# nianticlabs/panoptic-forecasting

Hardware: AMD Instinct MI355X
Metric: forecast frames/sec @1024x2048, 3-in->dt=3 bg (higher is better)
Workload: dtype f32 as 2 fp16 terms/operand, 3 MFMA products, f32 accumulate (strict f32: fp32_only); 1 GPU; configs[1] bg short-term forecast 3-in dt=3 @1024x2048: 3 warp/splats + HarDNet-70 + upsample/argmax; resident_frames_per_gpu=128, streams=4, sub_batch=32, launch=hipGraph replay, sub-batches staggered, weights=random-init, calibrated (tests/golden/calib_seed1234.json), world=1, device=AMD Radeon Graphics, backend=single process

## Files before the change

### include/pfhip.h

```cpp
#ifndef PFHIP_H
#define PFHIP_H

#include <stddef.h>
#include <stdint.h>

#ifdef __cplusplus
extern "C" {
#endif

#define PF_OK 0
#define PF_EINVAL (-1)
#define PF_EWORKSPACE (-2)
#define PF_EBLOB (-3)
#define PF_EHIP (-4)
#define PF_EUNSUPPORTED (-5)

typedef struct pf_plan pf_plan;

int pf_version(void);
const char *pf_last_error(void);

#define PF_SPLAT_PER_FRAME 1
#define PF_SPLAT_PER_SAMPLE_SENTINEL 2
int pf_warp_splat_workspace(int B, int T, int H, int W, int per_frame, size_t *bytes);
int pf_warp_splat(const float *depth, const uint8_t *depth_mask, const uint8_t *seg, int seg_channels,
                  const float *Kinv, const float *E, const float *T_tgt, const float *Einv,
                  const float *K, int B, int T_total, int t_first, int T, int H, int W, int per_frame,
                  uint8_t *out_seg, float *out_depth, int64_t *out_result2d,
                  void *ws, size_t ws_bytes, void *stream);

int pf_hardnet_plan_create(const void *blob_host, size_t bytes, int in_ch, int n_cls, pf_plan **out);
void pf_hardnet_plan_destroy(pf_plan *plan);
int pf_hardnet_workspace(const pf_plan *plan, int B, int H, int W, size_t *bytes);

#define PF_STATUS_RANGE 1u
#define PF_STATUS_RANGE_LOW 2u
#define PF_WS_STATUS_OFFSET 0
#define PF_WS_STICKY_OFFSET 4
#define PF_WS_STATUS_BYTES 2048
int pf_hardnet_status(const void *ws, unsigned *status, void *stream);
int pf_hardnet_status_sticky(void *ws, unsigned *status, int clear, void *stream);
int pf_hardnet_status_reset(void *ws, void *stream);
int pf_hardnet_range_maxima(const pf_plan *plan, const void *ws, float *maxima, int cap, int *n_ops, void *stream);

#define PF_HOP_NONE 0
#define PF_HOP_TRAINID_LUT 1
#define PF_HOP_DEPTH_U16 2

int pf_bg_forward(const pf_plan *plan, const void *seg, int seg_is_i64, const float *depth,
                  const uint8_t *depth_mask, float depth_mean, float depth_std, int hop_flags,
                  float min_depth, float max_depth, int B, int T, int H, int W, int out_h, int out_w,
                  void *out_seg, int out_seg_is_i64, float *out_logits, float *out_orig_logits,
                  void *ws, size_t ws_bytes, void *stream);

int pf_hardnet_forward_dense(const pf_plan *plan, const float *x, int B, int H, int W, int out_h,
                             int out_w, void *out_seg, int out_seg_is_i64, float *out_logits,
                             float *out_orig_logits, void *ws, size_t ws_bytes, void *stream);

int pf_hop_export(const void *seg, int seg_is_i64, int seg_mode, const float *depth, size_t n, uint8_t *out_seg,
                  uint16_t *out_depth_u16, void *stream);
int pf_hop_load(const uint16_t *depth_u16, size_t n, float min_depth, float max_depth, float *out_depth,
                uint8_t *out_mask, void *stream);

int pf_panoptic_merge_workspace(int n_instances, size_t *bytes);
int pf_panoptic_merge(const void *background, int bg_kind, const float *bg_depth, const uint8_t *bg_depth_mask,
                      const float *masks, int MH, int MW, const float *boxes, int box_is_ulbr,
                      const float *inst_depth, const int64_t *classes, const int32_t *inst_offsets,
                      int n_instances, int B, int H, int W, int use_depth_sorting, int panoptic_ids,
                      int clear_things, void *out, int out_is_i64, void *ws, size_t ws_bytes, void *stream);
int pf_panoptic_encode(const void *seg, int seg_is_i64, int convert_to_ids, int B, int H, int W, uint8_t *out_rgb,
                       int32_t *out_ids, uint8_t *out_present, void *stream);
int pf_panoptic_max_ids(void);

int pf_bg_dense_input(const void *frames, int kind, int channels, const float *depth, const uint8_t *depth_mask, float depth_mean,
                      float depth_std, int B, int T, int H, int W, float *x, void *stream);

int pf_seg_loss_workspace(int B, int out_h, int out_w, size_t *bytes);
int pf_seg_loss(const float *logits, int B, int C, int Hin, int Win, const void *labels, int labels_i64, int out_h,
                int out_w, int ignore_index, double *out3, void *ws, size_t ws_bytes, void *stream);

int pf_fg_weights_size(int flags, size_t *raw_floats, size_t *packed_floats);
int pf_fg_pack(const float *raw, float *packed, int flags, void *stream);
int pf_fg_workspace(int N, int T_in, int T_out, int flags, size_t *bytes);
int pf_fg_forward(const float *packed, int flags, int N, int T_in, int T_out, int odom_T, const float *trajs,
                  const float *traj_mask, const float *vel_mask, const float *feats, const int64_t *output_inds,
                  const float *odom, const float *depths, const float *depth_mask, const int64_t *classes,
                  float *traj_norm, float *traj_unnorm, float *mask_feats, float *output_feats, float *masks,
                  void *ws, size_t ws_bytes, void *stream);

int pf_odom_weights_size(int flags, size_t *raw_floats, size_t *packed_floats);
int pf_odom_pack(const float *raw, float *packed, int flags, void *stream);
int pf_odom_forward(const float *packed, int flags, int B, int T_in, int T_out, const float *inps, float *out,
                    float *out_norm, void *stream);

int pf_set_option(const char *name, int value);
int pf_hardnet_plan_set_option(pf_plan *plan, const char *name, int value);

typedef struct pf_train pf_train;
int pf_train_create(const void *blob, size_t blob_bytes, int in_ch, int n_cls, pf_train **out);
void pf_train_destroy(pf_train *t);
int pf_train_autotune(pf_train *t, int enable);
int pf_train_tuned_shapes(const pf_train *t, int *rows, int cap_rows, int *n_rows);
int pf_train_path_stats(const pf_train *t, int *stats, int cap, int *n);
int pf_train_param_count(const pf_train *t, size_t *n_floats);
int pf_train_param_layout(const pf_train *t, int op_index, size_t *w_off, size_t *aux_off, int *has_bn);
int pf_train_workspace(const pf_train *t, int B, int H, int W, int out_h, int out_w, size_t *bytes);
int pf_train_forward_backward(const pf_train *t, float *theta, float *grad, int accumulate_grads, const void *seg, int seg_is_i64,
                              const float *depth, const uint8_t *depth_mask, float depth_mean, float depth_std, int T,
                              const float *x_dense, int B, int H, int W, const void *labels, int labels_i64, int out_h, int out_w,
                              int ignore_index, float loss_scale, float bn_momentum, float bn_eps, int update_running_stats,
                              double *out3, void *ws, size_t ws_bytes, void *stream);
int pf_train_tensor_view(const pf_train *t, const char *name, int want_grad, int B, int H, int W, int out_h, int out_w,
                         size_t *ws_offset, int *channels, int *h, int *w);
int pf_sgd_workspace(size_t *bytes);
int pf_sgd_step(float *theta, float *grad, float *momentum_buf, const uint8_t *trainable, size_t n, float lr, float momentum,
                float weight_decay, float clip_norm, float clip_value, int first_step, void *ws, size_t ws_bytes, void *stream);

int pf_hardnet_tensor_view(const pf_plan *plan, const char *name, int B, int H, int W,
                           size_t *ws_offset, int *channels, int *h, int *w);
int pf_hardnet_tensor_read(const pf_plan *plan, const char *name, int B, int H, int W, const void *ws, float *dst, void *stream);
int pf_s4_pack(const float *src, void *dst, int B, int C, int H, int W, unsigned *status, void *stream);
int pf_s4_unpack(const void *src, float *dst, int B, int C, int H, int W, void *stream);
int pf_hardnet_flops(const pf_plan *plan, int H, int W, double *flops);

int pf_profile_enable(int on);
int pf_profile_collect(void);
int pf_profile_get(int i, char *label, size_t label_cap, int *launches, double *total_ms, double *flops,
                   double *bytes);

int pf_debug_force_conv(int kind, int p0, int p1, int p2);
int pf_debug_probe_read(long long *host64);

#ifdef __cplusplus
}
#endif
#endif
```

### panoptic-forecasting_amd/bg_model.py

```python
import collections.abc
import ctypes

import torch
import torch.nn.functional as F
from torch import nn

from . import hardnet_arch as arch
from . import lib as _lib
from . import packing
from .model_api import BaseModel
from .pc_transform_model import _as_u8


PLAN_OPTIONS = {'split_f16': 'split_f16', 'split_bf16': 'split_f16', 'fuse_pool': 'fuse_pool', 'fuse_upsample': 'fuse_upsample',
                'use_tuned_table': 'use_tuned_table', 'valu_remainder': 'valu_remainder', 'conv_table_batch': 'table_batch',
                'range_guard': 'range_guard', 'fuse_front': 'fuse_front', 'fuse_pairs': 'fuse_pairs'}
PF_STATUS_RANGE, PF_STATUS_RANGE_LOW = 1, 2
PF_STATUS_ANY = PF_STATUS_RANGE | PF_STATUS_RANGE_LOW
PF_WS_STATUS_BYTES = 2048


class _Pending:
    __slots__ = ('slot', 'event', 'stream', 'args', 'outs', 'done', 'stamps', 'error')


def _stamp(t):
    if not torch.is_tensor(t):
        return None
    return (t.data_ptr(), None if t.is_inference() else t._version)


def _unversioned(stamps):
    return any(s is not None and s[1] is None for s in stamps)


class LazyResult(collections.abc.MutableMapping):

    __slots__ = ('_data', '_model', '_token')

    def __init__(self, data, model, token):
        self._data, self._model, self._token = dict(data), model, token

    def _resolve(self):
        if self._token is not None:
            self._model._resolve(self._token)
            self._token = None

    def __getitem__(self, k):
        self._resolve()
        return self._data[k]

    def __setitem__(self, k, v):
        self._data[k] = v

    def __delitem__(self, k):
        self._resolve()
        del self._data[k]

    def __iter__(self):
        return iter(self._data)

    def __len__(self):
        return len(self._data)

    def __contains__(self, k):
        return k in self._data

    def keys(self):
        return self._data.keys()

    def copy(self):
        self._resolve()
        return dict(self._data)

    def __or__(self, other):
        return {**self.copy(), **other}

    def __ror__(self, other):
        return {**other, **self.copy()}

    def __reduce__(self):
        return (dict, (self.copy(),))

    def __repr__(self):
        return 'LazyResult(%s%s)' % (list(self._data), ', unchecked' if self._token is not None else '')


class _Node(nn.Module):
    """Anonymous container: gives dotted state_dict paths without any behaviour."""


def _get_or_make(root, path):
    node = root
    for part in path:
        if not hasattr(node, part):
            node.add_module(part, _Node())
        node = getattr(node, part)
    return node


class HardNetParams(nn.Module):

    def __init__(self, in_ch, n_cls):
        super().__init__()
        self.spec = arch.Spec(in_ch, n_cls)
        for op in self.spec.conv_ops():
            parts = op.name.split('.')
            if op.bn:
                holder = _get_or_make(self, parts)
                cin = 3 if op.kind == arch.OP_STEM else op.cin
                holder.add_module('conv', nn.Conv2d(cin, op.cout, op.k, op.stride, op.k // 2, bias=False))
                holder.add_module('norm', nn.BatchNorm2d(op.cout))
            else:
                parent = _get_or_make(self, parts[:-1])
                conv = nn.Conv2d(op.cin, op.cout, op.k, op.stride, 0, bias=True)
                nn.init.kaiming_normal_(conv.weight)
                parent.add_module(parts[-1], conv)
        stem = getattr(self.base, '0').conv
        w = stem.weight.data.mean(1, keepdim=True).expand(-1, in_ch, -1, -1).clone()
        stem.weight = nn.Parameter(w)

    def load_pretrained(self, path):
        sd = torch.load(path, map_location='cpu')['model_state']
        sd = {k[len('module.'):]: v for k, v in sd.items()}
        own = self.state_dict()
        for k, v in sd.items():
            if k in own and own[k].shape == v.shape:
                own[k].copy_(v)
            elif k == 'base.0.conv.weight':
                own[k].copy_(v.mean(1, keepdim=True).expand_as(own[k]))


class BGModel(BaseModel):

    def __init__(self, params):
        super().__init__()
        self.num_classes = num_classes = params['data']['num_classes']
        self.use_depth_inps = params['model'].get('use_depth_inps')
        self.num_inputs = params['model'].get('num_inputs', 1)
        self.min_depth = params['data'].get('min_depth')
        self.max_depth = params['data'].get('max_depth')
        self.convert2onehot = params['model'].get('convert2onehot')
        self.return_logits = params['model'].get('return_logits', True)
        final_w = params['model'].get('final_w')
        final_h = params['model'].get('final_h')
        self.final_size = (final_h, final_w) if final_w is not None and final_h is not None else None
        in_ch = num_classes
        if self.use_depth_inps:
            depth_norm_params = params['data'].get('depth_norm_params')
            if depth_norm_params is None:
                mean, std = torch.zeros(1), torch.zeros(1)
            else:
                mean, std = depth_norm_params
            self.depth_mean = nn.Parameter(torch.as_tensor(mean, dtype=torch.float32).reshape(1).clone(),
                                           requires_grad=False)
            self.depth_std = nn.Parameter(torch.as_tensor(std, dtype=torch.float32).reshape(1).clone(),
                                          requires_grad=False)
            in_ch += 1
        in_ch *= self.num_inputs
        self.in_ch = in_ch
        self.model = HardNetParams(in_ch, num_classes)
        pretrain = params['model'].get('hardnet', {}).get('pretrain_path')
        if pretrain is not None:
            self.model.load_pretrained(pretrain)
        self.plan_options = {c_name: int(params['model'][key]) for key, c_name in PLAN_OPTIONS.items()
                             if params['model'].get(key) is not None}
        self.on_range_overflow = params['model'].get('on_range_overflow', 'rerun')
        if self.on_range_overflow not in ('rerun', 'raise', 'ignore'):
            raise ValueError("model.on_range_overflow must be 'rerun', 'raise' or 'ignore'")
        self.range_check = params['model'].get('range_check', 'lazy')
        if self.range_check not in ('lazy', 'sync'):
            raise ValueError("model.range_check must be 'lazy' or 'sync'")
        self.range_reruns = 0
        self._pending = []
        self._pinned = None
        self._ring_next = 0
        self._plan = None
        self._ws = None
        self._norm = None
        self._trainer = None
        self._params_for_trainer = {'data': dict(params['data']), 'model': dict(params['model']),
                                    'training': dict(params.get('training') or {})}

    def load_state_dict(self, state_dict, strict=True):
        res = super().load_state_dict(state_dict, strict)
        self.invalidate()
        return res

    def invalidate(self):
        if self._pending:
            self._drain()
        if self._plan is not None:
            _lib.load().pf_hardnet_plan_destroy(self._plan)
        self._plan = None
        self._norm = None

    def __del__(self):
        try:
            self._pending = []
            self.invalidate()
        except Exception:
            pass

    def _get_plan(self):
        if self._plan is None:
            L = _lib.load()
            blob = packing.pack_blob(self.state_dict(), self.in_ch, self.num_classes)
            buf = ctypes.create_string_buffer(blob, len(blob))
            plan = ctypes.c_void_p()
            _lib.check(L.pf_hardnet_plan_create(buf, len(blob), self.in_ch, self.num_classes, ctypes.byref(plan)),
                       'pf_hardnet_plan_create')
            self._plan = plan
            for name, value in self.plan_options.items():
                _lib.check(L.pf_hardnet_plan_set_option(plan, name.encode(), value), 'pf_hardnet_plan_set_option')
            if self.use_depth_inps:
                self._norm = (float(self.depth_mean.item()), float(self.depth_std.item()))
        return self._plan

    def _workspace(self, b, h, w, device):
        L = _lib.load()
        need = ctypes.c_size_t()
        _lib.check(L.pf_hardnet_workspace(self._get_plan(), b, h, w, ctypes.byref(need)), 'pf_hardnet_workspace')
        if self._ws is None or self._ws.numel() < need.value or self._ws.device != device:
            if torch.cuda.is_current_stream_capturing():
                raise _lib.PfError('bg forward: the workspace must exist before stream capture (run one forward first)')
            self._drain()
            self._ws = torch.empty(need.value, dtype=torch.uint8, device=device)
            self._ws[:PF_WS_STATUS_BYTES].zero_()
        return self._ws

    def _guarded(self):
        return not (self.on_range_overflow == 'ignore' or self.plan_options.get('split_f16', 1) == 0
                    or self.plan_options.get('range_guard', 1) == 0)

    def range_status(self):
        if self._ws is None:
            return 0
        return int(self._ws[:4].view(torch.int32).item())

    def range_status_sticky(self, clear=False):
        if self._ws is None:
            return 0
        w = self._ws[4:8].view(torch.int32)
        v = int(w.item())
        if clear:
            w.zero_()
        return v

    def check_range(self, clear=True):
        self._drain()
        v = self.range_status_sticky(clear)
        if (v & PF_STATUS_ANY) and self._guarded():
            raise _lib.PfError('bg forward: status %d (PF_STATUS_RANGE = 1: |activation| > 65504, PF_STATUS_RANGE_LOW = 2: a tensor of '
                               'tiny values) on the two-term fp16 operand path inside a captured graph: the outputs of the flagged '
                               'replays are not usable; run eagerly (re-run on fp32) or with model.split_f16 = 0' % v)
        return v

    def range_maxima(self):
        L, plan = _lib.load(), self._get_plan()
        names = [op.name for op in self.model.spec.ops]
        buf = (ctypes.c_float * len(names))()
        n = ctypes.c_int()
        _lib.check(L.pf_hardnet_range_maxima(plan, self._ws.data_ptr(), buf, len(names), ctypes.byref(n), _lib.stream_ptr()),
                   'pf_hardnet_range_maxima')
        return {names[i]: float(buf[i]) for i in range(n.value)}

    _RING = 32

    def _resolve(self, token, owner=True):
        if token.done:
            if token.error is not None and owner:
                raise token.error
            return
        if not token.event.query():
            token.event.synchronize()
        token.done = True
        if token in self._pending:
            self._pending.remove(token)
        status = int(self._pinned[token.slot, 0])
        args, outs, stamps = token.args, token.outs, token.stamps
        token.args = token.outs = token.stamps = None
        if not (status & PF_STATUS_ANY):
            return
        if self.on_range_overflow == 'raise':
            token.error = _lib.PfError('bg forward: status %d on the two-term fp16 operand path (PF_STATUS_RANGE = 1: an activation '
                                       'exceeded 65504; PF_STATUS_RANGE_LOW = 2: a tensor of tiny values, max below 2^-6); run with '
                                       "model.split_f16 = 0 or on_range_overflow = 'rerun'" % status)
        elif stamps is not None and stamps != tuple(_stamp(t) for t in args[:3]):
            token.error = _lib.PfError('bg forward: status %d on the two-term fp16 operand path, and the input tensors of that forward were '
                                       'modified in place before its result was first touched - the fp32 re-run cannot see the original '
                                       "frame.  Keep a forward's inputs unchanged until its result has been read (or model.settle()), or "
                                       "build the model with model.range_check = 'sync'" % status)
        if token.error is not None:
            if owner:
                raise token.error
            return
        L, plan = _lib.load(), self._get_plan()
        self.range_reruns += 1
        prior = self.plan_options.get('split_f16', 1)
        _lib.check(L.pf_hardnet_plan_set_option(plan, b'split_f16', 0), 'pf_hardnet_plan_set_option')
        try:
            here = torch.cuda.current_stream()
            with torch.cuda.stream(token.stream):
                self._run_once(*args, outs=outs)
            if here != token.stream:
                here.wait_stream(token.stream)
        finally:
            _lib.check(L.pf_hardnet_plan_set_option(plan, b'split_f16', prior), 'pf_hardnet_plan_set_option')

    def _poll(self):
        while self._pending and self._pending[0].event.query():
            self._resolve(self._pending[0], owner=False)

    def _drain(self):
        while self._pending:
            self._resolve(self._pending[0], owner=False)

    def settle(self):
        self._drain()

    def run_async(self, inps, depths, depth_masks, want_logits=True, want_orig=True, hop_flags=0, seg_dtype=torch.int64,
                  own_inputs=False):
        capturing = torch.cuda.is_current_stream_capturing()
        if not capturing:
            self._poll()
        args = (inps, depths, depth_masks, want_logits, want_orig, hop_flags, seg_dtype)
        outs = self._run_once(*args)
        if not self._guarded() or capturing:
            return outs, None
        if self._pinned is None:
            self._pinned = torch.zeros((self._RING, 2), dtype=torch.int32).pin_memory()
        slot = self._ring_next
        self._ring_next = (slot + 1) % self._RING
        for t in list(self._pending):
            if t.slot == slot:
                self._resolve(t, owner=False)
        self._pinned[slot].copy_(self._ws[:8].view(torch.int32), non_blocking=True)
        token = _Pending()
        token.slot, token.args, token.outs, token.done, token.error = slot, args, outs, False, None
        token.stamps = None if own_inputs else tuple(_stamp(t) for t in args[:3])
        token.stream = torch.cuda.current_stream()
        token.event = torch.cuda.Event()
        token.event.record(token.stream)
        self._pending.append(token)
        if token.stamps is not None and _unversioned(token.stamps):
            self._resolve(token)
            return outs, None
        return outs, token

    def run(self, inps, depths, depth_masks, want_logits=True, want_orig=True, hop_flags=0, seg_dtype=torch.int64):
        outs, token = self.run_async(inps, depths, depth_masks, want_logits, want_orig, hop_flags, seg_dtype)
        if token is not None:
            self._resolve(token)
        return outs

    def _run_once(self, inps, depths, depth_masks, want_logits, want_orig, hop_flags, seg_dtype, outs=None):
        L = _lib.load()
        plan = self._get_plan()
        fused = bool(self.convert2onehot and self.use_depth_inps and inps.dim() == 4)
        if fused:
            b, t, h, w = inps.shape
        else:
            x = self._dense_input(inps, depths, depth_masks)
            b, _, h, w = x.shape
        dev = inps.device
        oh, ow = self.final_size if self.final_size is not None else (h, w)
        ws = self._workspace(b, h, w, dev)
        if outs is not None:
            seg, logits, orig = outs
        else:
            seg = torch.empty((b, oh, ow), dtype=seg_dtype, device=dev)
            logits = torch.empty((b, self.num_classes, oh, ow), dtype=torch.float32, device=dev) if want_logits else None
            orig = None
            if want_orig:
                vo, vc, vh, vw = ctypes.c_size_t(), ctypes.c_int(), ctypes.c_int(), ctypes.c_int()
                _lib.check(L.pf_hardnet_tensor_view(plan, b'finalConv', b, h, w, ctypes.byref(vo), ctypes.byref(vc),
                                                    ctypes.byref(vh), ctypes.byref(vw)), 'pf_hardnet_tensor_view')
                orig = torch.empty((b, vc.value, vh.value, vw.value), dtype=torch.float32, device=dev)
        ptr = lambda t_: t_.data_ptr() if t_ is not None else None
        i64 = int(seg_dtype == torch.int64)
        if fused:
            if inps.dtype not in (torch.uint8, torch.int64):
                inps = inps.long()
            inps = _lib.require_cuda(inps.contiguous(), 'seg')
            depths = _lib.require_cuda(depths.float().contiguous(), 'depth')
            mask = None
            if not (hop_flags & 2):
                mask = _lib.require_cuda(_as_u8(depth_masks), 'depth_mask')
            mean, std = self._norm
            rc = L.pf_bg_forward(plan, inps.data_ptr(), int(inps.dtype == torch.int64), depths.data_ptr(), ptr(mask),
                                 mean, std, hop_flags, float(self.min_depth or 0.0), float(self.max_depth or 0.0),
                                 b, t, h, w, oh, ow, seg.data_ptr(), i64, ptr(logits), ptr(orig),
                                 ws.data_ptr(), ws.numel(), _lib.stream_ptr())
            _lib.check(rc, 'pf_bg_forward')
        else:
            x = _lib.require_cuda(x.contiguous(), 'input')
            rc = L.pf_hardnet_forward_dense(plan, x.data_ptr(), b, h, w, oh, ow, seg.data_ptr(), i64, ptr(logits),
                                            ptr(orig), ws.data_ptr(), ws.numel(), _lib.stream_ptr())
            _lib.check(rc, 'pf_hardnet_forward_dense')
        return seg, logits, orig

    def _dense_input(self, inps, depths, depth_masks):
        L = _lib.load()
        if self.convert2onehot:
            b, t, h, w = inps.shape
            if inps.dtype not in (torch.uint8, torch.int64):
                inps = inps.long()
            frames, kind, c = _lib.require_cuda(inps.contiguous(), 'seg'), int(inps.dtype == torch.int64), self.num_classes
        else:
            b, t, c, h, w = inps.shape
            frames, kind = _lib.require_cuda(inps.float().contiguous(), 'seg'), 2
        dptr = mptr = None
        mean = std = 0.0
        if self.use_depth_inps:
            depths = _lib.require_cuda(depths.float().contiguous(), 'depth')
            mask = _lib.require_cuda(_as_u8(depth_masks), 'depth_mask')
            dptr, mptr = depths.data_ptr(), mask.data_ptr()
            self._get_plan()
            mean, std = self._norm
        x = torch.empty((b, t * c + (t if self.use_depth_inps else 0), h, w), dtype=torch.float32, device=inps.device)
        _lib.check(L.pf_bg_dense_input(frames.data_ptr(), kind, c, dptr, mptr, mean, std, b, t, h, w, x.data_ptr(), _lib.stream_ptr()),
                   'pf_bg_dense_input')
        return x

    def forward(self, inps, depths, depth_masks, return_orig_size=False):
        _, logits, orig = self.run(inps, depths, depth_masks, True, return_orig_size)
        return (logits, orig) if return_orig_size else logits

    def loss(self, inputs, labels):
        if self.training:
            return self._train_loss(inputs, labels)
        with torch.no_grad():
            return self._eval_loss(inputs, labels)

    def _get_trainer(self):
        from . import bg_train
        if self._trainer is None:
            self._trainer = bg_train.BGTrainer(self._params_for_trainer, device='cuda')
        if not self._trainer.is_adopted():
            self._trainer.adopt(self)
        return self._trainer

    def _train_loss(self, inputs, labels):
        from . import bg_train
        tr = self._get_trainer()
        self.invalidate()
        loss, acc = bg_train.TrainStepFunction.apply(tr, inputs, labels, *tr._adopted)
        torch._foreach_add_(self._bn_counters(), 1)
        return {'loss': loss, 'accuracy': acc}

    def _bn_counters(self):
        return [b for k, b in self.named_buffers() if k.endswith('num_batches_tracked')]

    def _eval_loss(self, inputs, labels):
        L = _lib.load()
        seg_labels = labels['seg']
        _, _, orig = self.run(inputs['seg'], inputs.get('depth'), inputs.get('depth_mask'), want_logits=False, want_orig=True)
        if seg_labels.dtype not in (torch.uint8, torch.int64):
            seg_labels = seg_labels.long()
        seg_labels = _lib.require_cuda(seg_labels.contiguous(), 'labels')
        b, c, hin, win = orig.shape
        oh, ow = seg_labels.shape[-2], seg_labels.shape[-1]
        need = ctypes.c_size_t()
        _lib.check(L.pf_seg_loss_workspace(b, oh, ow, ctypes.byref(need)), 'pf_seg_loss_workspace')
        ws = torch.empty(need.value, dtype=torch.uint8, device=orig.device)
        out3 = torch.empty(3, dtype=torch.float64, device=orig.device)
        _lib.check(L.pf_seg_loss(orig.data_ptr(), b, c, hin, win, seg_labels.data_ptr(), int(seg_labels.dtype == torch.int64), oh, ow,
                                 255, out3.data_ptr(), ws.data_ptr(), ws.numel(), _lib.stream_ptr()), 'pf_seg_loss')
        return {'loss': (out3[0] / out3[1]).float(), 'accuracy': (out3[2] / out3[1]).float()}

    @torch.no_grad()
    def predict(self, inputs, labels=None):
        (seg, logits, orig), token = self.run_async(inputs['seg'], inputs.get('depth'), inputs.get('depth_mask'),
                                                    want_logits=self.return_logits, want_orig=True)
        out = {'seg': seg, 'orig_size_logits': orig}
        if logits is not None:
            out['logits'] = logits
        if token is not None and self.range_check == 'sync':
            self._resolve(token)
            token = None
        return LazyResult(out, self, token)
```

### panoptic-forecasting_amd/csrc/conv_mfma.h

```cpp
#pragma once
#include "pf_blob.h"
#include "pf_common.h"

namespace pf {

struct ConvArgs {
    const float *src[kConvMaxSrc];
    int src_ctotal[kConvMaxSrc];
    int src_choff[kConvMaxSrc];
    int src_cstart[kConvMaxSrc + 1];
    int src_chunk0[kConvMaxSrc + 1];
    int n_src;
    const float *wpk;
    const float *bias;
    float *dst;
    int dst_ctotal, dst_choff;
    int Cin, Cout, Hin, Win, Hout, Wout;
    int tilesX, tilesY, nchunks, relu;
    const float *zero_page;
    int ntiles;
    int no_bias;
    int pool;
    const float *res;
    int res_ctotal, res_choff, Hres, Wres;
    float res_sh, res_sw;
    int res_lds_off;
    int res_rows, res_cols;
    unsigned res_magic_cs, res_magic_cols;
    const float *wrem;
    int rem;
    int src_begin, src_end;
    int chunk_begin, chunk_end;
    long long *probe;
    unsigned *status;
    unsigned *range_slot;
    int kacc;
    int accum;
    float acc_scale;
    int dst_fmt;
    int dst_c4;
    int dst_limit;
    int src_fmt;
    int src_c4[kConvMaxSrc];
    int src_g0[kConvMaxSrc];
    int src_gn[kConvMaxSrc];
    int src_ent0[kConvMaxSrc + 1];
};

typedef _Float16 split_t;
typedef split_t split_x2 __attribute__((ext_vector_type(2)));
typedef split_t split_x4 __attribute__((ext_vector_type(4)));
typedef split_t split_x8 __attribute__((ext_vector_type(8)));
constexpr float kSplitMaxAbs = 65504.f;
__device__ __forceinline__ void split_terms2(float x0, float x1, split_x2 &hi, split_x2 &mid) {
#if defined(__HIP_DEVICE_COMPILE__)
    typedef float f32x2 __attribute__((ext_vector_type(2)));
    hi = __builtin_convertvector(f32x2{x0, x1}, split_x2);
    const unsigned hu = __builtin_bit_cast(unsigned, hi);
    unsigned mu;
    asm("v_fma_mixlo_f16 %0, %1, -1.0, %2 op_sel_hi:[1,0,0]" : "=v"(mu) : "v"(hu), "v"(x0));
    asm("v_fma_mixhi_f16 %0, %1, -1.0, %2 op_sel:[1,0,0] op_sel_hi:[1,0,0]" : "+v"(mu) : "v"(hu), "v"(x1));
    mid = __builtin_bit_cast(split_x2, mu);
#endif
}
__device__ __forceinline__ float range_acc(float m, float a, float b, float c, float d) {
#if defined(__HIP_DEVICE_COMPILE__)
    asm("v_max3_f32 %0, %0, |%1|, |%2|" : "+v"(m) : "v"(a), "v"(b));
    asm("v_max3_f32 %0, %0, |%1|, |%2|" : "+v"(m) : "v"(c), "v"(d));
#endif
    return m;
}
constexpr float kRangeTarget = 8.0f;
constexpr float kRangeLowMax = 0.015625f;
__device__ __forceinline__ bool range_sampled() {
#if defined(__HIP_DEVICE_COMPILE__)
    const unsigned total = gridDim.x * gridDim.y * gridDim.z;
    const unsigned id = blockIdx.x + gridDim.x * (blockIdx.y + gridDim.y * blockIdx.z);
    const unsigned mask = total >= 16u ? (1u << (28 - __builtin_clz(total))) - 1u : 0u;
    return (((id * 0x9E3779B1u) >> 9) & mask) == 0u;
#else
    return false;
#endif
}
__device__ __forceinline__ void range_commit(unsigned *status, unsigned *slot, float m) {
#if defined(__HIP_DEVICE_COMPILE__)
    if (status == nullptr) return;
    if (!(m <= kSplitMaxAbs)) atomicOr(status, 1u);
    if (slot == nullptr || !range_sampled()) return;
    const unsigned mb = __builtin_bit_cast(unsigned, m);
    unsigned wm = 0;
    unsigned long long above = __builtin_amdgcn_ballot_w64(mb > wm);
    while (above != 0) {
        wm = (unsigned)__builtin_amdgcn_readlane((int)mb, (int)__builtin_ctzll(above));
        above = __builtin_amdgcn_ballot_w64(mb > wm);
    }
    const unsigned lane_id = __builtin_amdgcn_mbcnt_hi(~0u, __builtin_amdgcn_mbcnt_lo(~0u, 0u));
    if (lane_id == (unsigned)__builtin_ctzll(__builtin_amdgcn_ballot_w64(true))) atomicMax(slot, wm | 1u);
#endif
}
template <typename V4>
__device__ __forceinline__ void split_terms4(const V4 &v, split_x4 &hi, split_x4 &mid) {
    split_x2 h0, m0, h1, m1;
    split_terms2(v[0], v[1], h0, m0);
    split_terms2(v[2], v[3], h1, m1);
    hi = split_x4{h0[0], h0[1], h1[0], h1[1]};
    mid = split_x4{m0[0], m0[1], m1[0], m1[1]};
}
#define PF_MFMA_SPLIT(a, b, c) __builtin_amdgcn_mfma_f32_16x16x32_f16((a), (b), (c), 0, 0, 0)
unsigned short split_host_f16(float x);
float split_host_f32(unsigned short h);
float split_weight_scale(const float *w, size_t n);

__device__ __forceinline__ void xcd_tile_order(int ntiles_xy, int &tile_lin, int &group) {
#if defined(__HIP_DEVICE_COMPILE__)
    if ((ntiles_xy & 7) != 0) {
        tile_lin = (int)blockIdx.x;
        group = (int)blockIdx.y;
        return;
    }
    const int ngroups = (int)gridDim.y;
    const int lin = (int)blockIdx.x + ntiles_xy * (int)blockIdx.y;
    const int xcd = lin & 7, pos = lin >> 3;
    const int t = pos / ngroups;
    group = pos - t * ngroups;
    tile_lin = xcd * (ntiles_xy >> 3) + t;
#endif
}

struct ConvTiling {
    int ks, stride;
    int kc;
    int nt;
    int twt;
    int cout_blocks, nchunks;
    size_t packed_floats() const { return (size_t)cout_blocks * nchunks * (kc / 4) * ks * ks * nt * 64; }
};

ConvTiling choose_tiling(int ks, int stride, int cin, int cout, int wout_hint);
void pack_conv_weights(const float *w_oihw, int cin, int cout, const ConvTiling &t, float *out);
int launch_conv(const ConvArgs &a, const ConvTiling &t, int B, hipStream_t stream);

constexpr int dma_kc_ct(int ks, int stride) { return ks == 1 ? 16 : (stride == 2 ? 4 : 8); }
inline int dma_kc(int ks, int stride) { return dma_kc_ct(ks, stride); }
int dma_chunks(const int *src_ch, int n_src, int ks, int stride);
inline int dma_rem_rv(int rem) { return rem <= 2 ? 2 : (rem + 3) / 4 * 4; }
inline int dma_valu_split(int cout) {
    if (cout < 16) return 0;
    return cout % 16;
}
void pack_conv_weights_rem(const float *w_oihw, int cin, int cout, int rem, int ks, int kc, const int *src_ch, int n_src, float *out);
void pack_conv_weights_tiled(const float *w_oihw, int cin, int cout, int ks, int kc, const int *src_ch, int n_src, float *out);
int launch_conv_dma(const ConvArgs &a, int ks, int stride, int B, hipStream_t stream, int force_wm = 0, int force_nt = 0, int model_B = 0);
bool conv_dma_supported(const ConvArgs &a, int ks, int stride, int B, int force_wm, int force_nt, int model_B, int *wm, int *nt);

constexpr int wave_kc_ct(int ks) { return ks == 1 ? 32 : 8; }
inline int wave_kc(int ks) { return wave_kc_ct(ks); }
int wave_chunks(const int *src_ch, int n_src, int ks);
void pack_conv_weights_wave(const float *w_oihw, int cin, int cout, int ks, const int *src_ch, int n_src, float *out);
size_t wave_packed_floats(const int *src_ch, int n_src, int cout, int ks);
int launch_conv_wave(const ConvArgs &a, int ks, int mh, int nt, int wk, int B, hipStream_t stream);
bool conv_wave_supported(const ConvArgs &a, int ks, int mh, int nt, int wk);
constexpr size_t wave_lds_bytes(int ks, int mh, int nt, int wk) {
    const int kc = wave_kc_ct(ks), ih = mh + ks - 1, iw = 16 + (ks == 3 ? 8 : 0);
    const int raw = ih * iw, plane = (raw + 15) / 32 * 32 + 16, nit = (kc * (plane / 4) + 63) / 64;
    const size_t ring = (size_t)wk * 2 * nit * 256, red = (size_t)wk * mh * nt * 256;
    return 4 * (ring > red ? ring : red);
}

int split_chunks(const int *src_ch, int n_src);
size_t split_packed_floats(const int *src_ch, int n_src, int cout);
void pack_conv_weights_split(const float *w_oihw, int cin, int cout, const int *src_ch, int n_src, float *out);
int launch_conv_split(const ConvArgs &a, int nt, int wide, int B, hipStream_t stream);
bool conv_split_supported(const ConvArgs &a);
int split1_chunks(const int *src_ch, int n_src);
size_t split1_packed_floats(const int *src_ch, int n_src, int cout);
void pack_conv_weights_split1(const float *w_oihw, int cin, int cout, const int *src_ch, int n_src, float *out);
int launch_conv_split1(const ConvArgs &a, int nt, int B, hipStream_t stream);
bool conv_split1_supported(const ConvArgs &a, int nt);

struct S4Range { int choff, ch; };
int s4_entries(const S4Range *r, int n_src, int ks, int pad_sources);
int s4_rounds(const S4Range *r, int n_src, int ks, int pad_sources);
size_t s4_packed_floats(const S4Range *r, int n_src, int cout, int ks, int pad_sources);
void pack_conv_weights_s4(const float *w_oihw, int cin, int cout, int ks, const S4Range *r, int n_src, int pad_sources, float *out);
int launch_conv_s4(const ConvArgs &a, int ks, int nt, int wide, int B, hipStream_t stream);
void pack_conv_weights_s4_ex(const float *w_oihw, int cin, int cout, int ks, const S4Range *r, const int *cstart, int n_src, int pad_sources, float *out);

struct PairArgs {
    ConvArgs c;
    const float *p_wpk;
    const float *p_w9;
    const float *p_bias;
    float p_acc_scale;
    float *p_dst;
    int p_dst_c4, p_dst_choff, p_dst_limit, p_cout, p_cin, p_ntiles, p_relu;
    unsigned *p_range_slot;
    int rounds_s;
    int round_d;
    int merged;
};
bool conv_pair_supports(int c_cout, int p_cout);
bool conv_pair_merged_supports(int c_cout, int p_cout);
bool pair_wanted(int p_cin, int p_cout, int c_cin, int c_cout, int h, int w, int B, int mode);
size_t pair_p_two_floats(const S4Range &r, int cout);
size_t pair_p_nine_floats(const S4Range &r, int cout);
void pack_conv_weights_pair_p(const float *w_oihw, int cin, int cout, const S4Range &r, float *two, float *nine);
int launch_conv_pair(const PairArgs &pa, int B, hipStream_t stream);
int launch_s4_pack(const float *src, void *dst, int B, int C, int H, int W, unsigned *status, hipStream_t stream);
int launch_range_check(const float *x, size_t n, unsigned *status, unsigned *slot, hipStream_t stream);
int launch_range_finalize(unsigned *st, int live_word, int first_slot, int n_slots, int sticky_word, hipStream_t stream);
int launch_s4_unpack(const void *src, float *dst, int B, int C, int H, int W, hipStream_t stream);

struct FrontArgs {
    const void *x;
    const void *w1, *w2;
    const float *bias1, *bias2;
    float scale1, scale2;
    float *dst;
    int dst_fmt, dst_c4, dst_ctotal, dst_choff, dst_limit;
    int H1, W1, H2, W2, C1, C2, relu1, relu2;
    int tilesX, tilesY;
    int seg_steps;
    unsigned *status;
    unsigned *range_slot_mid, *range_slot;
    long long *probe;
};

bool conv_front_supports(int c0, int c1, int c2, int h1, int w1, int dst_ctotal);
int launch_conv_front(const FrontArgs &a, int B, hipStream_t s);

struct ConvChoice {
    int kind, p0, p1, p2;
};
ConvChoice choose_conv(int ks, int stride, int cin, int cout, int hout, int wout, int B, int need = 0, int use_tuned = 1);
bool choose_s4(int ks, int cin, int cout, int hout, int wout, int B, ConvChoice *out);
long long *probe_buffer();
extern ConvChoice g_conv_force;

}
```

### panoptic-forecasting_amd/csrc/conv_s4.hip

```cpp
#include <cstring>
#include <vector>

#include "conv_s4.h"
#include "pf_prof.h"

#ifndef PF_PROBE
#define PF_PROBE 0
#endif
#if PF_PROBE
#define S4_PROBE(i) do { if (threadIdx.x == 0 && blockIdx.x == gridDim.x / 2 && blockIdx.y == 0 && blockIdx.z == gridDim.z / 2 && a.probe && (i) < 60) a.probe[i] = clock64(); } while (0)
#else
#define S4_PROBE(i) do { } while (0)
#endif

[[maybe_unused]] constexpr int kS4IssueFirst = 1, kS4IssueStep = 2;

namespace pf {

template <int NT, int TW_, int TH_ = 8, int KS_ = 1>
struct S4Cfg {
    static constexpr int TW = TW_, TH = TH_, MTR = TW / 16, MP = 2 * MTR;
    static constexpr int KS = KS_;
    static constexpr int NW = TH / 2, NTHR = 64 * NW;
    static constexpr int IW = TW + 4, IH = TH + 2;
    static constexpr int ROWP = IW / 2, PIECES = IH * ROWP;
    static constexpr int NDMA_ALL = (PIECES + 63) / 64;
    static constexpr int NDMA = (NDMA_ALL + NW / 4 - 1) / (NW / 4);
    static constexpr bool COLREG = (NT == 2 || NT == 3) && TW_ == 32;
    static constexpr int PLANE = COLREG ? PIECES * 16 : NDMA_ALL * 64 * 16;
    static constexpr int ABUF = 4 * PLANE;
    static constexpr int WBLK = 2 * 64 * 16;
    static constexpr int BPT = COLREG ? 2 : 3;
    static constexpr int WBUF = NT * BPT * WBLK;
    static constexpr int WPIECES = WBUF / 16, NITW = (WPIECES + NTHR - 1) / NTHR;
    static constexpr size_t STAGES_BYTES = 2 * (size_t)ABUF + 2 * (size_t)WBUF;
    static constexpr size_t LDS_BYTES = KS * STAGES_BYTES + NT * 16 * sizeof(float);
    static_assert(KS == 1 || (size_t)MP * NT * NW * 64 * 16 <= STAGES_BYTES, "the K-split hand-over uses group 1's stage ring");
};

#define S4_KERNEL_NAME conv_s4_kernel
#define S4_KERNEL_KACC 0
#define S4_KERNEL_WAVES (KS_ == 4 ? 1 : (TH_ == 16 || KS_ == 2) ? 2 : (TW_ == 32 && NT <= 2) ? 4 : (TW_ == 32 && NT == 3) ? 3 : 2)
#include "conv_s4_kernel.inc"
#undef S4_KERNEL_NAME
#undef S4_KERNEL_KACC
#undef S4_KERNEL_WAVES
#define S4_KERNEL_NAME conv_s4_blocked_kernel
#define S4_KERNEL_KACC 1
#define S4_KERNEL_WAVES (NT == 1 ? 4 : (NT == 2 ? 3 : 2))
#include "conv_s4_kernel.inc"
#undef S4_KERNEL_NAME
#undef S4_KERNEL_KACC
#undef S4_KERNEL_WAVES

template <int NT, int TW_, int TH_ = 8, int KS_ = 1>
static int launch_s4_cfg(const ConvArgs &a0, int B, hipStream_t s) {
    using C = S4Cfg<NT, TW_, TH_, KS_>;
    ConvArgs a = a0;
    a.tilesX = (a.Wout + C::TW - 1) / C::TW;
    a.tilesY = (a.Hout + C::TH - 1) / C::TH;
    static bool attr_set = false;
    if (!attr_set) {
        PF_HIP_CHECK(hipFuncSetAttribute(reinterpret_cast<const void *>(&conv_s4_kernel<NT, TW_, TH_, KS_>),
                                         hipFuncAttributeMaxDynamicSharedMemorySize, (int)C::LDS_BYTES));
        attr_set = true;
    }
    char label[96];
    snprintf(label, sizeof(label), "void pf::conv_s4_kernel<%d, %d, %d, %d>(pf::ConvArgs)", NT, TW_, TH_, KS_);
    const double px = (double)B * a.Hout * a.Wout;
    ProfScope ps(s, label, 2.0 * px * a.Cout * a.Cin * 9,
                 4.0 * ((double)B * a.Cin * a.Hin * a.Win + px * a.Cout + (double)a.Cout * a.Cin * 9));
    hipLaunchKernelGGL((conv_s4_kernel<NT, TW_, TH_, KS_>), dim3(a.tilesX * a.tilesY, (a.ntiles + NT - 1) / NT, B), dim3(C::NTHR * C::KS), C::LDS_BYTES, s, a);
    PF_LAUNCH_CHECK("conv_s4_kernel");
    return PF_OK;
}

template <int NT>
static int launch_s4_blocked_cfg(const ConvArgs &a0, int B, hipStream_t s) {
    using C = S4Cfg<NT, 32, 8, 1>;
    ConvArgs a = a0;
    a.tilesX = (a.Wout + C::TW - 1) / C::TW;
    a.tilesY = (a.Hout + C::TH - 1) / C::TH;
    static bool attr_set = false;
    if (!attr_set) {
        PF_HIP_CHECK(hipFuncSetAttribute(reinterpret_cast<const void *>(&conv_s4_blocked_kernel<NT, 32, 8, 1>), hipFuncAttributeMaxDynamicSharedMemorySize, (int)C::LDS_BYTES));
        attr_set = true;
    }
    char label[96];
    snprintf(label, sizeof(label), "void pf::conv_s4_blocked_kernel<%d, 32, 8, 1>(pf::ConvArgs)", NT);
    const double px = (double)B * a.Hout * a.Wout;
    ProfScope ps(s, label, 2.0 * px * a.Cout * a.Cin * 9, 4.0 * ((double)B * a.Cin * a.Hin * a.Win + px * a.Cout + (double)a.Cout * a.Cin * 9));
    hipLaunchKernelGGL((conv_s4_blocked_kernel<NT, 32, 8, 1>), dim3(a.tilesX * a.tilesY, (a.ntiles + NT - 1) / NT, B), dim3(C::NTHR), C::LDS_BYTES, s, a);
    PF_LAUNCH_CHECK("conv_s4_blocked_kernel");
    return PF_OK;
}

template <int NT>
struct S41Cfg {
    static constexpr int TW = 32, TH = 8, MP = 4;
    static constexpr int WBUF = NT * 2 * 64 * 16;
    static constexpr int BIAS_OFF = 2 * WBUF;
    static constexpr int MAIN = 2 * WBUF + 256;
    static constexpr int WPIECES = WBUF / 16, NITW = (WPIECES + 255) / 256;
};

typedef unsigned s4_u32x4 __attribute__((ext_vector_type(4)));
typedef unsigned s4_u32x2 __attribute__((ext_vector_type(2)));

template <int NT, int EPI>
__global__ __launch_bounds__(256, NT <= 2 ? 4 : (NT == 3 ? 3 : 2)) void conv_s4_1x1_kernel(ConvArgs a) {
#if defined(__HIP_DEVICE_COMPILE__)
    using C = S41Cfg<NT>;
    extern __shared__ __attribute__((aligned(16))) unsigned char smem_raw[];
    const int tid = threadIdx.x, lane = tid & 63;
    const int wave = __builtin_amdgcn_readfirstlane(tid >> 6);
    int tid_lin, cgroup;
    xcd_tile_order(a.tilesX * a.tilesY, tid_lin, cgroup);
    const int tileY = tid_lin / a.tilesX, tileX = tid_lin - tileY * a.tilesX;
    const int tile0 = cgroup * NT, b = blockIdx.z;
    const size_t plane_bytes = (size_t)a.Hin * a.Win * 8;
    auto wbuf = [&](int i) { return smem_raw + i * C::WBUF; };
    const int g = lane >> 4;

    s4_f32x4 acc[C::MP][NT];
#pragma unroll
    for (int m = 0; m < C::MP; ++m)
#pragma unroll
        for (int n = 0; n < NT; ++n) acc[m][n] = s4_f32x4{0.f, 0.f, 0.f, 0.f};
    const bool has_res = EPI == 1 && a.res && a.res_lds_off >= 0;
    ResWin rw = ResWin();

    int poff[2];
#pragma unroll
    for (int rr = 0; rr < 2; ++rr) {
        const int gy = tileY * C::TH + 2 * wave + rr, gx = tileX * C::TW + 2 * (lane & 15);
        poff[rr] = (gy < a.Hin && gx < a.Win) ? (gy * a.Win + gx) * 8 : -1;
    }
    unsigned woff[C::NITW];
#pragma unroll
    for (int it = 0; it < C::NITW; ++it) {
        const int p = it * 256 + tid, n = p / (2 * 64);
        woff[it] = (p < C::WPIECES && tile0 + n < a.ntiles) ? (unsigned)((tile0 + n) * a.nchunks * (2 * 64) + (p - n * (2 * 64))) * 16u : kS4Oob;
    }
    const __amdgpu_buffer_rsrc_t wrsrc = __builtin_amdgcn_make_buffer_rsrc((void *)a.wpk, 0, 0x7FFFFFFF, 0x00020000);

    float *bias_lds = reinterpret_cast<float *>(smem_raw + C::BIAS_OFF);
    if (wave == 0 && lane < NT * 16) {
        const __amdgpu_buffer_rsrc_t brs = __builtin_amdgcn_make_buffer_rsrc((void *)a.bias, 0, 0x7FFFFFFF, 0x00020000);
        const int co = tile0 * 16 + lane;
        __builtin_amdgcn_raw_ptr_buffer_load_lds(brs, (s4_lds_ptr_t)bias_lds, 4, (!a.no_bias && co < a.ntiles * 16) ? (unsigned)co * 4u : kS4Oob, 0,
                                                 0, 0);
    }

    const int cb = a.chunk_begin, nrounds = a.chunk_end - cb;
    auto load_round = [&](int r, s4_u32x4 (&x)[2][2][2]) {
#pragma unroll
        for (int h = 0; h < 2; ++h) {
            const int e = 8 * (cb + r) + 2 * g + h;
            const float *sp = a.src[0];
            int c4 = a.src_c4[0], g0 = a.src_g0[0], gn = a.src_gn[0], e0 = 0;
#pragma unroll
            for (int k = 1; k < kConvMaxSrc; ++k) {
                const bool take = k < a.n_src && e >= a.src_ent0[k];
                sp = take ? a.src[k] : sp;
                c4 = take ? a.src_c4[k] : c4;
                g0 = take ? a.src_g0[k] : g0;
                gn = take ? a.src_gn[k] : gn;
                e0 = take ? a.src_ent0[k] : e0;
            }
            const bool real = e - e0 < gn;
            const char *hi = reinterpret_cast<const char *>(sp) + ((size_t)b * 2 * c4 + (g0 + min(e - e0, gn - 1))) * plane_bytes;
            const size_t tstride = (size_t)c4 * plane_bytes;
#pragma unroll
            for (int rr = 0; rr < 2; ++rr) {
                const bool ok = real && poff[rr] >= 0;
                const char *p = ok ? hi + poff[rr] : reinterpret_cast<const char *>(a.zero_page);
                x[rr][h][0] = *reinterpret_cast<const s4_u32x4 *>(p);
                x[rr][h][1] = *reinterpret_cast<const s4_u32x4 *>(ok ? p + tstride : p);
            }
        }
    };
    auto load_weights = [&](int r, unsigned char *wdst) {
#pragma unroll
        for (int it = 0; it < C::NITW; ++it)
            if (it * 256 + tid < C::WPIECES)
                __builtin_amdgcn_raw_ptr_buffer_load_lds(wrsrc, (s4_lds_ptr_t)(wdst + (it * 256 + wave * 64) * 16), 16, woff[it],
                                                         (unsigned)(cb + r) * (2 * 64 * 16), 0, 0);
    };

    s4_u32x4 cur[2][2][2], nxt[2][2][2];
    if (nrounds > 0) {
        load_weights(0, wbuf(0));
        load_round(0, cur);
    }
    if (has_res) {
        rw = res_window(a, tileY * C::TH, C::TH, tileX * C::TW, C::TW);
        rw.rows = a.res_rows;
        rw.cols = a.res_cols;
        rw.cs = res_chan_stride(a.res_rows, a.res_cols);
        const unsigned per = (unsigned)(rw.rows * rw.cols), total = (unsigned)(NT * 16 * rw.cs);
        const size_t rplane = (size_t)a.Hres * a.Wres;
        const __amdgpu_buffer_rsrc_t rrs = __builtin_amdgcn_make_buffer_rsrc(
            (void *)(a.res + ((size_t)b * a.res_ctotal + a.res_choff + tile0 * 16) * rplane), 0, 0x7FFFFFFF, 0x00020000);
        unsigned char *rdst = smem_raw + a.res_lds_off * 4;
        for (unsigned e0 = (unsigned)wave * 64; e0 < total; e0 += 256) {
            const unsigned e = e0 + lane;
            const unsigned c = __umulhi(e, a.res_magic_cs), rem = e - c * (unsigned)rw.cs;
            const unsigned r = __umulhi(rem, a.res_magic_cols), x = rem - r * (unsigned)rw.cols;
            const int row = min(rw.sy0 + (int)r, a.Hres - 1), col = min(rw.sx0 + (int)x, a.Wres - 1);
            const bool ok = e < total && rem < per && tile0 * 16 + (int)c < a.Cout;
            const unsigned off = ok ? (unsigned)((c * rplane + (size_t)row * a.Wres + col) * 4) : kS4Oob;
            __builtin_amdgcn_raw_ptr_buffer_load_lds(rrs, (s4_lds_ptr_t)(rdst + e0 * 4), 4, off, 0, 0, 0);
        }
    }

    for (int round = 0; round < nrounds; ++round) {
        asm volatile("s_waitcnt vmcnt(0)" ::: "memory");
        __syncthreads();
        const bool more = round + 1 < nrounds;
        if (more) {
            load_weights(round + 1, wbuf((round + 1) & 1));
            load_round(round + 1, nxt);
        }
        const unsigned char *wb = wbuf(round & 1);
        s4_h8 bh[NT], bm[NT];
#pragma unroll
        for (int n = 0; n < NT; ++n) {
            bh[n] = *reinterpret_cast<const s4_h8 *>(wb + ((n * 2 + 0) * 64 + lane) * 16);
            bm[n] = *reinterpret_cast<const s4_h8 *>(wb + ((n * 2 + 1) * 64 + lane) * 16);
        }
#pragma unroll
        for (int rr = 0; rr < 2; ++rr)
#pragma unroll
            for (int q = 0; q < 2; ++q) {
                const s4_u32x4 h0 = cur[rr][0][0], h1 = cur[rr][1][0], m0 = cur[rr][0][1], m1 = cur[rr][1][1];
                const s4_u32x4 fh = q ? s4_u32x4{h0[2], h0[3], h1[2], h1[3]} : s4_u32x4{h0[0], h0[1], h1[0], h1[1]};
                const s4_u32x4 fm = q ? s4_u32x4{m0[2], m0[3], m1[2], m1[3]} : s4_u32x4{m0[0], m0[1], m1[0], m1[1]};
                const s4_h8 ah = __builtin_bit_cast(s4_h8, fh), am = __builtin_bit_cast(s4_h8, fm);
                const int m = rr * 2 + q;
#pragma unroll
                for (int n = 0; n < NT; ++n) acc[m][n] = PF_MFMA_SPLIT(bh[n], am, acc[m][n]);
#pragma unroll
                for (int n = 0; n < NT; ++n) acc[m][n] = PF_MFMA_SPLIT(bm[n], ah, acc[m][n]);
#pragma unroll
                for (int n = 0; n < NT; ++n) acc[m][n] = PF_MFMA_SPLIT(bh[n], ah, acc[m][n]);
            }
        if (more) {
#pragma unroll
            for (int rr = 0; rr < 2; ++rr)
#pragma unroll
                for (int h = 0; h < 2; ++h)
#pragma unroll
                    for (int t = 0; t < 2; ++t) cur[rr][h][t] = nxt[rr][h][t];
        }
    }

    if (has_res) {
        asm volatile("s_waitcnt vmcnt(0)" ::: "memory");
        __syncthreads();
    }
    {
        __builtin_amdgcn_s_waitcnt(0x0F70);
        const lds_float *res_lds = (const lds_float *)(reinterpret_cast<float *>(smem_raw) + (has_res ? a.res_lds_off : 0));
        const int i2 = 2 * (lane & 15);
        const int ox = tileX * C::TW + i2;
        const bool pooled = EPI == 1 && a.pool;
        const int Ho = pooled ? a.Hout >> 1 : a.Hout, Wo = pooled ? a.Wout >> 1 : a.Wout;
        const size_t hw = (size_t)Ho * Wo, term = (size_t)a.dst_c4 * hw * 8;
        const bool mis = (a.dst_choff & 2) != 0;
        typedef split_x2 h2;
        float vmax = 0.f;
        const float relu_lo1 = a.relu ? 0.f : -__builtin_inff();
        auto finish = [&](int rr, int q, int n, const int (&o0)[2], const int (&o1)[2], const float (&lx1)[2], float hy1) {
            s4_f32x4 v = acc[rr * 2 + q][n];
            const s4_f32x4 b4 = *reinterpret_cast<const s4_f32x4 *>(bias_lds + n * 16 + 4 * g);
#pragma unroll
            for (int r = 0; r < 4; ++r) {
                v[r] = v[r] * a.acc_scale + b4[r];
                if (has_res) {
                    const lds_float *chan = res_lds + (n * 16 + 4 * g + r) * rw.cs;
                    const float lx0 = 1.f - lx1[q], hy0 = 1.f - hy1;
                    const float t0 = lx0 * chan[o0[q]] + lx1[q] * chan[o0[q] + 1];
                    const float t1 = lx0 * chan[o1[q]] + lx1[q] * chan[o1[q] + 1];
                    v[r] += hy0 * t0 + hy1 * t1;
                }
                v[r] = fmaxf(v[r], relu_lo1);
            }
            vmax = range_acc(vmax, v[0], v[1], v[2], v[3]);
            return v;
        };
        auto store_px = [&](int co, size_t pix, s4_f32x4 v) {
            if (a.dst_fmt) {
                s4_h4 hi, mid;
                split_terms4(v, hi, mid);
                const int chb = a.dst_choff + co;
                const bool ok0 = chb < a.dst_limit, ok1 = chb + 2 < a.dst_limit;
                char *p = reinterpret_cast<char *>(a.dst) + (size_t)b * 2 * term + pix * 8 + (size_t)(chb >> 2) * hw * 8;
                if (!mis) {
                    if (ok1) {
                        *reinterpret_cast<s4_h4 *>(p) = hi;
                        *reinterpret_cast<s4_h4 *>(p + term) = mid;
                    } else if (ok0) {
                        *reinterpret_cast<h2 *>(p) = h2{hi[0], hi[1]};
                        *reinterpret_cast<h2 *>(p + term) = h2{mid[0], mid[1]};
                    }
                } else {
                    if (ok0) {
                        *reinterpret_cast<h2 *>(p + 4) = h2{hi[0], hi[1]};
                        *reinterpret_cast<h2 *>(p + 4 + term) = h2{mid[0], mid[1]};
                    }
                    if (ok1) {
                        *reinterpret_cast<h2 *>(p + hw * 8) = h2{hi[2], hi[3]};
                        *reinterpret_cast<h2 *>(p + hw * 8 + term) = h2{mid[2], mid[3]};
                    }
                }
            } else {
#pragma unroll
                for (int r = 0; r < 4; ++r)
                    if (co + r < a.Cout) a.dst[((size_t)b * a.dst_ctotal + a.dst_choff + co + r) * hw + pix] = v[r];
            }
        };
        auto store_pair = [&](int co, size_t pix, s4_f32x4 v0, s4_f32x4 v1) {
            const int chb = a.dst_choff + co;
            if (a.dst_fmt && !mis && chb + 2 < a.dst_limit) {
                s4_h4 h0, m0, h1, m1;
                split_terms4(v0, h0, m0);
                split_terms4(v1, h1, m1);
                const s4_h8 hi = s4_join(h0, h1), mid = s4_join(m0, m1);
                char *p = reinterpret_cast<char *>(a.dst) + (size_t)b * 2 * term + pix * 8 + (size_t)(chb >> 2) * hw * 8;
                *reinterpret_cast<s4_h8 *>(p) = hi;
                *reinterpret_cast<s4_h8 *>(p + term) = mid;
            } else if (!a.dst_fmt) {
                typedef float f2 __attribute__((ext_vector_type(2)));
#pragma unroll
                for (int r = 0; r < 4; ++r)
                    if (co + r < a.Cout)
                        *reinterpret_cast<f2 *>(a.dst + ((size_t)b * a.dst_ctotal + a.dst_choff + co + r) * hw + pix) = f2{v0[r], v1[r]};
            } else {
                store_px(co, pix, v0);
                store_px(co, pix + 1, v1);
            }
        };
#pragma unroll
        for (int rr = 0; rr < 2; ++rr) {
            if (pooled && rr == 1) continue;
            const int oy = tileY * C::TH + 2 * wave + rr;
            if (oy >= a.Hout || ox >= a.Wout) continue;
            if (pooled && oy + 1 >= a.Hout) continue;
            int o0[2] = {0, 0}, o1[2] = {0, 0}, p0[2] = {0, 0}, p1[2] = {0, 0};
            float lx1[2] = {0.f, 0.f}, hy1 = 0.f, hy1b = 0.f;
            if (has_res) {
                int y0, y1;
                float hy0;
                lin_coord(oy, a.res_sh, a.Hres, y0, y1, hy0, hy1);
                int z0 = 0, z1 = 0;
                if (pooled) lin_coord(oy + 1, a.res_sh, a.Hres, z0, z1, hy0, hy1b);
#pragma unroll
                for (int q = 0; q < 2; ++q) {
                    int x0, x1;
                    float lx0;
                    lin_coord(min(ox + q, a.Wout - 1), a.res_sw, a.Wres, x0, x1, lx0, lx1[q]);
                    o0[q] = (y0 - rw.sy0) * rw.cols + (x0 - rw.sx0);
                    o1[q] = (y1 - rw.sy0) * rw.cols + (x0 - rw.sx0);
                    p0[q] = (z0 - rw.sy0) * rw.cols + (x0 - rw.sx0);
                    p1[q] = (z1 - rw.sy0) * rw.cols + (x0 - rw.sx0);
                }
            }
#pragma unroll
            for (int n = 0; n < NT; ++n) {
                const int co = (tile0 + n) * 16 + 4 * g;
                if (co >= a.Cout + 2) continue;
                const s4_f32x4 va = finish(rr, 0, n, o0, o1, lx1, hy1), vb = finish(rr, 1, n, o0, o1, lx1, hy1);
                if (!pooled) {
                    store_pair(co, (size_t)oy * a.Wout + ox, va, vb);
                } else {
                    const s4_f32x4 vc = finish(1, 0, n, p0, p1, lx1, hy1b), vd = finish(1, 1, n, p0, p1, lx1, hy1b);
                    s4_f32x4 pv;
#pragma unroll
                    for (int r = 0; r < 4; ++r) pv[r] = (((va[r] + vb[r]) + vc[r]) + vd[r]) * 0.25f;
                    if ((oy >> 1) < Ho && (ox >> 1) < Wo) store_px(co, (size_t)(oy >> 1) * Wo + (ox >> 1), pv);
                }
                __builtin_amdgcn_sched_barrier(0);
            }
        }
        range_commit(a.status, a.range_slot, vmax);
    }
#endif
}

template <int NT, int EPI>
static int launch_s41_cfg(const ConvArgs &a0, int B, hipStream_t s) {
    using C = S41Cfg<NT>;
    ConvArgs a = a0;
    a.tilesX = (a.Wout + C::TW - 1) / C::TW;
    a.tilesY = (a.Hout + C::TH - 1) / C::TH;
    size_t lds = C::MAIN;
    a.res_lds_off = -1;
    if (a.res) {
        a.res_rows = res_extent(C::TH, a.res_sh);
        a.res_cols = res_extent(C::TW, a.res_sw);
        const int cs = res_chan_stride(a.res_rows, a.res_cols);
        const size_t need = (size_t)NT * 16 * cs * sizeof(float);
        if (need > 64 * 1024 || (size_t)NT * 16 * cs >= 65536) return fail(PF_EUNSUPPORTED, "conv_s4 1x1: residual window of %zu B does not fit LDS", need);
        a.res_magic_cs = (unsigned)(0x100000000ull / (unsigned)cs) + 1u;
        a.res_magic_cols = (unsigned)(0x100000000ull / (unsigned)a.res_cols) + 1u;
        a.res_lds_off = C::MAIN / 4;
        lds = C::MAIN + align_up(need, 256);
    }
    static size_t attr_lds = 0;
    if (lds > attr_lds) {
        PF_HIP_CHECK(hipFuncSetAttribute(reinterpret_cast<const void *>(&conv_s4_1x1_kernel<NT, EPI>),
                                         hipFuncAttributeMaxDynamicSharedMemorySize, (int)lds));
        attr_lds = lds;
    }
    char label[112];
    snprintf(label, sizeof(label), "void pf::conv_s4_1x1_kernel<%d, %d>(pf::ConvArgs)", NT, EPI);
    if (a.res) strncat(label, " +res", sizeof(label) - strlen(label) - 1);
    if (a.pool) strncat(label, " +pool", sizeof(label) - strlen(label) - 1);
    if (a.no_bias) strncat(label, " lowres-half", sizeof(label) - strlen(label) - 1);
    const double px = (double)B * a.Hout * a.Wout;
    ProfScope ps(s, label, 2.0 * px * a.Cout * a.Cin, 4.0 * ((double)B * a.Cin * a.Hin * a.Win + px * a.Cout + (double)a.Cout * a.Cin));
    hipLaunchKernelGGL((conv_s4_1x1_kernel<NT, EPI>), dim3(a.tilesX * a.tilesY, (a.ntiles + NT - 1) / NT, B), dim3(256), lds, s, a);
    PF_LAUNCH_CHECK("conv_s4_1x1_kernel");
    return PF_OK;
}

int launch_conv_s4(const ConvArgs &a, int ks, int nt, int wide, int B, hipStream_t s) {
    if (!a.src_fmt) return fail(PF_EINVAL, "conv_s4: sources are not in the S4 layout");
    if ((a.Wout & 3) != 0 || a.Hin != a.Hout || a.Win != a.Wout) return fail(PF_EUNSUPPORTED, "conv_s4: stride 1, width % 4 == 0 only");
    nt = nt < 1 ? 1 : (nt > a.ntiles ? a.ntiles : nt);
    if (ks == 3) {
        if (a.pool || a.res || a.no_bias) return fail(PF_EUNSUPPORTED, "conv_s4 3x3: no fused epilogue stages");
        if (a.chunk_begin != 0 || a.chunk_end != a.nchunks) return fail(PF_EUNSUPPORTED, "conv_s4 3x3: whole K range only");
        if (a.kacc) {
            if (nt == 1) return launch_s4_blocked_cfg<1>(a, B, s);
            if (nt == 2) return launch_s4_blocked_cfg<2>(a, B, s);
            return launch_s4_blocked_cfg<3>(a, B, s);
        }
        if (wide == 2) {
            if (nt == 1) return launch_s4_cfg<1, 32, 16>(a, B, s);
            return launch_s4_cfg<2, 32, 16>(a, B, s);
        }
        if (wide == 4 && a.nchunks >= 16) {
            if (nt == 1) return launch_s4_cfg<1, 32, 8, 4>(a, B, s);
            return launch_s4_cfg<2, 32, 8, 4>(a, B, s);
        }
        if (wide >= 3 && a.nchunks >= 8) {
            if (nt == 1) return launch_s4_cfg<1, 32, 8, 2>(a, B, s);
            return launch_s4_cfg<2, 32, 8, 2>(a, B, s);
        }
        if (wide >= 3) wide = 0;
        if (wide) {
            if (nt == 1) return launch_s4_cfg<1, 64>(a, B, s);
            if (nt == 2) return launch_s4_cfg<2, 64>(a, B, s);
            return launch_s4_cfg<3, 32>(a, B, s);
        }
        if (nt == 1) return launch_s4_cfg<1, 32>(a, B, s);
        if (nt == 2) return launch_s4_cfg<2, 32>(a, B, s);
        if (nt == 3) return launch_s4_cfg<3, 32>(a, B, s);
        return launch_s4_cfg<4, 32>(a, B, s);
    }
    nt = nt > 4 ? 4 : nt;
    const bool fused = a.pool || a.res || a.no_bias;
#define PF_S41(NT_) \
    if (nt == NT_) return fused ? launch_s41_cfg<NT_, 1>(a, B, s) : launch_s41_cfg<NT_, 0>(a, B, s);
    PF_S41(1) PF_S41(2) PF_S41(3) PF_S41(4)
#undef PF_S41
    return PF_EUNSUPPORTED;
}

static int s4_range_groups(const S4Range &r) { return (r.choff + r.ch + 3) / 4 - r.choff / 4; }
int s4_entries(const S4Range *r, int n_src, int ks, int pad_sources) {
    const int per = ks == 3 ? 2 : 8;
    int n = 0;
    for (int j = 0; j < n_src; ++j) n += pad_sources ? (s4_range_groups(r[j]) + per - 1) / per * per : s4_range_groups(r[j]);
    return n;
}
int s4_rounds(const S4Range *r, int n_src, int ks, int pad_sources) {
    const int per = ks == 3 ? 2 : 8;
    return (s4_entries(r, n_src, ks, pad_sources) + per - 1) / per;
}
size_t s4_packed_floats(const S4Range *r, int n_src, int cout, int ks, int pad_sources) {
    const int rounds = s4_rounds(r, n_src, ks, pad_sources);
    return (size_t)((cout + 15) / 16) * (ks == 3 ? s4_blocks_total(rounds) : rounds) * 2 * 64 * 4;
}

void pack_conv_weights_s4(const float *w, int cin, int cout, int ks, const S4Range *r, int n_src, int pad_sources, float *out_f) {
    pack_conv_weights_s4_ex(w, cin, cout, ks, r, nullptr, n_src, pad_sources, out_f);
}
void pack_conv_weights_s4_ex(const float *w, int cin, int cout, int ks, const S4Range *r, const int *cstart, int n_src, int pad_sources, float *out_f) {
    unsigned short *out = reinterpret_cast<unsigned short *>(out_f);
    std::vector<int> ent_c0, ent_lo, ent_hi;
    const int per = ks == 3 ? 2 : 8;
    int c0 = 0;
    for (int j = 0; j < n_src; ++j) {
        if (cstart) c0 = cstart[j];
        const int g0 = r[j].choff / 4, g1 = (r[j].choff + r[j].ch + 3) / 4;
        for (int g = g0; g < g1; ++g) {
            ent_c0.push_back(c0 + 4 * g - r[j].choff);
            ent_lo.push_back(c0);
            ent_hi.push_back(c0 + r[j].ch);
        }
        while (pad_sources && ent_c0.size() % per != 0) {
            ent_c0.push_back(0);
            ent_lo.push_back(0);
            ent_hi.push_back(0);
        }
        c0 += r[j].ch;
    }
    const int n_ent = (int)ent_c0.size(), rounds = (n_ent + per - 1) / per, ntiles = (cout + 15) / 16;
    size_t o = 0;
    auto block = [&](int t, auto ent_of, auto tap_of) {
        for (int term = 0; term < 2; ++term)
            for (int lane = 0; lane < 64; ++lane)
                for (int e = 0; e < 8; ++e) {
                    const int co = t * 16 + (lane & 15), g = lane >> 4;
                    const int ent = ent_of(g, e / 4), tap = tap_of(g);
                    float v = 0.f;
                    if (co < cout && tap >= 0 && ent >= 0 && ent < n_ent) {
                        const int ci = ent_c0[ent] + (e & 3);
                        if (ci >= ent_lo[ent] && ci < ent_hi[ent]) v = w[((size_t)co * cin + ci) * ks * ks + tap];
                    }
                    const unsigned short hi = split_host_f16(v);
                    out[o++] = term == 0 ? hi : split_host_f16(v - split_host_f32(hi));
                }
    };
    static const int tap3[2][4] = {{0, 1, 3, 4}, {6, 7, 2, 5}};
    for (int t = 0; t < ntiles; ++t)
        for (int rd = 0; rd < rounds; ++rd) {
            if (ks == 1) {
                block(t, [&](int g, int h) { return rd * 8 + g * 2 + h; }, [](int) { return 0; });
                continue;
            }
            for (int s = 0; s < 2; ++s) block(t, [&](int, int h) { return rd * 2 + h; }, [&](int g) { return tap3[s][g]; });
            if ((rd & 3) == 3 || rd == rounds - 1) {
                const int q = rd / 4;
                block(t, [&](int g, int h) { return 4 * q + g < rounds ? (4 * q + g) * 2 + h : -1; }, [](int) { return 8; });
            }
        }
}

__global__ void s4_pack_kernel(const float *src, unsigned short *dst, int B, int C, int H, int W, unsigned *status) {
    const size_t hw = (size_t)H * W, c4 = (C + 3) / 4, n = (size_t)B * c4 * hw;
    bool bad = false;
    for (size_t i = (size_t)blockIdx.x * blockDim.x + threadIdx.x; i < n; i += (size_t)gridDim.x * blockDim.x) {
        const size_t px = i % hw, g = (i / hw) % c4, b = i / (hw * c4);
        for (int r = 0; r < 4; ++r) {
            const int c = (int)g * 4 + r;
            const float x = c < C ? src[((size_t)b * C + c) * hw + px] : 0.f;
            bad = bad || !(fabsf(x) <= kSplitMaxAbs);
            split_x2 h, m;
            split_terms2(x, 0.f, h, m);
            dst[(((b * 2 + 0) * c4 + g) * hw + px) * 4 + r] = __builtin_bit_cast(unsigned short, h[0]);
            dst[(((b * 2 + 1) * c4 + g) * hw + px) * 4 + r] = __builtin_bit_cast(unsigned short, m[0]);
        }
    }
    if (bad && status) atomicOr(status, 1u);
}
__global__ void range_check_kernel(const float *x, size_t n, unsigned *status, unsigned *slot) {
    bool bad = false;
    float m = 0.f;
    const size_t n4 = n / 4;
    for (size_t i = (size_t)blockIdx.x * blockDim.x + threadIdx.x; i < n4; i += (size_t)gridDim.x * blockDim.x) {
        const s4_f32x4 v = reinterpret_cast<const s4_f32x4 *>(x)[i];
        bad = bad || !(fabsf(v[0]) <= kSplitMaxAbs) || !(fabsf(v[1]) <= kSplitMaxAbs) || !(fabsf(v[2]) <= kSplitMaxAbs) ||
              !(fabsf(v[3]) <= kSplitMaxAbs);
        m = range_acc(m, v[0], v[1], v[2], v[3]);
    }
    if (blockIdx.x == 0 && threadIdx.x < n - n4 * 4) {
        const float t = x[n4 * 4 + threadIdx.x];
        bad = bad || !(fabsf(t) <= kSplitMaxAbs);
        m = range_acc(m, t, 0.f, 0.f, 0.f);
    }
    if (bad) atomicOr(status, 1u);
    range_commit(status, slot, m);
}
int launch_range_check(const float *x, size_t n, unsigned *status, unsigned *slot, hipStream_t s) {
    if (!status || n == 0) return PF_OK;
    if ((reinterpret_cast<uintptr_t>(x) & 15) != 0) return fail(PF_EINVAL, "range check: input is not 16-B aligned");
    const size_t blocks = (n / 4 + 255) / 256;
    hipLaunchKernelGGL(range_check_kernel, dim3((unsigned)(blocks < 2048 ? (blocks ? blocks : 1) : 2048)), dim3(256), 0, s, x, n, status, slot);
    PF_LAUNCH_CHECK("range_check_kernel");
    return PF_OK;
}
__global__ void range_finalize_kernel(unsigned *st, int live_word, int first_slot, int n_slots, unsigned low_bits, int sticky_word) {
    __shared__ unsigned low;
    if (threadIdx.x == 0) low = 0;
    __syncthreads();
    for (int i = threadIdx.x; i < n_slots; i += blockDim.x) {
        const unsigned v = st[first_slot + i];
        if ((v & ~1u) != 0 && v < low_bits) low = 1;
        st[first_slot + n_slots + i] = v;
        st[first_slot + i] = 0;
    }
    __syncthreads();
    if (threadIdx.x == 0) {
        const unsigned w = st[live_word] | (low ? 2u : 0u);
        st[0] = w;
        st[sticky_word] |= w;
        st[live_word] = 0;
    }
}
int launch_range_finalize(unsigned *st, int live_word, int first_slot, int n_slots, int sticky_word, hipStream_t s) {
    hipLaunchKernelGGL(range_finalize_kernel, dim3(1), dim3(256), 0, s, st, live_word, first_slot, n_slots,
                       __builtin_bit_cast(unsigned, kRangeLowMax), sticky_word);
    PF_LAUNCH_CHECK("range_finalize_kernel");
    return PF_OK;
}
__global__ void s4_unpack_kernel(const unsigned short *src, float *dst, int B, int C, int H, int W) {
    const size_t hw = (size_t)H * W, c4 = (C + 3) / 4, n = (size_t)B * C * hw;
    for (size_t i = (size_t)blockIdx.x * blockDim.x + threadIdx.x; i < n; i += (size_t)gridDim.x * blockDim.x) {
        const size_t px = i % hw, c = (i / hw) % C, b = i / (hw * C);
        const size_t at = ((c / 4) * hw + px) * 4 + (c & 3);
        const unsigned short h = src[(b * 2 + 0) * c4 * hw * 4 + at], m = src[(b * 2 + 1) * c4 * hw * 4 + at];
        dst[i] = (float)__builtin_bit_cast(split_t, h) + (float)__builtin_bit_cast(split_t, m);
    }
}
int launch_s4_pack(const float *src, void *dst, int B, int C, int H, int W, unsigned *status, hipStream_t s) {
    hipLaunchKernelGGL(s4_pack_kernel, dim3(1024), dim3(256), 0, s, src, (unsigned short *)dst, B, C, H, W, status);
    PF_LAUNCH_CHECK("s4_pack_kernel");
    return PF_OK;
}
int launch_s4_unpack(const void *src, float *dst, int B, int C, int H, int W, hipStream_t s) {
    hipLaunchKernelGGL(s4_unpack_kernel, dim3(1024), dim3(256), 0, s, (const unsigned short *)src, dst, B, C, H, W);
    PF_LAUNCH_CHECK("s4_unpack_kernel");
    return PF_OK;
}

}
```

### panoptic-forecasting_amd/csrc/conv_s4_kernel.inc

```
template <int NT, int TW_, int TH_, int KS_>
__global__ __launch_bounds__(32 * TH_ * KS_, S4_KERNEL_WAVES) void S4_KERNEL_NAME(ConvArgs a) {
    [[maybe_unused]] constexpr int KACC = S4_KERNEL_KACC;
#if defined(__HIP_DEVICE_COMPILE__)
    using C = S4Cfg<NT, TW_, TH_, KS_>;
    extern __shared__ __attribute__((aligned(16))) unsigned char smem_all[];
    const int lane = threadIdx.x & 63;
    const int wave_all = __builtin_amdgcn_readfirstlane((int)threadIdx.x >> 6);
    const int kgrp = C::KS > 1 ? wave_all / C::NW : 0;
    const int wave = C::KS > 1 ? wave_all % C::NW : wave_all;
    const int tid = C::KS > 1 ? (int)threadIdx.x & (C::NTHR - 1) : (int)threadIdx.x;
    unsigned char *const smem_raw = smem_all + kgrp * C::STAGES_BYTES;
    int tid_lin, cgroup;
    xcd_tile_order(a.tilesX * a.tilesY, tid_lin, cgroup);
    const int tileY = tid_lin / a.tilesX, tileX = tid_lin - tileY * a.tilesX;
    const int tile0 = cgroup * NT, b = blockIdx.z;
    const int iy0 = tileY * C::TH - 1, ix0 = tileX * C::TW - 2;
    const size_t plane_bytes = (size_t)a.Hin * a.Win * 8;
    auto abuf = [&](int i) { return smem_raw + i * C::ABUF; };
    auto wbuf = [&](int i) { return smem_raw + 2 * C::ABUF + i * C::WBUF; };

    s4_f32x4 acc[C::MP][NT];
    [[maybe_unused]] s4_f32x4 tot[KACC ? C::MP : 1][KACC ? NT : 1];
#pragma unroll
    for (int m = 0; m < C::MP; ++m)
#pragma unroll
        for (int n = 0; n < NT; ++n) {
            acc[m][n] = s4_f32x4{0.f, 0.f, 0.f, 0.f};
            if constexpr (KACC) tot[m][n] = s4_f32x4{0.f, 0.f, 0.f, 0.f};
        }

    const int w4 = C::NW == 4 ? wave : (wave & 3), jb = C::NW == 4 ? 0 : (wave >> 2) * C::NDMA;
    unsigned poff[C::NDMA];
#pragma unroll
    for (int j = 0; j < C::NDMA; ++j) {
        const int p = (jb + j) * 64 + lane, row = p / C::ROWP, cp = p - row * C::ROWP;
        const int gy = iy0 + row, gx = ix0 + 2 * cp;
        poff[j] = (p < C::PIECES && gy >= 0 && gy < a.Hin && gx >= 0 && gx < a.Win) ? (unsigned)(gy * a.Win + gx) * 8u : kS4Oob;
    }
    const int nblocks = s4_blocks_total(a.nchunks);
    unsigned woff[C::NITW];
    bool wcol[C::NITW];
#pragma unroll
    for (int it = 0; it < C::NITW; ++it) {
        const int p = it * C::NTHR + tid, n = p / (C::BPT * 2 * 64), rem = p - n * (C::BPT * 2 * 64);
        woff[it] = (p < C::WPIECES && tile0 + n < a.ntiles) ? ((unsigned)(tile0 + n) * (unsigned)nblocks * (2 * 64) + (unsigned)rem) * 16u : kS4Oob;
        wcol[it] = rem >= 2 * 2 * 64;
    }
    const __amdgpu_buffer_rsrc_t wrsrc = __builtin_amdgcn_make_buffer_rsrc((void *)a.wpk, 0, 0x7FFFFFFF, 0x00020000);

    const int g = lane >> 4;
    int aoff[2], aoff_col;
    {
        const int ky[2] = {g >> 1, g < 2 ? 2 : g - 2};
        const int kx[2] = {g & 1, g < 2 ? g : 2};
#pragma unroll
        for (int s = 0; s < 2; ++s) aoff[s] = ((wave * 2 + ky[s]) * C::IW + (lane & 15) + kx[s] + 1) * 8;
        aoff_col = ((wave * 2 + 2) * C::IW + (lane & 15) + 2 + 1) * 8;
    }

    float *bias_lds = reinterpret_cast<float *>(smem_all + C::KS * C::STAGES_BYTES);
    if (wave_all == 0 && lane < NT * 16) {
        const __amdgpu_buffer_rsrc_t brs = __builtin_amdgcn_make_buffer_rsrc((void *)a.bias, 0, 0x7FFFFFFF, 0x00020000);
        const int co = tile0 * 16 + lane;
        __builtin_amdgcn_raw_ptr_buffer_load_lds(brs, (s4_lds_ptr_t)bias_lds, 4, co < a.ntiles * 16 ? (unsigned)co * 4u : kS4Oob, 0, 0, 0);
    }

    const int nrounds = a.nchunks;
    const int chunk = C::KS > 1 ? (((nrounds + C::KS - 1) / C::KS + 3) / 4) * 4 : nrounds;
    const int r_begin = min(nrounds, kgrp * chunk), r_end = min(nrounds, r_begin + chunk);
    const int n_iter = chunk;
    constexpr int HALVES = C::MP / 4;
    __amdgpu_buffer_rsrc_t ars;
    unsigned asoff = 0;
    bool areal = true;
    auto prepare_round = [&](int r) {
        const char *base;
        unsigned goff, tstride;
        areal = s4_entry(a, 2 * r + (w4 & 1), b, plane_bytes, base, goff, tstride);
        ars = __builtin_amdgcn_make_buffer_rsrc((void *)base, 0, 0x7FFFFFFF, 0x00020000);
        asoff = goff + (unsigned)(w4 >> 1) * tstride;
    };
    auto is_flush = [&](int r) { return (r & 3) == 3 || r == nrounds - 1; };
    auto issue_part = [&](int r, int stage, int j) {
        if ((jb + j) * 64 + lane < C::PIECES)
            __builtin_amdgcn_raw_ptr_buffer_load_lds(ars, (s4_lds_ptr_t)(abuf(stage) + w4 * C::PLANE + (jb + j) * 1024), 16,
                                                     areal ? poff[j] : kS4Oob, asoff, 0, 0);
        unsigned char *wdst = wbuf(stage);
        const bool flush = is_flush(r);
#pragma unroll
        for (int it = j; it < C::NITW; it += C::NDMA)
            if (it * C::NTHR + tid < C::WPIECES && (flush || !wcol[it]))
                __builtin_amdgcn_raw_ptr_buffer_load_lds(wrsrc, (s4_lds_ptr_t)(wdst + (it * C::NTHR + wave * 64) * 16), 16, woff[it],
                                                         (unsigned)s4_blocks_before(r) * C::WBLK, 0, 0);
    };
    auto issue_slot = [&](int round, bool more, int slot) {
        if (!more) return;
#pragma unroll
        for (int j = 0; j < C::NDMA; ++j)
            if (slot == kS4IssueFirst + j * kS4IssueStep) issue_part(round + 1, (round + 1) & 1, j);
    };
    static_assert(kS4IssueFirst + (C::NDMA - 1) * kS4IssueStep < 6 * HALVES, "every DMA part needs a slot inside the two full instructions");

    s4_h8 col_h[C::MP], col_m[C::MP];
    const s4_h8 zero8 = {0, 0, 0, 0, 0, 0, 0, 0};
#pragma unroll
    for (int m = 0; m < C::MP; ++m) col_h[m] = col_m[m] = zero8;

    if (r_begin < r_end) {
        prepare_round(r_begin);
#pragma unroll
        for (int j = 0; j < C::NDMA; ++j) issue_part(r_begin, r_begin & 1, j);
    }
    for (int it_ = 0; it_ < n_iter; ++it_) {
        const int round = r_begin + it_;
        asm volatile("s_waitcnt vmcnt(0)" ::: "memory");
        S4_PROBE(round * 4 + 0);
        __syncthreads();
        S4_PROBE(round * 4 + 1);
        if (C::KS > 1 && round >= r_end) continue;
        const bool more = round + 1 < r_end;
        if (more) prepare_round(round + 1);
        S4_PROBE(round * 4 + 2);
        const unsigned char *ab = abuf(round & 1), *wb = wbuf(round & 1);
        auto frag = [&](const unsigned char *p, s4_h8 &h, s4_h8 &md) {
            typedef const volatile __attribute__((address_space(3))) s4_h4 *lds_h4;
            const lds_h4 q = (lds_h4)(const __attribute__((address_space(3))) unsigned char *)p;
            constexpr int PL = C::PLANE / 8;
            h = s4_join(q[0], q[PL]);
            md = s4_join(q[2 * PL], q[3 * PL]);
        };
        auto mtile_off = [&](int mm) {
            return ((mm / C::MTR) * C::IW + (mm % C::MTR) * 16) * 8;
        };
        constexpr int FT = (NT == 2 && C::MP == 4) ? 2 : 4;
        auto mfmas = [&](const s4_h8 (&wh)[NT], const s4_h8 (&wm)[NT], int m0, const auto &fh, const auto &fm, int slot0, bool dma) {
            constexpr int FTn = (int)(sizeof(fh) / sizeof(fh[0]));
#pragma unroll
            for (int m = 0; m < FTn; ++m)
#pragma unroll
                for (int n = 0; n < NT; ++n)
                    acc[m0 + m][n] = PF_MFMA_SPLIT(wh[n], fm[m], acc[m0 + m][n]);
            if (dma) issue_slot(round, more, slot0 + 0);
#pragma unroll
            for (int m = 0; m < FTn; ++m)
#pragma unroll
                for (int n = 0; n < NT; ++n)
                    acc[m0 + m][n] = PF_MFMA_SPLIT(wm[n], fh[m], acc[m0 + m][n]);
            if (dma) issue_slot(round, more, slot0 + 1);
#pragma unroll
            for (int m = 0; m < FTn; ++m)
#pragma unroll
                for (int n = 0; n < NT; ++n)
                    acc[m0 + m][n] = PF_MFMA_SPLIT(wh[n], fh[m], acc[m0 + m][n]);
            if (dma) issue_slot(round, more, slot0 + 2);
        };
        constexpr int NB = C::MP / FT;
#pragma unroll
        for (int s = 0; s < 2; ++s) {
            s4_h8 wh[NT], wm[NT];
#pragma unroll
            for (int n = 0; n < NT; ++n) {
                wh[n] = *reinterpret_cast<const s4_h8 *>(wb + (((n * C::BPT + s) * 2 + 0) * 64 + lane) * 16);
                wm[n] = *reinterpret_cast<const s4_h8 *>(wb + (((n * C::BPT + s) * 2 + 1) * 64 + lane) * 16);
            }
#pragma unroll
            for (int bt = 0; bt < NB; ++bt) {
                s4_h8 fh[FT], fm[FT];
#pragma unroll
                for (int m = 0; m < FT; ++m) frag(ab + aoff[s] + mtile_off(bt * FT + m), fh[m], fm[m]);
                mfmas(wh, wm, bt * FT, fh, fm, 3 * (s * NB + bt), true);
                __builtin_amdgcn_sched_barrier(0);
            }
        }
        if (g == (round & 3)) {
#pragma unroll
            for (int m = 0; m < C::MP; ++m) frag(ab + aoff_col + mtile_off(m), col_h[m], col_m[m]);
        }
        if (is_flush(round)) {
            s4_h8 cwh[NT], cwm[NT];
#pragma unroll
            for (int n = 0; n < NT; ++n) {
                if (C::COLREG) {
                    const bool real = tile0 + n < a.ntiles;
                    const char *wp = reinterpret_cast<const char *>(a.wpk) +
                                     ((size_t)(real ? tile0 + n : 0) * nblocks + s4_blocks_before(round) + 2) * C::WBLK + lane * 16;
                    cwh[n] = real ? *reinterpret_cast<const s4_h8 *>(wp) : zero8;
                    cwm[n] = real ? *reinterpret_cast<const s4_h8 *>(wp + 64 * 16) : zero8;
                } else {
                    cwh[n] = *reinterpret_cast<const s4_h8 *>(wb + (((n * 3 + 2) * 2 + 0) * 64 + lane) * 16);
                    cwm[n] = *reinterpret_cast<const s4_h8 *>(wb + (((n * 3 + 2) * 2 + 1) * 64 + lane) * 16);
                }
            }
#pragma unroll
            for (int hf = 0; hf < HALVES; ++hf) {
                s4_h8 fh[4], fm[4];
#pragma unroll
                for (int m = 0; m < 4; ++m) {
                    fh[m] = col_h[hf * 4 + m];
                    fm[m] = col_m[hf * 4 + m];
                }
                mfmas(cwh, cwm, hf * 4, fh, fm, 0, false);
                __builtin_amdgcn_sched_barrier(0);
            }
#pragma unroll
            for (int m = 0; m < C::MP; ++m) col_h[m] = col_m[m] = zero8;
        }
        if constexpr (KACC) {
#pragma unroll
            for (int m = 0; m < C::MP; ++m)
#pragma unroll
                for (int n = 0; n < NT; ++n) {
                    tot[m][n] += acc[m][n];
                    acc[m][n] = s4_f32x4{0.f, 0.f, 0.f, 0.f};
                }
        }
        S4_PROBE(round * 4 + 3);
    }
    if constexpr (KACC) {
#pragma unroll
        for (int m = 0; m < C::MP; ++m)
#pragma unroll
            for (int n = 0; n < NT; ++n) acc[m][n] = tot[m][n];
    }
    S4_PROBE(58);
    if (C::KS > 1) {
        __syncthreads();
        if (kgrp > 0) {
            s4_f32x4 *red = reinterpret_cast<s4_f32x4 *>(smem_raw);
#pragma unroll
            for (int m = 0; m < C::MP; ++m)
#pragma unroll
                for (int n = 0; n < NT; ++n) red[((m * NT + n) * C::NW + wave) * 64 + lane] = acc[m][n];
        }
        __syncthreads();
        if (kgrp > 0) return;
#pragma unroll
        for (int k = 1; k < C::KS; ++k) {
            const s4_f32x4 *red = reinterpret_cast<const s4_f32x4 *>(smem_all + k * C::STAGES_BYTES);
#pragma unroll
            for (int m = 0; m < C::MP; ++m)
#pragma unroll
                for (int n = 0; n < NT; ++n) acc[m][n] += red[((m * NT + n) * C::NW + wave) * 64 + lane];
        }
    }

    {
        __builtin_amdgcn_s_waitcnt(0x0F70);
        const int g = lane >> 4, px = lane & 15;
        const size_t hw = (size_t)a.Hout * a.Wout;
        const size_t term = (size_t)a.dst_c4 * hw * 8;
        const bool mis = (a.dst_choff & 2) != 0;
        const float relu_lo = a.relu ? 0.f : -__builtin_inff();
        float vmax = 0.f;
        typedef split_x2 h2;
        auto store_px = [&](int co, size_t pix, s4_f32x4 v) {
            s4_h4 hi, mid;
            split_terms4(v, hi, mid);
            const int chb = a.dst_choff + co;
            const bool ok0 = chb < a.dst_limit, ok1 = chb + 2 < a.dst_limit;
            char *p = reinterpret_cast<char *>(a.dst) + (size_t)b * 2 * term + pix * 8 + (size_t)(chb >> 2) * hw * 8;
            if (!mis) {
                if (ok1) {
                    *reinterpret_cast<s4_h4 *>(p) = hi;
                    *reinterpret_cast<s4_h4 *>(p + term) = mid;
                } else if (ok0) {
                    *reinterpret_cast<h2 *>(p) = h2{hi[0], hi[1]};
                    *reinterpret_cast<h2 *>(p + term) = h2{mid[0], mid[1]};
                }
            } else {
                if (ok0) {
                    *reinterpret_cast<h2 *>(p + 4) = h2{hi[0], hi[1]};
                    *reinterpret_cast<h2 *>(p + 4 + term) = h2{mid[0], mid[1]};
                }
                if (ok1) {
                    *reinterpret_cast<h2 *>(p + hw * 8) = h2{hi[2], hi[3]};
                    *reinterpret_cast<h2 *>(p + hw * 8 + term) = h2{mid[2], mid[3]};
                }
            }
        };
#pragma unroll
        for (int m = 0; m < C::MP; ++m) {
            const int mt = wave * C::MP + m;
            const int oy = tileY * C::TH + mt / C::MTR;
            const int ox = tileX * C::TW + (mt % C::MTR) * 16 + px;
            if (oy >= a.Hout || ox >= a.Wout) continue;
            const size_t pix = (size_t)oy * a.Wout + ox;
#pragma unroll
            for (int n = 0; n < NT; ++n) {
                const int co = (tile0 + n) * 16 + 4 * g;
                if (co >= a.Cout + 2) continue;
                s4_f32x4 v = acc[m][n];
                const s4_f32x4 b4 = *reinterpret_cast<const s4_f32x4 *>(bias_lds + n * 16 + 4 * g);
#pragma unroll
                for (int r = 0; r < 4; ++r) v[r] = fmaxf(v[r] * a.acc_scale + b4[r], relu_lo);
                vmax = range_acc(vmax, v[0], v[1], v[2], v[3]);
                if (a.dst_fmt) {
                    store_px(co, pix, v);
                } else {
#pragma unroll
                    for (int r = 0; r < 4; ++r)
                        if (co + r < a.Cout) a.dst[((size_t)b * a.dst_ctotal + a.dst_choff + co + r) * hw + pix] = v[r];
                }
            }
        }
        range_commit(a.status, a.range_slot, vmax);
    }
    S4_PROBE(59);
#endif
}
```

### panoptic-forecasting_amd/csrc/conv_select.cpp

```cpp
#include "conv_mfma.h"

namespace pf {

ConvChoice g_conv_force = {0, 0, 0, 0};

namespace {
struct Tuned {
    int ks, cin, cout, hout, wout, B;
    ConvChoice c;
};
const Tuned kTuned[] = {
#include "conv_tuned.inc"
};

const Tuned kTunedS4[] = {
    {0, 0, 0, 0, 0, 0, {0, 0, 0, 0}},
#include "conv_s4_tuned.inc"
};

}

namespace {
bool measured_geometry(int ks, int cin, int cout, int hout, int wout, int B, int *ht, int *wt, double *b_eq, bool *exact) {
    const Tuned *first = nullptr;
    for (const Tuned &t : kTunedS4) {
        if (t.B <= 0 || t.ks != ks || t.cin != cin || t.cout != cout) continue;
        if (t.hout == hout && t.wout == wout) {
            *ht = hout;
            *wt = wout;
            *exact = true;
            *b_eq = (double)B;
            return true;
        }
        if (!first) first = &t;
    }
    if (!first) return false;
    *ht = first->hout;
    *wt = first->wout;
    *exact = false;
    *b_eq = (double)B * hout * wout / ((double)first->hout * first->wout);
    return *b_eq >= 0.5;
}
}

bool choose_s4(int ks, int cin, int cout, int hout, int wout, int B, ConvChoice *out) {
    int ht, wt;
    double b_eq;
    bool exact;
    if (!measured_geometry(ks, cin, cout, hout, wout, B, &ht, &wt, &b_eq, &exact)) return false;
    const Tuned *best = nullptr;
    double best_d = 0.0;
    for (const Tuned &t : kTunedS4) {
        if (t.ks != ks || t.cin != cin || t.cout != cout || t.hout != ht || t.wout != wt || t.B <= 0) continue;
        const double d = t.B > b_eq ? (double)t.B / b_eq : b_eq / (double)t.B;
        if (!best || d < best_d || (d == best_d && t.B > best->B)) { best = &t; best_d = d; }
    }
    if (!best) return false;
    *out = best->c;
    return true;
}

bool pair_wanted(int p_cin, int p_cout, int c_cin, int c_cout, int h, int w, int B, int mode) {
    if (mode == 4) return conv_pair_merged_supports(c_cout, p_cout);
    if (mode >= 2) return true;
    if (mode <= 0) return false;
    const long px = (long)B * h * w;
    return c_cout <= 32 && p_cout <= 16 && px >= 65536 && px <= 196608;
}

ConvChoice choose_conv(int ks, int stride, int cin, int cout, int hout, int wout, int B, int need, int use_tuned) {
    if (stride != 1) return ConvChoice{1, 0, 0, 0};
    int Bt = B, ht = hout, wt = wout;
    if (use_tuned) {
        double b_eq = (double)B;
        bool exact = true;
        if (!measured_geometry(ks, cin, cout, hout, wout, B, &ht, &wt, &b_eq, &exact)) { ht = hout; wt = wout; b_eq = (double)B; }
        const int measured[6] = {1, 2, 4, 8, 16, 32};
        Bt = measured[5];
        for (int m : measured)
            if ((double)m >= b_eq) { Bt = (m > 1 && (double)m != b_eq && b_eq * b_eq < (double)m * (m / 2)) ? m / 2 : m; break; }
    }
    for (const Tuned &t : kTuned)
        if (use_tuned && t.ks == ks && t.cin == cin && t.cout == cout && t.hout == ht && t.wout == wt && t.B == Bt &&
            (!(need & 2) || t.c.kind != 2 || t.c.p0 != 1))
            return t.c;
    if (ks == 3 && (need == 0) && (wout & 3) == 0 && (long)B * hout * wout >= 32768) {
        const int nt = cout <= 16 ? 1 : (cout <= 32 ? 2 : 3);
        const long tiles_wide = (long)B * ((hout + 7) / 8) * ((wout + 63) / 64) * (((cout + 15) / 16 + nt - 1) / nt);
        return ConvChoice{4, nt, (nt <= 2 && tiles_wide >= 512) ? 1 : 0, 0};
    }
    const long px = (long)B * hout * wout;
    if (px >= 131072 || (ks == 1 && px >= 32768)) return ConvChoice{1, 0, 0, 0};
    const int ntiles = (cout + 15) / 16;
    ConvChoice best{2, (need & 2) ? 2 : 1, 1, 8};
    long best_reuse = -1, best_waves = -1;
    const int mhs[3] = {4, 2, 1}, wks[3] = {2, 4, 8};
    for (int mh : mhs)
        for (int nt = 2; nt >= 1; --nt) {
            if ((need & 2) && mh == 1) continue;
            if (nt > ntiles) continue;
            for (int wk : wks) {
                if (wave_lds_bytes(ks, mh, nt, wk) > 64 * 1024) continue;
                const long waves = (long)B * ((hout + mh - 1) / mh) * ((wout + 15) / 16) * ((ntiles + nt - 1) / nt) * wk;
                const long reuse = waves >= 2048 ? mh * nt : 0;
                if (reuse > best_reuse || (reuse == best_reuse && reuse == 0 && waves > best_waves)) {
                    best = ConvChoice{2, mh, nt, wk};
                    best_reuse = reuse;
                    best_waves = waves;
                }
            }
        }
    return best;
}

}

static long long *g_probe_dev = nullptr;
namespace pf {
long long *probe_buffer() {
    if (!g_probe_dev) {
        if (hipMalloc((void **)&g_probe_dev, 64 * sizeof(long long)) != hipSuccess) return nullptr;
        (void)hipMemset(g_probe_dev, 0, 64 * sizeof(long long));
        (void)hipMemset(g_probe_dev + 60, 0xFF, sizeof(long long));
    }
    return g_probe_dev;
}
}

extern "C" int pf_debug_probe_read(long long *host64) {
    if (!g_probe_dev) return PF_EINVAL;
    if (hipMemcpy(host64, g_probe_dev, 64 * sizeof(long long), hipMemcpyDeviceToHost) != hipSuccess) return PF_EHIP;
    (void)hipMemset(g_probe_dev, 0, 64 * sizeof(long long));
    (void)hipMemset(g_probe_dev + 60, 0xFF, sizeof(long long));
    return PF_OK;
}

extern "C" int pf_debug_force_conv(int kind, int p0, int p1, int p2) {
    pf::g_conv_force = pf::ConvChoice{kind, p0, p1, p2};
    return PF_OK;
}
```

### panoptic-forecasting_amd/csrc/hardnet_plan.h

```cpp
#pragma once
#include <vector>

#include "conv_epilogue.h"
#include "net_kernels.h"
#include "pf_net.h"

struct ConvPlan {
    pf::ConvTiling tiling;
    size_t wpk_off = 0;
    size_t bias_off = 0;
    size_t raw_off = 0;
    size_t dep_off = 0;
    size_t oh_off = 0;
    size_t tiled_off = 0;
    int tiled_chunks = 0;
    size_t rem_off = 0;
    int rem_count = 0;
    size_t wave_off = 0;
    int wave_chunks = 0;
    size_t split_off = 0;
    int split_chunks = 0;
    size_t s4_off = 0;
    int s4_rounds = 0;
    bool s4_pad = false;
    size_t front_off = 0;
    float split_acc_scale = 1.0f;
    size_t pair_c_off = 0, pair_two_off = 0, pair_nine_off = 0;
    int pair_rounds = 0;
    bool pair_merged = false;
};

struct PlanOptions {
    int fuse_pool = 1, fuse_upsample = 1, valu_remainder = 1, split_f16 = 1, use_tuned_table = 1;
    int table_batch = 0;
    int fuse_front = 1;
    int range_guard = 1;
    int packed_acts = 1;
    int normalize_ranges = 1;
    int profile_tag_ops = 0;
    int fuse_pairs = 1;
};

struct pf_plan {
    pf::NetTable net;
    std::vector<ConvPlan> conv;
    std::vector<int> readers;
    float *dev_weights = nullptr;
    uint8_t *dev_lut = nullptr;
    size_t dev_floats = 0;
    PlanOptions opt;
    mutable std::vector<uint8_t> last_fmt;
    std::vector<std::vector<float>> chan_scale;
    std::vector<size_t> inv_scale_off;
    std::vector<uint8_t> feeds_conv;
};

namespace pf {

extern PlanOptions g_plan_opt;

constexpr size_t kStatusBytes = PF_WS_STATUS_BYTES;
constexpr int kStickyWord = PF_WS_STICKY_OFFSET / 4, kLiveWord = 2, kSlot0 = 16, kMaxSlots = ((int)(kStatusBytes / 4) - kSlot0) / 2;

int layout(const pf_plan *p, int B, int H, int W, std::vector<Dims> &d, std::vector<size_t> &off, size_t &total);

bool is_conv_pair(const NetTable &t, size_t i);

}
```

### panoptic-forecasting_amd/csrc/hardnet_plan.hip

```cpp
#include <cstdlib>
#include <cstring>

#include "hardnet_plan.h"
#include "pf_prof.h"

using namespace pf;

namespace {

enum StepKind : uint8_t {
    S_RANGE_CHECK, S_STEM, S_STEM_FRONT, S_PAIR, S_CONV, S_CONV_S4, S_CONV_GENERIC, S_CONV_SPLIT, S_CONV_SPLIT1, S_CONV_WAVE, S_CONV_DMA,
    S_POOL, S_UPSAMPLE, S_HEAD };
struct PlainArgs { const float *src; float *dst; int planes, hin, win, hout, wout; size_t n; unsigned *status, *slot; };
struct Step {
    StepKind kind;
    int op;
    char tag[96];
    int ci, need, sb, se;
    uint32_t src_t[kConvMaxSrc], dst_t;
    bool can_read, can_write, can_write_s4;
    ConvChoice ch;
    int nt, wide;
    union {
        ConvArgs c; PairArgs pair; PlainArgs x;
        struct { StemArgs stem; FrontArgs front; char front_tag[96]; } sf;
        struct { HeadArgs h; float *orig; size_t orig_bytes; } head;
    } u;
};
inline bool is_conv_step(StepKind k) { return k >= S_CONV_S4 && k <= S_CONV_DMA; }

int build_schedule(const pf_plan *p, const StemArgs *stem, const float *dense_x, int B, int H, int W, int out_h, int out_w,
                   void *out_seg, int out_seg_is_i64, float *out_logits, float *out_orig, void *ws, size_t ws_bytes,
                   std::vector<Step> &steps, std::vector<uint8_t> &fmt) {
    std::vector<Dims> d;
    std::vector<size_t> off;
    size_t ws_need = 0;
    int rc = layout(p, B, H, W, d, off, ws_need);
    if (rc) return rc;
    if (ws_bytes < ws_need) return fail(PF_EWORKSPACE, "workspace %zu B < required %zu B", ws_bytes, ws_need);
    const uint32_t input = p->net.ops[0].src[0].tensor;
    auto tptr = [&](uint32_t t) -> float * {
        return t == input ? const_cast<float *>(dense_x) : reinterpret_cast<float *>((char *)ws + off[t]);
    };

    const bool tags = (p->opt.profile_tag_ops != 0 || g_plan_opt.profile_tag_ops != 0) && prof_enabled();
    const bool fuse = p->opt.fuse_pool != 0;
    const int Bt = p->opt.table_batch > 0 ? p->opt.table_batch : B;
    unsigned *const st_words = reinterpret_cast<unsigned *>(ws);
    unsigned *const status_all = (p->opt.split_f16 && p->opt.range_guard) ? st_words + kLiveWord : nullptr;
    auto status_of = [&](uint32_t dst_t) -> unsigned * { return p->feeds_conv[dst_t] ? status_all : nullptr; };
    auto slot_of = [&](size_t op_i, uint32_t dst_t) -> unsigned * {
        return (status_all && p->feeds_conv[dst_t]) ? st_words + kSlot0 + op_i : nullptr;
    };

    const size_t nT = p->net.tensors.size();
    fmt.assign(nT, 0);
    std::vector<uint8_t> cand(nT, 1);
    std::vector<std::vector<uint8_t>> written(nT);
    for (size_t t = 0; t < nT; ++t) written[t].assign(p->net.tensors[t].channels + 8, 0);
    const bool s4_allowed = p->opt.packed_acts && p->opt.split_f16 && (g_conv_force.kind == 0 || g_conv_force.kind == 5);
    auto claim = [&](uint32_t t, int lo, int hi) -> int {
        std::vector<uint8_t> &wr = written[t];
        if ((lo & 3) == 2 && !wr[lo - 2]) cand[t] = 0;
        const int limit = ((hi & 3) != 0 && !wr[hi]) ? (hi + 3) / 4 * 4 : hi;
        for (int c = lo; c < hi; ++c) wr[c] = 1;
        return limit;
    };
    auto pin_fp32 = [&](const BlobOp &op) {
        for (uint32_t j = 0; j < op.n_src; ++j) cand[op.src[j].tensor] = 0;
        cand[op.dst] = 0;
    };

    steps.clear();
    steps.reserve(2 * p->net.ops.size());
    auto push = [&](StepKind kind, size_t i) -> Step & {
        Step &st = steps.emplace_back();
        memset(&st, 0, sizeof(st));
        st.kind = kind; st.op = (int)i;
        const BlobOp &o = p->net.ops[i];
        const Dims out = o.kind == OP_HEAD ? d[o.src[0].tensor] : d[o.dst];
        if (tags) snprintf(st.tag, sizeof(st.tag), "%02zu %s %u->%u %dx%d", i, p->net.tensors[o.dst].name, o.cin, o.cout, out.h, out.w);
        return st;
    };
    auto conv_step = [&](size_t i, size_t ci, const Dims &in, const Dims &out) -> Step & {
        Step &st = push(S_CONV, i);
        const BlobOp &o = p->net.ops[ci];
        ConvArgs &a = st.u.c;
        st.ci = (int)ci; st.dst_t = o.dst;
        a.n_src = (int)o.n_src;
        int c0 = 0;
        for (int j = 0; j < a.n_src; ++j) {
            a.src[j] = tptr((st.src_t[j] = o.src[j].tensor));
            a.src_ctotal[j] = (int)p->net.tensors[o.src[j].tensor].channels;
            a.src_choff[j] = (int)o.src[j].choff;
            a.src_cstart[j] = c0;
            c0 += (int)o.src[j].ch;
        }
        for (int j = a.n_src; j <= kConvMaxSrc; ++j) a.src_cstart[j] = c0;
        a.bias = p->dev_weights + p->conv[ci].bias_off;
        a.dst = tptr(o.dst);
        a.dst_ctotal = (int)p->net.tensors[o.dst].channels; a.dst_choff = (int)o.dst_choff;
        a.Cin = (int)o.cin; a.Cout = (int)o.cout;
        a.Hin = in.h; a.Win = in.w; a.Hout = out.h; a.Wout = out.w;
        a.relu = (int)o.relu;
        a.zero_page = p->dev_weights;
        a.ntiles = ((int)o.cout + 15) / 16;
        a.src_end = a.n_src;
        a.acc_scale = 1.0f;
        a.status = status_of(o.dst); a.range_slot = slot_of(ci, o.dst);
        return st;
    };
    auto choose = [&](Step &st, int need) {
        const BlobOp &o = p->net.ops[st.ci];
        const ConvPlan &cp = p->conv[st.ci];
        const ConvArgs &a = st.u.c;
        const bool generic = (a.Win & 3) != 0;
        ConvChoice ch{0, 0, 0, 0};
        if (!generic) {
            ch = choose_conv((int)o.k, (int)o.stride, a.Cin, a.Cout, a.Hout, a.Wout, Bt, need, p->opt.use_tuned_table);
            if (g_conv_force.kind == 2 && o.stride == 1) {
                ch = g_conv_force;
                if ((need & 2) && ch.p0 == 1) ch.p0 = 2;
            }
            if (g_conv_force.kind == 1) ch = g_conv_force;
            if (g_conv_force.kind == 4 && cp.split_off && (!need || o.k == 1)) ch = g_conv_force;
            if (ch.kind == 4 && (!cp.split_off || (need && o.k != 1) || !p->opt.split_f16)) ch = ConvChoice{1, 0, 0, 0};
            if (g_conv_force.kind == 5) ch = ConvChoice{1, 0, 0, 0};
        }
        st.ch = ch; st.need = need; st.sb = a.src_begin; st.se = a.src_end;
        const bool forced = g_conv_force.kind == 5;
        const long px = (long)Bt * a.Hout * a.Wout;
        bool want = ch.kind == 4 || (o.k == 1 && px >= 32768 && ch.kind == 1) || forced;
        st.nt = forced ? g_conv_force.p0 : (o.k == 1 ? 4 : (ch.kind == 4 ? ch.p0 : 2));
        st.wide = forced ? g_conv_force.p1 : (ch.kind == 4 ? ch.p1 : 0);
        ConvChoice s4c;
        if (!forced && !generic && p->opt.use_tuned_table && choose_s4((int)o.k, a.Cin, a.Cout, a.Hout, a.Wout, Bt, &s4c)) {
            want = s4c.kind == 5;
            if (want) { st.nt = s4c.p0; st.wide = s4c.p1; }
        }
        const int nt1 = st.nt < 1 ? 1 : (st.nt > a.ntiles ? a.ntiles : st.nt);
        const bool res_fits = !a.res || (size_t)nt1 * 16 * res_chan_stride(res_extent(8, a.res_sh), res_extent(32, a.res_sw)) * sizeof(float) <= 60 * 1024;
        st.can_read = s4_allowed && !generic && o.stride == 1 && o.kind == OP_CONV && cp.s4_off && (need == 0 || o.k == 1) && want &&
                      res_fits && ((a.src_begin == 0 && a.src_end == a.n_src) || cp.s4_pad);
        st.can_write_s4 = s4_allowed && !generic && (a.dst_choff & 1) == 0;
        st.can_write = st.can_write_s4 && (ch.kind == 1 || ch.kind == 4);
        st.u.c.dst_limit = claim(st.dst_t, a.dst_choff, a.dst_choff + a.Cout);
    };
    const bool fuse_up = p->opt.fuse_upsample != 0;
    auto can_commute_upsample = [&](size_t i, const Dims &in, const Dims &out) -> bool {
        if (!fuse || !fuse_up || i + 1 >= p->net.ops.size()) return false;
        const BlobOp &o = p->net.ops[i], &n = p->net.ops[i + 1];
        return n.kind == OP_CONV && n.k == 1 && n.stride == 1 && n.n_src == 2 && n.src[0].tensor == o.dst &&
               n.src[0].choff == 0 && n.src[0].ch == p->net.tensors[o.dst].channels && p->readers[o.dst] == 1 &&
               (in.w & 3) == 0 && (out.w & 3) == 0 && n.cout <= p->net.tensors[o.dst].channels &&
               2 * in.h <= out.h + 1 && 2 * in.w <= out.w + 1;
    };

    cand[input] = 0;
    for (size_t i = 0; i < p->net.ops.size(); ++i) {
        const BlobOp &o = p->net.ops[i];
        const Dims in = d[o.src[0].tensor];
        const Dims out = o.kind == OP_HEAD ? in : d[o.dst];
        if (o.kind == OP_STEM && stem) {
            StemArgs a = *stem;
            a.w = p->dev_weights + p->conv[i].raw_off; a.wdep = p->dev_weights + p->conv[i].dep_off;
            a.woh = p->conv[i].oh_off ? p->dev_weights + p->conv[i].oh_off : nullptr; a.bias = p->dev_weights + p->conv[i].bias_off;
            a.status = status_of(o.dst); a.range_slot = slot_of(i, o.dst);
            a.lut = p->dev_lut; a.dst = tptr(o.dst); a.Hout = out.h; a.Wout = out.w;
            bool front = false;
            if (s4_allowed && p->opt.fuse_front && i + 2 < p->net.ops.size()) {
                const BlobOp &n1 = p->net.ops[i + 1], &n2 = p->net.ops[i + 2];
                front = n1.kind == OP_CONV && n1.k == 3 && n1.stride == 1 && n1.n_src == 1 && n1.src[0].tensor == o.dst && n1.src[0].choff == 0 &&
                        n1.src[0].ch == p->net.tensors[o.dst].channels && n1.dst_choff == 0 && n1.cout == p->net.tensors[n1.dst].channels &&
                        p->readers[o.dst] == 1 && p->readers[n1.dst] == 1 && n1.relu && p->conv[i + 1].s4_off && p->conv[i + 1].s4_rounds == 2 &&
                        n2.kind == OP_CONV && n2.k == 3 && n2.stride == 2 && n2.n_src == 1 && n2.src[0].tensor == n1.dst && n2.src[0].choff == 0 &&
                        n2.src[0].ch == n1.cout && p->conv[i + 2].front_off && (n2.dst_choff & 3) == 0 &&
                        conv_front_supports((int)o.cout, (int)n1.cout, (int)n2.cout, out.h, out.w, (int)p->net.tensors[n2.dst].channels) && stem_writes_s4(a) && g_conv_force.kind == 0;
            }
            if (!front) {
                if (o.cout != 16 || o.k != 3 || o.stride != 2 || o.dst_choff != 0 ||
                    p->net.tensors[o.dst].channels != 16 || (uint32_t)(a.T * (a.n_cls + 1)) != o.cin)
                    return fail(PF_EUNSUPPORTED, "fused stem expects a 3x3/s2 conv %d->16, got %u->%u k%u s%u",
                                a.T * (a.n_cls + 1), o.cin, o.cout, o.k, o.stride);
                push(S_STEM, i).u.sf.stem = a;
                pin_fp32(o);
                continue;
            }
            const BlobOp &n1 = p->net.ops[i + 1], &n2 = p->net.ops[i + 2];
            const Dims o2 = d[n2.dst];
            cand[o.dst] = 0; cand[n1.dst] = 0;
            Step &st = push(S_STEM_FRONT, i);
            st.u.sf.stem = a; st.u.sf.stem.dst_fmt = 1;
            FrontArgs &f = st.u.sf.front;
            f.x = tptr(o.dst);
            f.w1 = p->dev_weights + p->conv[i + 1].s4_off; f.w2 = p->dev_weights + p->conv[i + 2].front_off;
            f.bias1 = p->dev_weights + p->conv[i + 1].bias_off; f.bias2 = p->dev_weights + p->conv[i + 2].bias_off;
            f.scale1 = p->conv[i + 1].split_acc_scale; f.scale2 = p->conv[i + 2].split_acc_scale;
            f.dst = tptr(n2.dst);
            f.dst_ctotal = (int)p->net.tensors[n2.dst].channels; f.dst_c4 = (f.dst_ctotal + 3) / 4; f.dst_choff = (int)n2.dst_choff;
            f.dst_limit = claim(n2.dst, f.dst_choff, f.dst_choff + (int)n2.cout);
            f.H1 = out.h; f.W1 = out.w; f.H2 = o2.h; f.W2 = o2.w;
            f.C1 = (int)n1.cout; f.C2 = (int)n2.cout; f.relu1 = (int)n1.relu; f.relu2 = (int)n2.relu;
            f.status = status_all;
            f.range_slot_mid = slot_of(i + 1, n1.dst); f.range_slot = slot_of(i + 2, n2.dst);
            st.dst_t = n2.dst; st.can_write = st.can_write_s4 = true;
            if (tags)
                snprintf(st.u.sf.front_tag, sizeof(st.u.sf.front_tag), "%02zu+%02zu %s+%s %u->%u->%u %dx%d", i + 1, i + 2, p->net.tensors[n1.dst].name,
                         p->net.tensors[n2.dst].name, o.cout, n1.cout, n2.cout, o2.h, o2.w);
            i += 2;
        } else if (o.kind == OP_STEM || o.kind == OP_CONV) {
            if (o.src[0].tensor == input && !dense_x)
                return fail(PF_EINVAL, "network input is consumed by a generic conv: use pf_hardnet_forward_dense");
            if (o.src[0].tensor == input && status_all) {
                PlainArgs &x = push(S_RANGE_CHECK, i).u.x;
                x.src = dense_x; x.n = (size_t)B * p->net.tensors[input].channels * in.h * in.w;
                x.status = status_all; x.slot = st_words + kSlot0 + kMaxSlots - 1;
            }
            const BlobOp *pool = nullptr;
            if (fuse && i + 1 < p->net.ops.size() && p->net.ops[i + 1].kind == OP_POOL && o.stride == 1 && o.k == 1 && (in.w & 3) == 0 &&
                p->net.ops[i + 1].src[0].tensor == o.dst && o.dst_choff == 0 && o.cout == p->net.tensors[o.dst].channels &&
                p->readers[o.dst] == 1 && out.h >= 2 && out.w >= 2)
                pool = &p->net.ops[i + 1];
            Step &st = conv_step(i, i, in, out);
            if (pool) {
                ConvArgs &a = st.u.c;
                a.pool = 1; a.dst = tptr(pool->dst); a.dst_ctotal = (int)p->net.tensors[pool->dst].channels;
                st.dst_t = pool->dst;
                a.status = status_of(pool->dst); a.range_slot = slot_of(i, pool->dst);
                ++i;
            }
            choose(st, pool ? 2 : 0);
        } else if (o.kind == OP_UPSAMPLE && can_commute_upsample(i, in, out)) {
            const BlobOp &n = p->net.ops[i + 1];
            const Dims hi = out;
            cand[o.dst] = 0;
            auto tag_half = [&](Step &st, const char *half, int cin, const Dims &dd) {
                if (tags)
                    snprintf(st.tag, sizeof(st.tag), "%02zu%c %s.%s %d->%u %dx%d", i + 1, half[0] == 'l' ? 'a' : 'b', p->net.tensors[n.dst].name,
                             half, cin, n.cout, dd.h, dd.w);
            };
            Step &ls = conv_step(i, i + 1, in, in);
            ConvArgs &lo = ls.u.c;
            lo.src[0] = tptr(o.src[0].tensor);
            ls.src_t[0] = o.src[0].tensor;
            lo.src_ctotal[0] = (int)p->net.tensors[o.src[0].tensor].channels; lo.src_choff[0] = (int)o.src[0].choff;
            lo.dst = tptr(o.dst);
            ls.dst_t = o.dst;
            lo.dst_ctotal = (int)n.cout; lo.dst_choff = 0;
            lo.relu = 0; lo.no_bias = 1;
            lo.status = nullptr; lo.range_slot = nullptr;
            lo.Cin = (int)n.src[0].ch;
            lo.src_end = 1;
            tag_half(ls, "lo", lo.Cin, in);
            choose(ls, 4);
            Step &hs = conv_step(i, i + 1, hi, hi);
            ConvArgs &ha = hs.u.c;
            ha.Cin = (int)n.src[1].ch;
            ha.src_begin = 1; ha.src_end = 2;
            tag_half(hs, "hi", ha.Cin, hi);
            ha.res = tptr(o.dst); ha.res_ctotal = (int)n.cout;
            ha.Hres = in.h; ha.Wres = in.w;
            ha.res_sh = hi.h > 1 ? (float)(in.h - 1) / (float)(hi.h - 1) : 0.f;
            ha.res_sw = hi.w > 1 ? (float)(in.w - 1) / (float)(hi.w - 1) : 0.f;
            choose(hs, 4);
            ++i;
        } else if (o.kind == OP_HEAD) {
            pin_fp32(o);
            Step &st = push(S_HEAD, i);
            HeadArgs &a = st.u.head.h;
            a.logits = tptr(o.src[0].tensor);
            a.out_seg = out_seg; a.out_logits = out_logits; a.out_is_i64 = out_seg_is_i64;
            a.B = B; a.C = (int)o.cin; a.Hin = in.h; a.Win = in.w; a.Hout = out_h; a.Wout = out_w;
            st.u.head.orig = out_orig; st.u.head.orig_bytes = (size_t)B * a.C * in.h * in.w * sizeof(float);
        } else {
            pin_fp32(o);
            PlainArgs &x = push(o.kind == OP_POOL ? S_POOL : S_UPSAMPLE, i).u.x;
            x.src = tptr(o.src[0].tensor); x.dst = tptr(o.dst); x.planes = B * (int)o.cin;
            x.hin = in.h; x.win = in.w; x.hout = out.h; x.wout = out.w;
            x.status = status_of(o.dst); x.slot = slot_of(i, o.dst);
        }
    }

    if (!s4_allowed) std::fill(cand.begin(), cand.end(), 0);
    for (bool changed = true; changed;) {
        changed = false;
        for (const Step &r : steps) {
            if (r.kind != S_CONV && r.kind != S_STEM_FRONT) continue;
            bool all = r.can_read;
            for (int j = r.sb; j < r.se; ++j) all = all && cand[r.src_t[j]];
            if (!all)
                for (int j = r.sb; j < r.se; ++j)
                    if (cand[r.src_t[j]]) { cand[r.src_t[j]] = 0; changed = true; }
            if (!(r.can_write || (all && r.can_write_s4)) && cand[r.dst_t]) { cand[r.dst_t] = 0; changed = true; }
        }
    }
    std::vector<uint8_t> read_s4(nT, 0);
    for (const Step &r : steps)
        if (r.kind == S_CONV)
            for (int j = r.sb; j < r.se; ++j) read_s4[r.src_t[j]] = 1;
    for (size_t t = 0; t < nT; ++t) fmt[t] = cand[t] && read_s4[t];

    for (Step &st : steps) {
        if (st.kind == S_STEM_FRONT) {
            st.u.sf.front.dst_fmt = fmt[st.dst_t];
            fmt[p->net.ops[st.op].dst] = 1;
            fmt[p->net.ops[st.op + 1].dst] = 0xFF;
        }
        if (st.kind != S_CONV) continue;
        const BlobOp &o = p->net.ops[st.ci];
        const ConvPlan &cp = p->conv[st.ci];
        ConvArgs &a = st.u.c;
        a.dst_fmt = fmt[st.dst_t]; a.dst_c4 = (a.dst_ctotal + 3) / 4;
        bool s4 = st.can_read;
        for (int j = st.sb; j < st.se; ++j) s4 = s4 && fmt[st.src_t[j]];
        if (s4) {
            const int per = o.k == 3 ? 2 : 8;
            int e = 0;
            for (int j = 0; j < a.n_src; ++j) {
                const int ch0 = a.src_choff[j], chn = a.src_cstart[j + 1] - a.src_cstart[j];
                a.src_c4[j] = (a.src_ctotal[j] + 3) / 4;
                a.src_g0[j] = ch0 / 4;
                a.src_gn[j] = (ch0 + chn + 3) / 4 - ch0 / 4;
                a.src_ent0[j] = e;
                e += cp.s4_pad ? (a.src_gn[j] + per - 1) / per * per : a.src_gn[j];
            }
            for (int j = a.n_src; j <= kConvMaxSrc; ++j) a.src_ent0[j] = e;
            a.src_fmt = 1; a.acc_scale = cp.split_acc_scale;
            a.wpk = p->dev_weights + cp.s4_off; a.nchunks = cp.s4_rounds;
            a.chunk_begin = a.src_ent0[a.src_begin] / per;
            a.chunk_end = (a.src_ent0[a.src_end] + per - 1) / per;
            st.kind = S_CONV_S4; continue;
        }
        if ((a.Win & 3) != 0) {
            if (st.need) return fail(PF_EUNSUPPORTED, "fused conv on a width that is not a multiple of 4");
            a.wpk = p->dev_weights + cp.wpk_off; a.nchunks = cp.tiling.nchunks;
            st.kind = S_CONV_GENERIC; continue;
        }
        auto use = [&](size_t wpk_off, int nchunks, int kc) {
            a.wpk = p->dev_weights + wpk_off;
            a.nchunks = nchunks;
            a.src_chunk0[0] = 0;
            for (int j = 0; j < kConvMaxSrc; ++j)
                a.src_chunk0[j + 1] = a.src_chunk0[j] + (j < a.n_src ? ((int)o.src[j].ch + kc - 1) / kc : 0);
            a.chunk_begin = a.src_chunk0[a.src_begin];
            a.chunk_end = a.src_chunk0[a.src_end];
        };
        ConvChoice &ch = st.ch;
        if (ch.kind == 4) {
            use(cp.split_off, cp.split_chunks, o.k == 1 ? 32 : 8);
            a.acc_scale = cp.split_acc_scale;
            st.kind = o.k == 1 ? S_CONV_SPLIT1 : S_CONV_SPLIT;
            if (o.k == 1 ? conv_split1_supported(a, ch.p0) : conv_split_supported(a)) continue;
            ch = ConvChoice{1, 0, 0, 0};
        }
        if (ch.kind == 2) {
            use(cp.wave_off, cp.wave_chunks, wave_kc((int)o.k));
            ch.p1 = ch.p1 < a.ntiles ? ch.p1 : a.ntiles;
            st.kind = S_CONV_WAVE;
            if (conv_wave_supported(a, (int)o.k, ch.p0, ch.p1, ch.p2)) continue;
            ch = ConvChoice{1, 0, 0, 0};
        }
        use(cp.tiled_off, cp.tiled_chunks, dma_kc((int)o.k, (int)o.stride));
        st.kind = S_CONV_DMA;
        int wm, nt;
        if (p->opt.valu_remainder && cp.rem_off && !st.need && !a.dst_fmt && a.src_begin == 0 && a.src_end == a.n_src && (ch.p0 == 0 || ch.p0 == 4)) {
            ConvArgs r = a;
            r.rem = cp.rem_count;
            r.wrem = p->dev_weights + cp.rem_off;
            r.ntiles = ((int)o.cout - r.rem) / 16;
            if (conv_dma_supported(r, (int)o.k, (int)o.stride, B, 4, ch.p0 == 4 && ch.p1 > 0 ? ch.p1 : 0, p->opt.table_batch, &wm, &nt)) {
                a = r;
                ch = ConvChoice{1, wm, nt, 0};
                continue;
            }
        }
        conv_dma_supported(a, (int)o.k, (int)o.stride, B, ch.p0, ch.p1, p->opt.table_batch, &wm, &nt);
        ch = ConvChoice{1, wm, nt, 0};
    }

    size_t w = 0;
    for (size_t k = 0; k < steps.size(); ++k, ++w) {
        const size_t i = (size_t)steps[k].op;
        const bool pair = p->opt.fuse_pairs && k + 1 < steps.size() && steps[k].kind == S_CONV_S4 && steps[k + 1].kind == S_CONV_S4 &&
                          steps[k + 1].op == (int)i + 1 && is_conv_pair(p->net, i) && p->conv[i + 1].pair_c_off && steps[k].u.c.dst_fmt && steps[k + 1].u.c.dst_fmt;
        const BlobOp &o = p->net.ops[i];
        if (!pair || !pair_wanted((int)o.cin, (int)o.cout, (int)p->net.ops[i + 1].cin, (int)p->net.ops[i + 1].cout, d[o.dst].h, d[o.dst].w, Bt,
                                  p->opt.fuse_pairs)) {
            if (w != k) steps[w] = steps[k];
            continue;
        }
        const BlobOp &C = p->net.ops[i + 1];
        Step st = steps[k + 1];
        st.kind = S_PAIR; st.op = (int)i;
        if (tags)
            snprintf(st.tag, sizeof(st.tag), "%02zu+%02zu %s+%s %u->%u->%u %dx%d", i, i + 1, p->net.tensors[o.dst].name, p->net.tensors[C.dst].name, o.cin,
                     o.cout, C.cout, d[o.dst].h, d[o.dst].w);
        PairArgs &pa = st.u.pair;
        ConvArgs &a = pa.c;
        const int n = (int)C.n_src;
        int e = 0;
        for (int j = 0; j < n; ++j) {
            const BlobSrc &sj = C.src[(j + 1) % n];
            const bool isP = j == n - 1;
            a.src[j] = tptr(sj.tensor);
            a.src_ctotal[j] = (int)p->net.tensors[sj.tensor].channels;
            a.src_choff[j] = (int)sj.choff;
            a.src_c4[j] = (a.src_ctotal[j] + 3) / 4;
            a.src_g0[j] = isP ? 0 : (int)sj.choff / 4;
            a.src_gn[j] = isP ? ((int)sj.ch + 3) / 4 : ((int)sj.choff + (int)sj.ch + 3) / 4 - (int)sj.choff / 4;
            a.src_ent0[j] = e;
            e += (a.src_gn[j] + 1) / 2 * 2;
        }
        for (int j = n; j <= kConvMaxSrc; ++j) a.src_ent0[j] = e;
        a.chunk_begin = a.chunk_end = 0;
        a.wpk = p->dev_weights + p->conv[i + 1].pair_c_off; a.nchunks = p->conv[i + 1].pair_rounds;
        pa.p_wpk = p->dev_weights + p->conv[i + 1].pair_two_off; pa.p_w9 = p->dev_weights + p->conv[i + 1].pair_nine_off;
        pa.p_bias = p->dev_weights + p->conv[i].bias_off; pa.p_acc_scale = p->conv[i].split_acc_scale;
        pa.p_dst = tptr(o.dst); pa.p_dst_c4 = ((int)p->net.tensors[o.dst].channels + 3) / 4;
        pa.p_dst_choff = (int)o.dst_choff; pa.p_dst_limit = steps[k].u.c.dst_limit;
        pa.p_cout = (int)o.cout; pa.p_cin = (int)o.cin; pa.p_ntiles = ((int)o.cout + 15) / 16; pa.p_relu = (int)o.relu;
        pa.p_range_slot = slot_of(i, o.dst);
        pa.rounds_s = a.src_ent0[1] / 2; pa.round_d = a.src_ent0[n - 1] / 2;
        pa.merged = p->conv[i + 1].pair_merged && p->opt.fuse_pairs != 3;
        steps[w] = st;
        ++k;
    }
    steps.resize(w);
    return PF_OK;
}

int run_net(const pf_plan *p, const StemArgs *stem, const float *dense_x, int B, int H, int W, int out_h, int out_w,
            void *out_seg, int out_seg_is_i64, float *out_logits, float *out_orig, void *ws, size_t ws_bytes,
            hipStream_t s) {
    std::vector<Step> steps;
    std::vector<uint8_t> fmt;
    int rc = build_schedule(p, stem, dense_x, B, H, W, out_h, out_w, out_seg, out_seg_is_i64, out_logits, out_orig, ws, ws_bytes, steps, fmt);
    if (rc) return rc;
    p->last_fmt = fmt;
    static const bool sync_ops = ab_env("PF_SYNC_OPS") != nullptr;
    static const bool probe_on = ab_env("PF_PROBE") != nullptr;
    long long *const probe = probe_on ? probe_buffer() : nullptr;
    for (size_t k = 0; k < steps.size(); ++k) {
        Step &st = steps[k];
        if (sync_ops && (k == 0 || steps[k - 1].op != st.op))
            fprintf(stderr, "[pf] before op %d (%s): %s\n", st.op, p->net.tensors[p->net.ops[st.op].dst].name, hipGetErrorString(hipStreamSynchronize(s)));
        else if (sync_ops && is_conv_step(steps[k - 1].kind) && steps[k - 1].u.c.no_bias)
            fprintf(stderr, "[pf]   low-resolution half: %s\n", hipGetErrorString(hipStreamSynchronize(s)));
        if (st.tag[0]) prof_set_tag(st.tag);
        const BlobOp &o = p->net.ops[st.ci];
        ConvArgs &a = st.u.c;
        const PlainArgs &x = st.u.x;
        if (is_conv_step(st.kind)) a.probe = probe;
        switch (st.kind) {
            case S_RANGE_CHECK: rc = launch_range_check(x.src, x.n, x.status, x.slot, s); break;
            case S_STEM: st.u.sf.stem.probe = probe; rc = launch_stem(st.u.sf.stem, s); break;
            case S_STEM_FRONT:
                if ((rc = launch_stem(st.u.sf.stem, s))) break;
                if (st.u.sf.front_tag[0]) prof_set_tag(st.u.sf.front_tag);
                st.u.sf.front.probe = probe; rc = launch_conv_front(st.u.sf.front, B, s); break;
            case S_PAIR: st.u.pair.c.probe = probe; rc = launch_conv_pair(st.u.pair, B, s); break;
            case S_CONV_S4: rc = launch_conv_s4(a, (int)o.k, st.nt, st.wide, B, s); break;
            case S_CONV_GENERIC: rc = launch_conv(a, p->conv[st.ci].tiling, B, s); break;
            case S_CONV_SPLIT: rc = launch_conv_split(a, st.ch.p0, st.ch.p1, B, s); break;
            case S_CONV_SPLIT1: rc = launch_conv_split1(a, st.ch.p0, B, s); break;
            case S_CONV_WAVE: rc = launch_conv_wave(a, (int)o.k, st.ch.p0, st.ch.p1, st.ch.p2, B, s); break;
            case S_CONV_DMA: rc = launch_conv_dma(a, (int)o.k, (int)o.stride, B, s, st.ch.p0, st.ch.p1, p->opt.table_batch); break;
            case S_POOL: rc = launch_avgpool2(x.src, x.dst, x.planes, x.hin, x.win, x.status, x.slot, s); break;
            case S_UPSAMPLE: rc = launch_upsample(x.src, x.dst, x.planes, x.hin, x.win, x.hout, x.wout, x.status, x.slot, s); break;
            case S_HEAD:
                if (st.u.head.orig && (rc = launch_copy(st.u.head.orig, st.u.head.h.logits, st.u.head.orig_bytes, s))) break;
                rc = launch_head(st.u.head.h, s); break;
            case S_CONV: break;
        }
        if (rc) return rc;
    }
    if (p->opt.profile_tag_ops != 0 || g_plan_opt.profile_tag_ops != 0) prof_set_tag(nullptr);
    return launch_range_finalize(reinterpret_cast<unsigned *>(ws), kLiveWord, kSlot0, kMaxSlots, kStickyWord, s);
}

}

extern "C" int pf_bg_forward(const pf_plan *p, const void *seg, int seg_is_i64, const float *depth,
                             const uint8_t *depth_mask, float depth_mean, float depth_std, int hop_flags,
                             float min_depth, float max_depth, int B, int T, int H, int W, int out_h, int out_w,
                             void *out_seg, int out_seg_is_i64, float *out_logits, float *out_orig_logits, void *ws,
                             size_t ws_bytes, void *stream) {
    if (!p || !seg || !depth || !out_seg || !ws) return fail(PF_EINVAL, "pf_bg_forward: null pointer argument");
    if (!depth_mask && !(hop_flags & PF_HOP_DEPTH_U16))
        return fail(PF_EINVAL, "pf_bg_forward: depth_mask is required unless PF_HOP_DEPTH_U16 is set");
    if (B <= 0 || T <= 0 || H <= 0 || W <= 0 || out_h <= 0 || out_w <= 0)
        return fail(PF_EINVAL, "pf_bg_forward: bad dims");
    if (p->net.ops.empty() || p->net.ops[0].kind != OP_STEM)
        return fail(PF_EUNSUPPORTED, "pf_bg_forward: plan does not start with a fused stem");
    StemArgs st;
    memset(&st, 0, sizeof(st));
    st.seg = seg; st.depth = depth; st.mask = depth_mask;
    st.depth_mean = depth_mean; st.depth_std = depth_std; st.min_depth = min_depth; st.max_depth = max_depth;
    st.seg_is_i64 = seg_is_i64; st.hop = hop_flags; st.B = B; st.T = T; st.n_cls = (int)p->net.hdr.n_cls;
    st.H = H; st.W = W;
    return run_net(p, &st, nullptr, B, H, W, out_h, out_w, out_seg, out_seg_is_i64, out_logits, out_orig_logits, ws,
                   ws_bytes, (hipStream_t)stream);
}

extern "C" int pf_hardnet_forward_dense(const pf_plan *p, const float *x, int B, int H, int W, int out_h, int out_w,
                                        void *out_seg, int out_seg_is_i64, float *out_logits, float *out_orig_logits,
                                        void *ws, size_t ws_bytes, void *stream) {
    if (!p || !x || !ws) return fail(PF_EINVAL, "pf_hardnet_forward_dense: null pointer argument");
    if (B <= 0 || H <= 0 || W <= 0) return fail(PF_EINVAL, "pf_hardnet_forward_dense: bad dims");
    const bool has_head = !p->net.ops.empty() && p->net.ops.back().kind == OP_HEAD;
    if (has_head && (!out_seg || out_h <= 0 || out_w <= 0))
        return fail(PF_EINVAL, "pf_hardnet_forward_dense: out_seg/out size required");
    return run_net(p, nullptr, x, B, H, W, out_h, out_w, out_seg, out_seg_is_i64, out_logits, out_orig_logits, ws,
                   ws_bytes, (hipStream_t)stream);
}
```

### panoptic-forecasting_amd/csrc/plan_access.hip

```cpp
#include <cstring>

#include "hardnet_plan.h"

using namespace pf;

int pf::layout(const pf_plan *p, int B, int H, int W, std::vector<Dims> &d, std::vector<size_t> &off, size_t &total) {
    int rc = propagate_dims(p->net, H, W, d);
    if (rc) return rc;
    off.assign(p->net.tensors.size(), (size_t)-1);
    size_t cur = kStatusBytes;
    const uint32_t input = p->net.ops[0].src[0].tensor;
    for (size_t t = 0; t < p->net.tensors.size(); ++t) {
        if (t == input || d[t].h == 0) continue;
        off[t] = cur;
        cur += align_up((size_t)B * ((p->net.tensors[t].channels + 3) / 4 * 4) * d[t].h * d[t].w * sizeof(float), 256);
    }
    total = cur;
    return PF_OK;
}

extern "C" int pf_hardnet_workspace(const pf_plan *p, int B, int H, int W, size_t *bytes) {
    if (!p || !bytes || B <= 0 || H <= 0 || W <= 0) return fail(PF_EINVAL, "pf_hardnet_workspace: bad argument");
    std::vector<Dims> d;
    std::vector<size_t> off;
    return layout(p, B, H, W, d, off, *bytes);
}

extern "C" int pf_hardnet_status(const void *ws, unsigned *status, void *stream) {
    if (!ws || !status) return fail(PF_EINVAL, "pf_hardnet_status: null argument");
    PF_HIP_CHECK(hipMemcpyAsync(status, ws, sizeof(unsigned), hipMemcpyDeviceToHost, (hipStream_t)stream));
    PF_HIP_CHECK(hipStreamSynchronize((hipStream_t)stream));
    return PF_OK;
}

extern "C" int pf_hardnet_status_sticky(void *ws, unsigned *status, int clear, void *stream) {
    if (!ws || !status) return fail(PF_EINVAL, "pf_hardnet_status_sticky: null argument");
    char *w = (char *)ws + PF_WS_STICKY_OFFSET;
    PF_HIP_CHECK(hipMemcpyAsync(status, w, sizeof(unsigned), hipMemcpyDeviceToHost, (hipStream_t)stream));
    if (clear) {
        int rc = launch_zero_fill(w, sizeof(unsigned), (hipStream_t)stream);
        if (rc) return rc;
    }
    PF_HIP_CHECK(hipStreamSynchronize((hipStream_t)stream));
    return PF_OK;
}

extern "C" int pf_hardnet_status_reset(void *ws, void *stream) {
    if (!ws) return fail(PF_EINVAL, "pf_hardnet_status_reset: null argument");
    return launch_zero_fill(ws, PF_WS_STATUS_BYTES, (hipStream_t)stream);
}

extern "C" int pf_hardnet_range_maxima(const pf_plan *p, const void *ws, float *maxima, int cap, int *n_ops, void *stream) {
    if (!p || !ws || !maxima || !n_ops) return fail(PF_EINVAL, "pf_hardnet_range_maxima: null argument");
    *n_ops = (int)p->net.ops.size();
    if (cap < *n_ops) return fail(PF_EINVAL, "pf_hardnet_range_maxima: room for %d values, the plan has %d ops", cap, *n_ops);
    PF_HIP_CHECK(hipMemcpyAsync(maxima, (const char *)ws + (kSlot0 + kMaxSlots) * 4, p->net.ops.size() * sizeof(float), hipMemcpyDeviceToHost, (hipStream_t)stream));
    PF_HIP_CHECK(hipStreamSynchronize((hipStream_t)stream));
    return PF_OK;
}

extern "C" int pf_hardnet_tensor_view(const pf_plan *p, const char *name, int B, int H, int W, size_t *ws_offset,
                                      int *channels, int *h, int *w) {
    if (!p || !name || !ws_offset || !channels || !h || !w) return fail(PF_EINVAL, "pf_hardnet_tensor_view: null");
    std::vector<Dims> d;
    std::vector<size_t> off;
    size_t total;
    int rc = layout(p, B, H, W, d, off, total);
    if (rc) return rc;
    for (size_t t = 0; t < p->net.tensors.size(); ++t) {
        if (strncmp(p->net.tensors[t].name, name, sizeof(p->net.tensors[t].name)) == 0) {
            if (off[t] == (size_t)-1) return fail(PF_EINVAL, "tensor '%s' is not materialised", name);
            *ws_offset = off[t];
            *channels = (int)p->net.tensors[t].channels;
            *h = d[t].h;
            *w = d[t].w;
            return PF_OK;
        }
    }
    return fail(PF_EINVAL, "no tensor named '%s'", name);
}

__global__ void unscale_channels_kernel(float *x, const float *inv_scale, int C, size_t hw, size_t n) {
    for (size_t i = (size_t)blockIdx.x * blockDim.x + threadIdx.x; i < n; i += (size_t)gridDim.x * blockDim.x)
        x[i] *= inv_scale[(i / hw) % C];
}

extern "C" int pf_hardnet_tensor_read(const pf_plan *p, const char *name, int B, int H, int W, const void *ws, float *dst,
                                      void *stream) {
    if (!p || !name || !ws || !dst) return fail(PF_EINVAL, "pf_hardnet_tensor_read: null");
    size_t off;
    int c, h, w;
    int rc = pf_hardnet_tensor_view(p, name, B, H, W, &off, &c, &h, &w);
    if (rc) return rc;
    size_t t = 0;
    while (strncmp(p->net.tensors[t].name, name, sizeof(p->net.tensors[t].name)) != 0) ++t;
    const char *src = (const char *)ws + off;
    if (t < p->last_fmt.size() && p->last_fmt[t] == 0xFF)
        return fail(PF_EUNSUPPORTED, "tensor '%s' was elided by the fused front end (never stored); set plan option fuse_front = 0 to tap it", name);
    if (t < p->last_fmt.size() && p->last_fmt[t]) {
        if ((rc = launch_s4_unpack(src, dst, B, c, h, w, (hipStream_t)stream))) return rc;
    } else {
        int rc = launch_copy(dst, src, (size_t)B * c * h * w * sizeof(float), (hipStream_t)stream);
        if (rc) return rc;
    }
    if (p->inv_scale_off[t]) {
        const size_t n = (size_t)B * c * h * w;
        hipLaunchKernelGGL(unscale_channels_kernel, dim3((unsigned)((n + 255) / 256 < 4096 ? (n + 255) / 256 : 4096)), dim3(256), 0, (hipStream_t)stream,
                           dst, p->dev_weights + p->inv_scale_off[t], c, (size_t)h * w, n);
        PF_LAUNCH_CHECK("unscale_channels_kernel");
    }
    return PF_OK;
}

extern "C" int pf_s4_pack(const float *src, void *dst, int B, int C, int H, int W, unsigned *status, void *stream) {
    if (!src || !dst || B <= 0 || C <= 0 || H <= 0 || W <= 0) return fail(PF_EINVAL, "pf_s4_pack: bad argument");
    return launch_s4_pack(src, dst, B, C, H, W, status, (hipStream_t)stream);
}
extern "C" int pf_s4_unpack(const void *src, float *dst, int B, int C, int H, int W, void *stream) {
    if (!src || !dst || B <= 0 || C <= 0 || H <= 0 || W <= 0) return fail(PF_EINVAL, "pf_s4_unpack: bad argument");
    return launch_s4_unpack(src, dst, B, C, H, W, (hipStream_t)stream);
}

extern "C" int pf_hardnet_flops(const pf_plan *p, int H, int W, double *flops) {
    if (!p || !flops) return fail(PF_EINVAL, "pf_hardnet_flops: null");
    std::vector<Dims> d;
    int rc = propagate_dims(p->net, H, W, d);
    if (rc) return rc;
    double f = 0;
    for (const BlobOp &o : p->net.ops)
        if (o.kind == OP_STEM || o.kind == OP_CONV)
            f += 2.0 * o.cout * d[o.dst].h * d[o.dst].w * o.cin * o.k * o.k;
    *flops = f;
    return PF_OK;
}
```

### panoptic-forecasting_amd/csrc/plan_create.hip

```cpp
#include <algorithm>
#include <cmath>
#include <cstring>

#include "hardnet_plan.h"

using namespace pf;

namespace pf {
PlanOptions g_plan_opt;
extern int g_opt_train_side, g_opt_wgrad_taps, g_opt_train_s4, g_opt_train_kacc, g_opt_train_table_batch, g_opt_up_two_pass;
}

namespace {

struct Option {
    const char *name, *alias;
    int PlanOptions::*member;
    int *global;
    bool process, per_plan, clamp0;
};
const Option kOptions[] = {
    {"fuse_pool", nullptr, &PlanOptions::fuse_pool, nullptr, true, true, false},
    {"fuse_upsample", nullptr, &PlanOptions::fuse_upsample, nullptr, true, true, false},
    {"use_tuned_table", nullptr, &PlanOptions::use_tuned_table, nullptr, true, true, false},
    {"valu_remainder", nullptr, &PlanOptions::valu_remainder, nullptr, true, true, false},
    {"split_f16", "split_bf16", &PlanOptions::split_f16, nullptr, true, true, false},
    {"packed_acts", nullptr, &PlanOptions::packed_acts, nullptr, true, true, false},
    {"range_guard", nullptr, &PlanOptions::range_guard, nullptr, true, true, false},
    {"fuse_front", nullptr, &PlanOptions::fuse_front, nullptr, true, true, false},
    {"fuse_pairs", nullptr, &PlanOptions::fuse_pairs, nullptr, true, true, false},
    {"profile_tag_ops", nullptr, &PlanOptions::profile_tag_ops, nullptr, true, true, false},
    {"table_batch", nullptr, &PlanOptions::table_batch, nullptr, false, true, true},
    {"normalize_ranges", nullptr, &PlanOptions::normalize_ranges, nullptr, true, false, false},
    {"train_side_stream", nullptr, nullptr, &g_opt_train_side, true, false, false},
    {"wgrad_taps", nullptr, nullptr, &g_opt_wgrad_taps, true, false, false},
    {"train_forward_s4", nullptr, nullptr, &g_opt_train_s4, true, false, false},
    {"train_blocked_sum", nullptr, nullptr, &g_opt_train_kacc, true, false, false},
    {"train_table_batch", nullptr, nullptr, &g_opt_train_table_batch, true, false, true},
    {"upsample_bwd_two_pass", nullptr, nullptr, &g_opt_up_two_pass, true, false, false},
};

int set_option(const char *who, PlanOptions *plan, const char *name, int value) {
    for (const Option &o : kOptions) {
        if (strcmp(name, o.name) != 0 && !(o.alias && !strcmp(name, o.alias))) continue;
        if (!(plan ? o.per_plan : o.process)) break;
        if (o.clamp0 && value < 0) value = 0;
        *(o.member ? &((plan ? *plan : g_plan_opt).*o.member) : o.global) = value;
        return PF_OK;
    }
    return fail(PF_EINVAL, "%s: unknown option '%s'", who, name);
}

}

extern "C" int pf_set_option(const char *name, int value) {
    if (!name) return fail(PF_EINVAL, "pf_set_option: null name");
    return set_option("pf_set_option", nullptr, name, value);
}

extern "C" int pf_hardnet_plan_set_option(pf_plan *p, const char *name, int value) {
    if (!p || !name) return fail(PF_EINVAL, "pf_hardnet_plan_set_option: null argument");
    return set_option("pf_hardnet_plan_set_option", &p->opt, name, value);
}

bool pf::is_conv_pair(const NetTable &t, size_t i) {
    if (i + 1 >= t.ops.size()) return false;
    const BlobOp &P = t.ops[i], &C = t.ops[i + 1];
    if (P.kind != OP_CONV || C.kind != OP_CONV || P.k != 3 || C.k != 3 || P.stride != 1 || C.stride != 1) return false;
    if (P.n_src != 1 || C.n_src < 2 || (P.dst_choff & 1) || (C.dst_choff & 1)) return false;
    if (C.src[0].tensor != P.dst || C.src[0].choff != P.dst_choff || C.src[0].ch != P.cout) return false;
    if (C.src[1].tensor != P.src[0].tensor || C.src[1].choff != P.src[0].choff || C.src[1].ch != P.src[0].ch) return false;
    for (uint32_t j = 0; j < C.n_src; ++j)
        if (C.src[j].choff & 1) return false;
    return conv_pair_supports((int)C.cout, (int)P.cout);
}

static void fill_lut(uint8_t *lut) {
    memset(lut, 0, 256);
    for (int i = 0; i < 34; ++i) lut[i] = 255;
    const int ids[19] = {7, 8, 11, 12, 13, 17, 19, 20, 21, 22, 23, 24, 25, 26, 27, 28, 31, 32, 33};
    for (int t = 0; t < 19; ++t) lut[ids[t]] = (uint8_t)t;
}

static void normalize_ranges(pf_plan *p, std::vector<float> &w) {
    const size_t nT = p->net.tensors.size();
    p->chan_scale.assign(nT, std::vector<float>());
    std::vector<std::vector<double>> est(nT);
    for (size_t t = 0; t < nT; ++t) {
        p->chan_scale[t].assign(p->net.tensors[t].channels, 1.0f);
        est[t].assign(p->net.tensors[t].channels, 1.0);
    }
    p->feeds_conv.assign(nT, 0);
    for (size_t i = p->net.ops.size(); i-- > 0;) {
        const BlobOp &o = p->net.ops[i];
        if (o.kind == OP_STEM || o.kind == OP_CONV)
            for (uint32_t j = 0; j < o.n_src; ++j) p->feeds_conv[o.src[j].tensor] = 1;
        else if ((o.kind == OP_POOL || o.kind == OP_UPSAMPLE) && p->feeds_conv[o.dst])
            p->feeds_conv[o.src[0].tensor] = 1;
    }
    std::vector<uint8_t> pinned(nT, 0), read(nT, 0);
    for (const BlobOp &o : p->net.ops) {
        for (uint32_t j = 0; j < (o.kind == OP_UPSAMPLE ? 1u : o.n_src); ++j) read[o.src[j].tensor] = 1;
        if (o.kind == OP_HEAD) pinned[o.src[0].tensor] = 1;
    }
    for (size_t t = 0; t < nT; ++t) pinned[t] = pinned[t] || !read[t] || !p->feeds_conv[t];
    if (p->net.ops.empty()) return;
    const uint32_t input = p->net.ops[0].src[0].tensor;
    pinned[input] = 1;
    if (p->net.ops[0].kind == OP_STEM && p->net.hdr.n_cls > 0) {
        const uint32_t C = p->net.tensors[input].channels, T = C / (p->net.hdr.n_cls + 1);
        if (T * (p->net.hdr.n_cls + 1) == C)
            for (uint32_t c = 0; c < T * p->net.hdr.n_cls; ++c) est[input][c] = std::sqrt(1.0 / p->net.hdr.n_cls);
    }
    for (size_t i = p->net.ops.size(); i-- > 0;) {
        const BlobOp &o = p->net.ops[i];
        if ((o.kind == OP_POOL || o.kind == OP_UPSAMPLE) && pinned[o.dst]) pinned[o.src[0].tensor] = 1;
    }
    for (const BlobOp &o : p->net.ops) {
        if (o.kind == OP_POOL || o.kind == OP_UPSAMPLE) {
            for (uint32_t c = 0; c < o.src[0].ch; ++c) {
                p->chan_scale[o.dst][o.dst_choff + c] = p->chan_scale[o.src[0].tensor][o.src[0].choff + c];
                est[o.dst][o.dst_choff + c] = est[o.src[0].tensor][o.src[0].choff + c];
            }
            continue;
        }
        if (o.kind != OP_STEM && o.kind != OP_CONV) continue;
        const size_t kk = (size_t)o.k * o.k;
        std::vector<double> e_in(o.cin);
        std::vector<float> s_in(o.cin);
        uint32_t k0 = 0;
        for (uint32_t j = 0; j < o.n_src; ++j)
            for (uint32_t c = 0; c < o.src[j].ch; ++c, ++k0) {
                e_in[k0] = est[o.src[j].tensor][o.src[j].choff + c];
                s_in[k0] = p->chan_scale[o.src[j].tensor][o.src[j].choff + c];
            }
        for (uint32_t co = 0; co < o.cout; ++co) {
            float *wr = w.data() + o.w_off + (size_t)co * o.cin * kk;
            float &b = w[o.b_off + co];
            double var = (double)b * b;
            for (uint32_t k = 0; k < o.cin; ++k) {
                double ss = 0;
                for (size_t q = 0; q < kk; ++q) ss += (double)wr[k * kk + q] * wr[k * kk + q];
                var += ss * e_in[k] * e_in[k];
            }
            double e = std::sqrt(var);
            if (o.relu) e *= 0.70710678118654752;
            float s_out = 1.0f;
            if (p->opt.normalize_ranges && !pinned[o.dst] && e > 0 && std::isfinite(e)) {
                int ex = (int)std::lround(std::log2((double)kRangeTarget / e));
                ex = ex < -60 ? -60 : (ex > 60 ? 60 : ex);
                s_out = std::ldexp(1.0f, ex);
            }
            for (uint32_t k = 0; k < o.cin; ++k) {
                const float f = s_out / s_in[k];
                if (f != 1.0f)
                    for (size_t q = 0; q < kk; ++q) wr[k * kk + q] *= f;
            }
            b *= s_out;
            p->chan_scale[o.dst][o.dst_choff + co] = s_out;
            est[o.dst][o.dst_choff + co] = e;
        }
    }
}

namespace {

struct Arena {
    std::vector<float> &f;
    size_t take(size_t n_floats, size_t align = 1) {
        f.resize(align_up(f.size(), align), 0.f);
        f.resize(f.size() + n_floats);
        return f.size() - n_floats;
    }
    float *at(size_t off) { return f.data() + off; }
};

void pack_generic(const BlobOp &o, const float *w, const float *bias, Arena &a, ConvPlan &c) {
    c.tiling = choose_tiling((int)o.k, (int)o.stride, (int)o.cin, (int)o.cout, 0);
    c.wpk_off = a.take(c.tiling.packed_floats());
    pack_conv_weights(w, (int)o.cin, (int)o.cout, c.tiling, a.at(c.wpk_off));
    c.bias_off = a.take((size_t)c.tiling.cout_blocks * c.tiling.nt * 16);
    memcpy(a.at(c.bias_off), bias, o.cout * sizeof(float));
}

void pack_dma(const BlobOp &o, const float *w, const int *src_ch, Arena &a, ConvPlan &c) {
    const int kc = dma_kc((int)o.k, (int)o.stride);
    c.tiled_chunks = dma_chunks(src_ch, (int)o.n_src, (int)o.k, (int)o.stride);
    c.tiled_off = a.take((size_t)((o.cout + 15) / 16) * c.tiled_chunks * (kc / 4) * o.k * o.k * 64);
    pack_conv_weights_tiled(w, (int)o.cin, (int)o.cout, (int)o.k, kc, src_ch, (int)o.n_src, a.at(c.tiled_off));
    constexpr int valu_max = 8;
    const int split = (o.k == 3 && o.stride == 1) ? dma_valu_split((int)o.cout) : 0;
    if (split > 0 && split <= valu_max) {
        c.rem_count = split;
        c.rem_off = a.take((size_t)c.tiled_chunks * (kc / 4) * 9 * dma_rem_rv(split) * 4, 4);
        pack_conv_weights_rem(w, (int)o.cin, (int)o.cout, split, 3, kc, src_ch, (int)o.n_src, a.at(c.rem_off));
    }
}

float scale_weights(const float *w, size_t n, std::vector<float> &ws) {
    const float sc = split_weight_scale(w, n);
    ws.resize(n);
    for (size_t q = 0; q < n; ++q) ws[q] = w[q] * sc;
    return sc;
}

void pack_split(const BlobOp &o, const float *ws, const int *src_ch, Arena &a, ConvPlan &c) {
    if (o.k == 3) {
        c.split_chunks = split_chunks(src_ch, (int)o.n_src);
        c.split_off = a.take(split_packed_floats(src_ch, (int)o.n_src, (int)o.cout), 16);
        pack_conv_weights_split(ws, (int)o.cin, (int)o.cout, src_ch, (int)o.n_src, a.at(c.split_off));
    } else {
        c.split_chunks = split1_chunks(src_ch, (int)o.n_src);
        c.split_off = a.take(split1_packed_floats(src_ch, (int)o.n_src, (int)o.cout), 16);
        pack_conv_weights_split1(ws, (int)o.cin, (int)o.cout, src_ch, (int)o.n_src, a.at(c.split_off));
    }
}

void pack_s4(const BlobOp &o, const float *ws, Arena &a, ConvPlan &c) {
    S4Range rg[kConvMaxSrc];
    for (uint32_t j = 0; j < o.n_src; ++j) {
        rg[j] = S4Range{(int)o.src[j].choff, (int)o.src[j].ch};
        if (o.src[j].choff & 1) return;
    }
    c.s4_pad = o.k == 1 && o.n_src == 2;
    c.s4_rounds = s4_rounds(rg, (int)o.n_src, (int)o.k, c.s4_pad);
    c.s4_off = a.take(s4_packed_floats(rg, (int)o.n_src, (int)o.cout, (int)o.k, c.s4_pad), 16);
    pack_conv_weights_s4(ws, (int)o.cin, (int)o.cout, (int)o.k, rg, (int)o.n_src, c.s4_pad, a.at(c.s4_off));
}

void pack_pair(const BlobOp &P, const float *wP, const BlobOp &o, const float *ws, Arena &a, ConvPlan &c) {
    const int n = (int)o.n_src;
    S4Range rg[kConvMaxSrc];
    int cstart[kConvMaxSrc], c0s[kConvMaxSrc], acc0 = 0;
    for (int j = 0; j < n; ++j) { c0s[j] = acc0; acc0 += (int)o.src[j].ch; }
    for (int j = 0; j < n; ++j) {
        const int sj = (j + 1) % n;
        rg[j] = sj == 0 ? S4Range{0, (int)o.src[0].ch} : S4Range{(int)o.src[sj].choff, (int)o.src[sj].ch};
        cstart[j] = c0s[sj];
    }
    c.pair_rounds = s4_rounds(rg, n, 3, 1);
    c.pair_c_off = a.take(s4_packed_floats(rg, n, (int)o.cout, 3, 1), 16);
    std::vector<float> wp;
    scale_weights(wP, (size_t)P.cout * P.cin * 9, wp);
    c.pair_merged = conv_pair_merged_supports((int)o.cout, (int)P.cout);
    if (c.pair_merged) {
        const int nt = ((int)o.cout + 15) / 16, row0 = ((int)o.cout + 3) / 4 * 4, cS = c0s[1 % n];
        std::vector<float> waug((size_t)nt * 16 * o.cin * 9, 0.f);
        std::copy(ws, ws + (size_t)o.cout * o.cin * 9, waug.begin());
        for (int pc = 0; pc < (int)P.cout; ++pc)
            for (int ci = 0; ci < (int)P.cin; ++ci)
                for (int t = 0; t < 9; ++t) waug[((size_t)(row0 + pc) * o.cin + cS + ci) * 9 + t] = wp[((size_t)pc * P.cin + ci) * 9 + t];
        pack_conv_weights_s4_ex(waug.data(), (int)o.cin, nt * 16, 3, rg, cstart, n, 1, a.at(c.pair_c_off));
    } else {
        pack_conv_weights_s4_ex(ws, (int)o.cin, (int)o.cout, 3, rg, cstart, n, 1, a.at(c.pair_c_off));
    }
    const S4Range rs{(int)P.src[0].choff, (int)P.src[0].ch};
    c.pair_two_off = a.take(pair_p_two_floats(rs, (int)P.cout), 16);
    c.pair_nine_off = a.take(pair_p_nine_floats(rs, (int)P.cout), 16);
    pack_conv_weights_pair_p(wp.data(), (int)P.cin, (int)P.cout, rs, a.at(c.pair_two_off), a.at(c.pair_nine_off));
}

void pack_front(const BlobOp &o, const float *ws, Arena &a, ConvPlan &c) {
    const S4Range rg{(int)o.src[0].choff, (int)o.src[0].ch};
    c.front_off = a.take(s4_packed_floats(&rg, 1, (int)o.cout, 3, 0), 16);
    pack_conv_weights_s4(ws, (int)o.cin, (int)o.cout, 3, &rg, 1, 0, a.at(c.front_off));
}

void pack_wave(const BlobOp &o, const float *w, const int *src_ch, Arena &a, ConvPlan &c) {
    c.wave_chunks = wave_chunks(src_ch, (int)o.n_src, (int)o.k);
    c.wave_off = a.take(wave_packed_floats(src_ch, (int)o.n_src, (int)o.cout, (int)o.k));
    pack_conv_weights_wave(w, (int)o.cin, (int)o.cout, (int)o.k, src_ch, (int)o.n_src, a.at(c.wave_off));
}

void pack_stem(const BlobOp &o, const float *w, int n_cls, Arena &a, ConvPlan &c) {
    const int ks2 = (int)(o.k * o.k);
    c.raw_off = a.take((size_t)o.cout * o.cin * ks2);
    memcpy(a.at(c.raw_off), w, (size_t)o.cout * o.cin * ks2 * sizeof(float));
    const int T = (int)o.cin / (n_cls + 1);
    if (T < 1 || (uint32_t)(T * (n_cls + 1)) != o.cin || o.cout != 16) return;
    c.dep_off = a.take((size_t)ks2 * T * 16, 16);
    float *q = a.at(c.dep_off);
    for (int tap = 0; tap < ks2; ++tap)
        for (int t = 0; t < T; ++t)
            for (int co = 0; co < 16; ++co) *q++ = w[((size_t)co * o.cin + T * n_cls + t) * ks2 + tap];
    c.oh_off = a.take((size_t)ks2 * T * (n_cls + 1) * 16, 16);
    q = a.at(c.oh_off);
    for (int tap = 0; tap < ks2; ++tap)
        for (int t = 0; t < T; ++t)
            for (int r = 0; r <= n_cls; ++r)
                for (int co = 0; co < 16; ++co) *q++ = r < n_cls ? w[((size_t)co * o.cin + t * n_cls + r) * ks2 + tap] : 0.f;
}

int build_plan_weights(pf_plan &p, const float *wts, std::vector<float> &host) {
    host.assign(64, 0.f);
    Arena a{host};
    const std::vector<BlobOp> &ops = p.net.ops;
    p.conv.assign(ops.size(), ConvPlan());
    for (size_t i = 0; i < ops.size(); ++i) {
        const BlobOp &o = ops[i];
        if (o.kind != OP_STEM && o.kind != OP_CONV) continue;
        if (o.k == 1 && o.stride != 1) return fail(PF_EUNSUPPORTED, "1x1 conv with stride %u", o.stride);
        ConvPlan &c = p.conv[i];
        const float *w = wts + o.w_off, *ws = w;
        int src_ch[kConvMaxSrc];
        for (uint32_t j = 0; j < o.n_src; ++j) src_ch[j] = (int)o.src[j].ch;
        pack_generic(o, w, wts + o.b_off, a, c);
        pack_dma(o, w, src_ch, a, c);
        std::vector<float> wsc;
        if (o.stride == 1 || o.n_src == 1) {
            c.split_acc_scale = 1.0f / scale_weights(w, (size_t)o.cout * o.cin * o.k * o.k, wsc);
            ws = wsc.data();
        }
        if (o.stride == 1) pack_split(o, ws, src_ch, a, c);
        if (o.stride == 1 && o.kind == OP_CONV) pack_s4(o, ws, a, c);
        if (i > 0 && is_conv_pair(p.net, i - 1)) pack_pair(ops[i - 1], wts + ops[i - 1].w_off, o, ws, a, c);
        if (o.k == 3 && o.stride == 2 && o.kind == OP_CONV && o.n_src == 1 && (o.src[0].choff & 3) == 0 && o.cout <= 32) pack_front(o, ws, a, c);
        if (o.stride == 1) pack_wave(o, w, src_ch, a, c);
        if (o.kind == OP_STEM) pack_stem(o, w, (int)p.net.hdr.n_cls, a, c);
        a.take(0, 64);
    }
    p.inv_scale_off.assign(p.net.tensors.size(), 0);
    for (size_t t = 0; t < p.net.tensors.size(); ++t) {
        bool any = false;
        for (float v : p.chan_scale[t]) any = any || v != 1.0f;
        if (!any) continue;
        p.inv_scale_off[t] = a.take(p.chan_scale[t].size());
        for (size_t ch = 0; ch < p.chan_scale[t].size(); ++ch) host[p.inv_scale_off[t] + ch] = 1.0f / p.chan_scale[t][ch];
        a.take(0, 64);
    }
    return PF_OK;
}

int check_plan_ops(const NetTable &t, size_t n_w) {
    for (size_t i = 0; i < t.ops.size(); ++i) {
        const BlobOp &o = t.ops[i];
        uint32_t cin = 0;
        for (uint32_t j = 0; j < o.n_src; ++j) cin += o.src[j].ch;
        bool ok = true;
        if (o.kind == OP_STEM || o.kind == OP_CONV)
            ok = cin == o.cin && o.dst_choff + o.cout <= t.tensors[o.dst].channels && (o.k == 1 || o.k == 3) &&
                 (o.stride == 1 || o.stride == 2) && o.w_off + (uint64_t)o.cout * o.cin * o.k * o.k <= n_w && o.b_off + o.cout <= n_w;
        if (o.kind == OP_POOL || o.kind == OP_UPSAMPLE) ok = o.src[0].ch <= t.tensors[o.dst].channels;
        if (!ok) return fail(PF_EBLOB, "op %zu is inconsistent with the tensor table", i);
    }
    return PF_OK;
}

}

extern "C" int pf_hardnet_plan_create(const void *blob, size_t bytes, int in_ch, int n_cls, pf_plan **out) {
    if (!blob || !out) return fail(PF_EINVAL, "pf_hardnet_plan_create: null argument");
    pf_plan *p = new pf_plan();
    p->opt = g_plan_opt;
    int rc = parse_net_table(blob, bytes, in_ch, n_cls, p->net);
    if ((int)p->net.ops.size() >= kMaxSlots - 1)
        rc = fail(PF_EUNSUPPORTED, "op table of %zu ops: the status block has %d per-op words", p->net.ops.size(), kMaxSlots - 1);
    const size_t n_w = rc ? 0 : (bytes - p->net.hdr.weights_off) / sizeof(float);
    if (!rc) rc = check_plan_ops(p->net, n_w);
    std::vector<float> wnorm, host;
    if (!rc) {
        const float *w0 = reinterpret_cast<const float *>((const char *)blob + p->net.hdr.weights_off);
        wnorm.assign(w0, w0 + n_w);
        normalize_ranges(p, wnorm);
        rc = build_plan_weights(*p, wnorm.data(), host);
    }
    if (rc) {
        delete p;
        return rc;
    }
    p->readers.assign(p->net.tensors.size(), 0);
    for (const BlobOp &o : p->net.ops)
        for (uint32_t j = 0; j < o.n_src; ++j) p->readers[o.src[j].tensor]++;
    p->dev_floats = host.size();
    uint8_t lut[256];
    fill_lut(lut);
    hipError_t e = hipMalloc((void **)&p->dev_weights, (host.size() + 64) * sizeof(float));
    if (e == hipSuccess) e = hipMalloc((void **)&p->dev_lut, 256);
    if (e == hipSuccess) e = hipMemcpy(p->dev_weights, host.data(), host.size() * sizeof(float), hipMemcpyHostToDevice);
    if (e == hipSuccess) e = hipMemcpy(p->dev_lut, lut, 256, hipMemcpyHostToDevice);
    if (e != hipSuccess) {
        pf_hardnet_plan_destroy(p);
        return fail(PF_EHIP, "plan upload: %s", hipGetErrorString(e));
    }
    *out = p;
    return PF_OK;
}

extern "C" void pf_hardnet_plan_destroy(pf_plan *p) {
    if (!p) return;
    if (p->dev_weights) (void)hipFree(p->dev_weights);
    if (p->dev_lut) (void)hipFree(p->dev_lut);
    delete p;
}
```

### panoptic-forecasting_amd/lib.py

```python
import ctypes
import os

_HERE = os.path.dirname(os.path.abspath(__file__))
LIB_PATH = os.environ.get('PF_LIBPFHIP') or os.path.join(_HERE, 'csrc', 'libpfhip.so')

_c = ctypes
_vp, _i, _f, _sz = _c.c_void_p, _c.c_int, _c.c_float, _c.c_size_t

SIGNATURES = {
    'pf_version': (_i, []),
    'pf_last_error': (_c.c_char_p, []),
    'pf_warp_splat_workspace': (_i, [_i, _i, _i, _i, _i, _c.POINTER(_sz)]),
    'pf_warp_splat': (_i, [_vp, _vp, _vp, _i, _vp, _vp, _vp, _vp, _vp, _i, _i, _i, _i, _i, _i, _i,
                           _vp, _vp, _vp, _vp, _sz, _vp]),
    'pf_hardnet_plan_create': (_i, [_vp, _sz, _i, _i, _c.POINTER(_vp)]),
    'pf_hardnet_plan_destroy': (None, [_vp]),
    'pf_hardnet_workspace': (_i, [_vp, _i, _i, _i, _c.POINTER(_sz)]),
    'pf_bg_forward': (_i, [_vp, _vp, _i, _vp, _vp, _f, _f, _i, _f, _f, _i, _i, _i, _i, _i, _i,
                           _vp, _i, _vp, _vp, _vp, _sz, _vp]),
    'pf_hardnet_forward_dense': (_i, [_vp, _vp, _i, _i, _i, _i, _i, _vp, _i, _vp, _vp, _vp, _sz, _vp]),
    'pf_hardnet_tensor_view': (_i, [_vp, _c.c_char_p, _i, _i, _i, _c.POINTER(_sz), _c.POINTER(_i),
                                    _c.POINTER(_i), _c.POINTER(_i)]),
    'pf_hardnet_tensor_read': (_i, [_vp, _c.c_char_p, _i, _i, _i, _vp, _vp, _vp]),
    'pf_hardnet_status': (_i, [_vp, _c.POINTER(_c.c_uint), _vp]),
    'pf_hardnet_status_sticky': (_i, [_vp, _c.POINTER(_c.c_uint), _i, _vp]),
    'pf_hardnet_status_reset': (_i, [_vp, _vp]),
    'pf_hardnet_range_maxima': (_i, [_vp, _vp, _vp, _i, _c.POINTER(_i), _vp]),
    'pf_s4_pack': (_i, [_vp, _vp, _i, _i, _i, _i, _vp, _vp]),
    'pf_s4_unpack': (_i, [_vp, _vp, _i, _i, _i, _i, _vp]),
    'pf_hardnet_flops': (_i, [_vp, _i, _i, _c.POINTER(_c.c_double)]),
    'pf_hop_export': (_i, [_vp, _i, _i, _vp, _sz, _vp, _vp, _vp]),
    'pf_hop_load': (_i, [_vp, _sz, _f, _f, _vp, _vp, _vp]),
    'pf_panoptic_merge_workspace': (_i, [_i, _c.POINTER(_sz)]),
    'pf_panoptic_merge': (_i, [_vp, _i, _vp, _vp, _vp, _i, _i, _vp, _i, _vp, _vp, _vp, _i, _i, _i, _i, _i, _i, _i,
                               _vp, _i, _vp, _sz, _vp]),
    'pf_panoptic_encode': (_i, [_vp, _i, _i, _i, _i, _i, _vp, _vp, _vp, _vp]),
    'pf_panoptic_max_ids': (_i, []),
    'pf_bg_dense_input': (_i, [_vp, _i, _i, _vp, _vp, _f, _f, _i, _i, _i, _i, _vp, _vp]),
    'pf_seg_loss_workspace': (_i, [_i, _i, _i, _c.POINTER(_sz)]),
    'pf_seg_loss': (_i, [_vp, _i, _i, _i, _i, _vp, _i, _i, _i, _i, _vp, _vp, _sz, _vp]),
    'pf_train_create': (_i, [_vp, _sz, _i, _i, _c.POINTER(_vp)]),
    'pf_train_destroy': (None, [_vp]),
    'pf_train_autotune': (_i, [_vp, _i]),
    'pf_train_tuned_shapes': (_i, [_vp, _c.POINTER(_i), _i, _c.POINTER(_i)]),
    'pf_train_path_stats': (_i, [_vp, _c.POINTER(_i), _i, _c.POINTER(_i)]),
    'pf_train_param_count': (_i, [_vp, _c.POINTER(_sz)]),
    'pf_train_param_layout': (_i, [_vp, _i, _c.POINTER(_sz), _c.POINTER(_sz), _c.POINTER(_i)]),
    'pf_train_workspace': (_i, [_vp, _i, _i, _i, _i, _i, _c.POINTER(_sz)]),
    'pf_train_forward_backward': (_i, [_vp, _vp, _vp, _i, _vp, _i, _vp, _vp, _f, _f, _i, _vp, _i, _i, _i, _vp, _i, _i, _i, _i, _f, _f,
                                       _f, _i, _vp, _vp, _sz, _vp]),
    'pf_train_tensor_view': (_i, [_vp, _c.c_char_p, _i, _i, _i, _i, _i, _i, _c.POINTER(_sz), _c.POINTER(_i), _c.POINTER(_i),
                                  _c.POINTER(_i)]),
    'pf_sgd_workspace': (_i, [_c.POINTER(_sz)]),
    'pf_sgd_step': (_i, [_vp, _vp, _vp, _vp, _sz, _f, _f, _f, _f, _f, _i, _vp, _sz, _vp]),
    'pf_fg_weights_size': (_i, [_i, _c.POINTER(_sz), _c.POINTER(_sz)]),
    'pf_fg_pack': (_i, [_vp, _vp, _i, _vp]),
    'pf_fg_workspace': (_i, [_i, _i, _i, _i, _c.POINTER(_sz)]),
    'pf_fg_forward': (_i, [_vp, _i, _i, _i, _i, _i, _vp, _vp, _vp, _vp, _vp, _vp, _vp, _vp, _vp, _vp, _vp, _vp, _vp, _vp,
                           _vp, _sz, _vp]),
    'pf_odom_weights_size': (_i, [_i, _c.POINTER(_sz), _c.POINTER(_sz)]),
    'pf_odom_pack': (_i, [_vp, _vp, _i, _vp]),
    'pf_odom_forward': (_i, [_vp, _i, _i, _i, _i, _vp, _vp, _vp, _vp]),
    'pf_set_option': (_i, [_c.c_char_p, _i]),
    'pf_hardnet_plan_set_option': (_i, [_vp, _c.c_char_p, _i]),
    'pf_debug_force_conv': (_i, [_i, _i, _i, _i]),
    'pf_debug_probe_read': (_i, [_c.POINTER(_c.c_longlong)]),
    'pf_profile_enable': (_i, [_i]),
    'pf_profile_collect': (_i, []),
    'pf_profile_get': (_i, [_i, _c.c_char_p, _sz, _c.POINTER(_i), _c.POINTER(_c.c_double),
                            _c.POINTER(_c.c_double), _c.POINTER(_c.c_double)]),
}


def profile(enable):
    check(load().pf_profile_enable(int(enable)), 'pf_profile_enable')


def profile_results():
    L = load()
    n = L.pf_profile_collect()
    if n < 0:
        check(n, 'pf_profile_collect')
    out = []
    for i in range(n):
        buf = ctypes.create_string_buffer(160)
        la, ms, fl, by = _i(), _c.c_double(), _c.c_double(), _c.c_double()
        check(L.pf_profile_get(i, buf, 160, ctypes.byref(la), ctypes.byref(ms), ctypes.byref(fl), ctypes.byref(by)),
              'pf_profile_get')
        out.append({'label': buf.value.decode(), 'launches': la.value, 'ms': ms.value, 'flops': fl.value,
                    'bytes': by.value})
    return out

_lib = None


class PfError(RuntimeError):
    pass


def load():
    global _lib
    if _lib is None:
        import torch
        if not os.path.exists(LIB_PATH):
            raise PfError('%s not found: build it with `python -c "import __graft_entry__ as g; g.build()"` '
                          '(make -C panoptic-forecasting_amd/csrc). There is no fallback path.' % LIB_PATH)
        lib = ctypes.CDLL(LIB_PATH)
        for name, (res, args) in SIGNATURES.items():
            fn = getattr(lib, name)
            fn.restype, fn.argtypes = res, args
        _lib = lib
    return _lib


def check(rc, what):
    if rc != 0:
        raise PfError('%s failed (%d): %s' % (what, rc, load().pf_last_error().decode()))


def require_cuda(t, name):
    if not t.is_cuda:
        raise PfError('%s must live on the GPU (got %s): the HIP path has no CPU fallback' % (name, t.device))
    if not t.is_contiguous():
        raise PfError('%s must be contiguous' % name)
    return t


def stream_ptr():
    import torch
    return ctypes.c_void_p(torch.cuda.current_stream().cuda_stream)
```

Measured before the change: 2846 frames/s.

## Share input reads between adjacent HarDNet convs by computing partial sums in producer kernel

For adjacent conv pairs where the second conv consumes the first conv's input as one of its sources, the first conv now also computes the second conv's contribution from that shared input. It stores those partial sums to a workspace scratch tensor. The second conv then skips that source and adds the stored partials in its epilogue. This removes a second read of the large shared input and the matching MFMA work, at the cost of extra scratch traffic and more weight packing. A heuristic limits it to a specific channel shape (10→18, cin≥48, large pixel count).

```diff
diff --git a/include/pfhip.h b/include/pfhip.h
--- a/include/pfhip.h
+++ b/include/pfhip.h
@@ -129,6 +129,8 @@
                    double *bytes);
 
 int pf_debug_force_conv(int kind, int p0, int p1, int p2);
+int pf_debug_plan_arena(const void *blob, size_t bytes, int in_ch, int n_cls, float *out, size_t cap, size_t *n_floats,
+                        long long *table, int table_ops);
 int pf_debug_probe_read(long long *host64);
 
 #ifdef __cplusplus
diff --git a/panoptic-forecasting_amd/bg_model.py b/panoptic-forecasting_amd/bg_model.py
--- a/panoptic-forecasting_amd/bg_model.py
+++ b/panoptic-forecasting_amd/bg_model.py
@@ -14,7 +14,7 @@
 
 PLAN_OPTIONS = {'split_f16': 'split_f16', 'split_bf16': 'split_f16', 'fuse_pool': 'fuse_pool', 'fuse_upsample': 'fuse_upsample',
                 'use_tuned_table': 'use_tuned_table', 'valu_remainder': 'valu_remainder', 'conv_table_batch': 'table_batch',
-                'range_guard': 'range_guard', 'fuse_front': 'fuse_front', 'fuse_pairs': 'fuse_pairs'}
+                'range_guard': 'range_guard', 'fuse_front': 'fuse_front', 'fuse_pairs': 'fuse_pairs', 'share_s': 'share_s'}
 PF_STATUS_RANGE, PF_STATUS_RANGE_LOW = 1, 2
 PF_STATUS_ANY = PF_STATUS_RANGE | PF_STATUS_RANGE_LOW
 PF_WS_STATUS_BYTES = 2048
diff --git a/panoptic-forecasting_amd/csrc/conv_mfma.h b/panoptic-forecasting_amd/csrc/conv_mfma.h
--- a/panoptic-forecasting_amd/csrc/conv_mfma.h
+++ b/panoptic-forecasting_amd/csrc/conv_mfma.h
@@ -45,6 +45,10 @@
     int src_g0[kConvMaxSrc];
     int src_gn[kConvMaxSrc];
     int src_ent0[kConvMaxSrc + 1];
+    float *share;
+    int share_off;
+    int share_cout;
+    float share_scale;
 };
 
 typedef _Float16 split_t;
@@ -184,6 +188,10 @@
 size_t s4_packed_floats(const S4Range *r, int n_src, int cout, int ks, int pad_sources);
 void pack_conv_weights_s4(const float *w_oihw, int cin, int cout, int ks, const S4Range *r, int n_src, int pad_sources, float *out);
 int launch_conv_s4(const ConvArgs &a, int ks, int nt, int wide, int B, hipStream_t stream);
+int launch_conv_s4_share(const ConvArgs &a, int nt, int B, hipStream_t stream);
+int launch_conv_s4_add(const ConvArgs &a, int nt, int B, hipStream_t stream);
+inline int share_row0(int p_cout) { return (p_cout + 3) / 4 * 4; }
+bool share_wanted(int p_cin, int p_cout, int c_cin, int c_cout, int h, int w, int B, int mode);
 void pack_conv_weights_s4_ex(const float *w_oihw, int cin, int cout, int ks, const S4Range *r, const int *cstart, int n_src, int pad_sources, float *out);
 
 struct PairArgs {
diff --git a/panoptic-forecasting_amd/csrc/conv_s4.hip b/panoptic-forecasting_amd/csrc/conv_s4.hip
--- a/panoptic-forecasting_amd/csrc/conv_s4.hip
+++ b/panoptic-forecasting_amd/csrc/conv_s4.hip
@@ -40,17 +40,31 @@
 
 #define S4_KERNEL_NAME conv_s4_kernel
 #define S4_KERNEL_KACC 0
+#define S4_KERNEL_EPI 0
 #define S4_KERNEL_WAVES (KS_ == 4 ? 1 : (TH_ == 16 || KS_ == 2) ? 2 : (TW_ == 32 && NT <= 2) ? 4 : (TW_ == 32 && NT == 3) ? 3 : 2)
 #include "conv_s4_kernel.inc"
 #undef S4_KERNEL_NAME
+#undef S4_KERNEL_EPI
+#define S4_KERNEL_NAME conv_s4_share_kernel
+#define S4_KERNEL_EPI 1
+#include "conv_s4_kernel.inc"
+#undef S4_KERNEL_NAME
+#undef S4_KERNEL_EPI
+#define S4_KERNEL_NAME conv_s4_add_kernel
+#define S4_KERNEL_EPI 2
+#include "conv_s4_kernel.inc"
+#undef S4_KERNEL_NAME
+#undef S4_KERNEL_EPI
 #undef S4_KERNEL_KACC
 #undef S4_KERNEL_WAVES
 #define S4_KERNEL_NAME conv_s4_blocked_kernel
 #define S4_KERNEL_KACC 1
+#define S4_KERNEL_EPI 0
 #define S4_KERNEL_WAVES (NT == 1 ? 4 : (NT == 2 ? 3 : 2))
 #include "conv_s4_kernel.inc"
 #undef S4_KERNEL_NAME
 #undef S4_KERNEL_KACC
+#undef S4_KERNEL_EPI
 #undef S4_KERNEL_WAVES
 
 template <int NT, int TW_, int TH_ = 8, int KS_ = 1>
@@ -94,6 +108,57 @@
     PF_LAUNCH_CHECK("conv_s4_blocked_kernel");
     return PF_OK;
 }
+
+template <int NT, bool ADD>
+static int launch_s4_share_cfg(const ConvArgs &a0, int B, hipStream_t s) {
+    using C = S4Cfg<NT, 32, 8, 1>;
+    ConvArgs a = a0;
+    a.tilesX = (a.Wout + C::TW - 1) / C::TW;
+    a.tilesY = (a.Hout + C::TH - 1) / C::TH;
+    const void *fn = ADD ? reinterpret_cast<const void *>(&conv_s4_add_kernel<NT, 32, 8, 1>) : reinterpret_cast<const void *>(&conv_s4_share_kernel<NT, 32, 8, 1>);
+    static bool attr_set = false;
+    if (!attr_set) {
+        PF_HIP_CHECK(hipFuncSetAttribute(fn, hipFuncAttributeMaxDynamicSharedMemorySize, (int)C::LDS_BYTES));
+        attr_set = true;
+    }
+    char label[96];
+    snprintf(label, sizeof(label), "void pf::conv_s4_%s_kernel<%d, 32, 8, 1>(pf::ConvArgs)", ADD ? "add" : "share", NT);
+    const double px = (double)B * a.Hout * a.Wout;
+    const int rows = ADD ? a.Cout : a.Cout + a.share_cout;
+    ProfScope ps(s, label, 2.0 * px * rows * a.Cin * 9,
+                 4.0 * ((double)B * a.Cin * a.Hin * a.Win + px * (a.Cout + (double)(a.share_cout + 3) / 4 * 4) + (double)rows * a.Cin * 9));
+    const dim3 grid(a.tilesX * a.tilesY, (a.ntiles + NT - 1) / NT, B);
+    if (ADD) hipLaunchKernelGGL((conv_s4_add_kernel<NT, 32, 8, 1>), grid, dim3(C::NTHR), C::LDS_BYTES, s, a);
+    else hipLaunchKernelGGL((conv_s4_share_kernel<NT, 32, 8, 1>), grid, dim3(C::NTHR), C::LDS_BYTES, s, a);
+    PF_LAUNCH_CHECK(ADD ? "conv_s4_add_kernel" : "conv_s4_share_kernel");
+    return PF_OK;
+}
+
+static int check_share(const ConvArgs &a, const char *who) {
+    if (!a.src_fmt || !a.dst_fmt) return fail(PF_EINVAL, "%s: sources and destination in the S4 layout only", who);
+    if ((a.Wout & 3) != 0 || a.Hin != a.Hout || a.Win != a.Wout) return fail(PF_EUNSUPPORTED, "%s: stride 1, width %% 4 == 0 only", who);
+    if (a.pool || a.res || a.no_bias || a.kacc) return fail(PF_EUNSUPPORTED, "%s: no fused epilogue stages", who);
+    if (a.chunk_begin != 0 || a.chunk_end != a.nchunks) return fail(PF_EUNSUPPORTED, "%s: whole K range only", who);
+    if (!a.share || a.share_cout < 1 || (reinterpret_cast<uintptr_t>(a.share) & 15) != 0) return fail(PF_EINVAL, "%s: no scratch tensor", who);
+    return PF_OK;
+}
+#define PF_S4_SHARE(ADD_) \
+    nt = nt < 1 ? 1 : (nt > a.ntiles ? a.ntiles : nt); \
+    if (nt == 1) return launch_s4_share_cfg<1, ADD_>(a, B, s); \
+    if (nt == 2) return launch_s4_share_cfg<2, ADD_>(a, B, s); \
+    return launch_s4_share_cfg<3, ADD_>(a, B, s);
+int launch_conv_s4_share(const ConvArgs &a, int nt, int B, hipStream_t s) {
+    if (int rc = check_share(a, "conv_s4 share")) return rc;
+    if ((a.share_off & 3) != 0 || a.share_off < a.Cout || a.share_off + a.share_cout > a.ntiles * 16)
+        return fail(PF_EINVAL, "conv_s4 share: rows %d + %d in %d tiles", a.share_off, a.share_cout, a.ntiles);
+    PF_S4_SHARE(false)
+}
+int launch_conv_s4_add(const ConvArgs &a, int nt, int B, hipStream_t s) {
+    if (int rc = check_share(a, "conv_s4 add")) return rc;
+    if (a.share_cout != a.Cout) return fail(PF_EINVAL, "conv_s4 add: stored sums of %d channels for %d", a.share_cout, a.Cout);
+    PF_S4_SHARE(true)
+}
+#undef PF_S4_SHARE
 
 template <int NT>
 struct S41Cfg {
diff --git a/panoptic-forecasting_amd/csrc/conv_s4_kernel.inc b/panoptic-forecasting_amd/csrc/conv_s4_kernel.inc
--- a/panoptic-forecasting_amd/csrc/conv_s4_kernel.inc
+++ b/panoptic-forecasting_amd/csrc/conv_s4_kernel.inc
@@ -1,6 +1,7 @@
 template <int NT, int TW_, int TH_, int KS_>
 __global__ __launch_bounds__(32 * TH_ * KS_, S4_KERNEL_WAVES) void S4_KERNEL_NAME(ConvArgs a) {
     [[maybe_unused]] constexpr int KACC = S4_KERNEL_KACC;
+    [[maybe_unused]] constexpr int EPI = S4_KERNEL_EPI;
 #if defined(__HIP_DEVICE_COMPILE__)
     using C = S4Cfg<NT, TW_, TH_, KS_>;
     extern __shared__ __attribute__((aligned(16))) unsigned char smem_all[];
@@ -62,7 +63,8 @@
     if (wave_all == 0 && lane < NT * 16) {
         const __amdgpu_buffer_rsrc_t brs = __builtin_amdgcn_make_buffer_rsrc((void *)a.bias, 0, 0x7FFFFFFF, 0x00020000);
         const int co = tile0 * 16 + lane;
-        __builtin_amdgcn_raw_ptr_buffer_load_lds(brs, (s4_lds_ptr_t)bias_lds, 4, co < a.ntiles * 16 ? (unsigned)co * 4u : kS4Oob, 0, 0, 0);
+        const int nbias = EPI == 1 ? (a.Cout + 15) / 16 * 16 : a.ntiles * 16;
+        __builtin_amdgcn_raw_ptr_buffer_load_lds(brs, (s4_lds_ptr_t)bias_lds, 4, co < nbias ? (unsigned)co * 4u : kS4Oob, 0, 0, 0);
     }
 
     const int nrounds = a.nchunks;
@@ -245,6 +247,25 @@
     }
 
     {
+        [[maybe_unused]] s4_f32x4 part[EPI == 2 ? C::MP : 1][EPI == 2 ? NT : 1];
+        [[maybe_unused]] const size_t su_frame = EPI ? (size_t)((a.share_cout + 3) >> 2) * a.Hout * a.Wout : 0;
+        if constexpr (EPI == 2) {
+#pragma unroll
+            for (int m = 0; m < C::MP; ++m) {
+                const int mt = wave * C::MP + m;
+                const int oy = tileY * C::TH + mt / C::MTR;
+                const int ox = tileX * C::TW + (mt % C::MTR) * 16 + (lane & 15);
+                const bool in = oy < a.Hout && ox < a.Wout;
+#pragma unroll
+                for (int n = 0; n < NT; ++n) {
+                    const int co = (tile0 + n) * 16 + 4 * (lane >> 4);
+                    part[m][n] = s4_f32x4{0.f, 0.f, 0.f, 0.f};
+                    if (in && co < a.share_cout)
+                        part[m][n] = reinterpret_cast<const s4_f32x4 *>(a.share)[(size_t)b * su_frame + (size_t)(co >> 2) * a.Hout * a.Wout +
+                                                                                 (size_t)oy * a.Wout + ox];
+                }
+            }
+        }
         __builtin_amdgcn_s_waitcnt(0x0F70);
         const int g = lane >> 4, px = lane & 15;
         const size_t hw = (size_t)a.Hout * a.Wout;
@@ -288,11 +309,26 @@
 #pragma unroll
             for (int n = 0; n < NT; ++n) {
                 const int co = (tile0 + n) * 16 + 4 * g;
+                if constexpr (EPI == 1) {
+                    const int cs = co - a.share_off;
+                    if (cs >= 0) {
+                        if (cs < a.share_cout) {
+                            s4_f32x4 u = acc[m][n];
+#pragma unroll
+                            for (int r = 0; r < 4; ++r) u[r] *= a.share_scale;
+                            reinterpret_cast<s4_f32x4 *>(a.share)[(size_t)b * su_frame + (size_t)(cs >> 2) * hw + pix] = u;
+                        }
+                        continue;
+                    }
+                }
                 if (co >= a.Cout + 2) continue;
                 s4_f32x4 v = acc[m][n];
                 const s4_f32x4 b4 = *reinterpret_cast<const s4_f32x4 *>(bias_lds + n * 16 + 4 * g);
 #pragma unroll
-                for (int r = 0; r < 4; ++r) v[r] = fmaxf(v[r] * a.acc_scale + b4[r], relu_lo);
+                for (int r = 0; r < 4; ++r) {
+                    if constexpr (EPI == 2) v[r] = fmaxf(__builtin_fmaf(v[r], a.acc_scale, part[m][n][r]) + b4[r], relu_lo);
+                    else v[r] = fmaxf(v[r] * a.acc_scale + b4[r], relu_lo);
+                }
                 vmax = range_acc(vmax, v[0], v[1], v[2], v[3]);
                 if (a.dst_fmt) {
                     store_px(co, pix, v);
diff --git a/panoptic-forecasting_amd/csrc/conv_select.cpp b/panoptic-forecasting_amd/csrc/conv_select.cpp
--- a/panoptic-forecasting_amd/csrc/conv_select.cpp
+++ b/panoptic-forecasting_amd/csrc/conv_select.cpp
@@ -66,6 +66,14 @@
     if (mode <= 0) return false;
     const long px = (long)B * h * w;
     return c_cout <= 32 && p_cout <= 16 && px >= 65536 && px <= 196608;
+}
+
+bool share_wanted(int p_cin, int p_cout, int c_cin, int c_cout, int h, int w, int B, int mode) {
+    if (mode >= 2) return true;
+    if (mode <= 0) return false;
+    const int packed = (share_row0(p_cout) + c_cout + 15) / 16, apart = (p_cout + 15) / 16 + (c_cout + 15) / 16;
+    if (packed >= apart || pair_wanted(p_cin, p_cout, c_cin, c_cout, h, w, B, 1)) return false;
+    return p_cout == 10 && c_cout == 18 && p_cin >= 48 && (long)B * h * w >= 4194304;
 }
 
 ConvChoice choose_conv(int ks, int stride, int cin, int cout, int hout, int wout, int B, int need, int use_tuned) {
diff --git a/panoptic-forecasting_amd/csrc/hardnet_plan.h b/panoptic-forecasting_amd/csrc/hardnet_plan.h
--- a/panoptic-forecasting_amd/csrc/hardnet_plan.h
+++ b/panoptic-forecasting_amd/csrc/hardnet_plan.h
@@ -28,6 +28,8 @@
     size_t pair_c_off = 0, pair_two_off = 0, pair_nine_off = 0;
     int pair_rounds = 0;
     bool pair_merged = false;
+    size_t share_a_off = 0, share_b_off = 0;
+    int share_a_tiles = 0, share_b_rounds = 0;
 };
 
 struct PlanOptions {
@@ -39,6 +41,7 @@
     int normalize_ranges = 1;
     int profile_tag_ops = 0;
     int fuse_pairs = 1;
+    int share_s = 1;
 };
 
 struct pf_plan {
@@ -62,7 +65,7 @@
 constexpr size_t kStatusBytes = PF_WS_STATUS_BYTES;
 constexpr int kStickyWord = PF_WS_STICKY_OFFSET / 4, kLiveWord = 2, kSlot0 = 16, kMaxSlots = ((int)(kStatusBytes / 4) - kSlot0) / 2;
 
-int layout(const pf_plan *p, int B, int H, int W, std::vector<Dims> &d, std::vector<size_t> &off, size_t &total);
+int layout(const pf_plan *p, int B, int H, int W, std::vector<Dims> &d, std::vector<size_t> &off, size_t &total, size_t *share_off = nullptr);
 
 bool is_conv_pair(const NetTable &t, size_t i);
 
diff --git a/panoptic-forecasting_amd/csrc/hardnet_plan.hip b/panoptic-forecasting_amd/csrc/hardnet_plan.hip
--- a/panoptic-forecasting_amd/csrc/hardnet_plan.hip
+++ b/panoptic-forecasting_amd/csrc/hardnet_plan.hip
@@ -9,7 +9,7 @@
 namespace {
 
 enum StepKind : uint8_t {
-    S_RANGE_CHECK, S_STEM, S_STEM_FRONT, S_PAIR, S_CONV, S_CONV_S4, S_CONV_GENERIC, S_CONV_SPLIT, S_CONV_SPLIT1, S_CONV_WAVE, S_CONV_DMA,
+    S_RANGE_CHECK, S_STEM, S_STEM_FRONT, S_PAIR, S_CONV, S_CONV_S4, S_CONV_S4_SHARE, S_CONV_S4_ADD, S_CONV_GENERIC, S_CONV_SPLIT, S_CONV_SPLIT1, S_CONV_WAVE, S_CONV_DMA,
     S_POOL, S_UPSAMPLE, S_HEAD };
 struct PlainArgs { const float *src; float *dst; int planes, hin, win, hout, wout; size_t n; unsigned *status, *slot; };
 struct Step {
@@ -35,7 +35,8 @@
     std::vector<Dims> d;
     std::vector<size_t> off;
     size_t ws_need = 0;
-    int rc = layout(p, B, H, W, d, off, ws_need);
+    size_t share_off = (size_t)-1;
+    int rc = layout(p, B, H, W, d, off, ws_need, &share_off);
     if (rc) return rc;
     if (ws_bytes < ws_need) return fail(PF_EWORKSPACE, "workspace %zu B < required %zu B", ws_bytes, ws_need);
     const uint32_t input = p->net.ops[0].src[0].tensor;
@@ -381,11 +382,43 @@
     size_t w = 0;
     for (size_t k = 0; k < steps.size(); ++k, ++w) {
         const size_t i = (size_t)steps[k].op;
-        const bool pair = p->opt.fuse_pairs && k + 1 < steps.size() && steps[k].kind == S_CONV_S4 && steps[k + 1].kind == S_CONV_S4 &&
-                          steps[k + 1].op == (int)i + 1 && is_conv_pair(p->net, i) && p->conv[i + 1].pair_c_off && steps[k].u.c.dst_fmt && steps[k + 1].u.c.dst_fmt;
+        const bool adjacent = k + 1 < steps.size() && steps[k].kind == S_CONV_S4 && steps[k + 1].kind == S_CONV_S4 && steps[k + 1].op == (int)i + 1 &&
+                              is_conv_pair(p->net, i) && steps[k].u.c.dst_fmt && steps[k + 1].u.c.dst_fmt;
+        const bool pair = p->opt.fuse_pairs && adjacent && p->conv[i + 1].pair_c_off;
         const BlobOp &o = p->net.ops[i];
         if (!pair || !pair_wanted((int)o.cin, (int)o.cout, (int)p->net.ops[i + 1].cin, (int)p->net.ops[i + 1].cout, d[o.dst].h, d[o.dst].w, Bt,
                                   p->opt.fuse_pairs)) {
+            if (adjacent && p->opt.share_s && p->conv[i + 1].share_a_off && share_off != (size_t)-1 && steps[k].wide == 0 && steps[k + 1].wide == 0 &&
+                share_wanted((int)o.cin, (int)o.cout, (int)p->net.ops[i + 1].cin, (int)p->net.ops[i + 1].cout, d[o.dst].h, d[o.dst].w, Bt, p->opt.share_s)) {
+                const ConvPlan &cc = p->conv[i + 1];
+                Step sa = steps[k], sb = steps[k + 1];
+                float *const sums = reinterpret_cast<float *>((char *)ws + share_off);
+                ConvArgs &a = sa.u.c, &c = sb.u.c;
+                sa.kind = S_CONV_S4_SHARE;
+                a.wpk = p->dev_weights + cc.share_a_off; a.ntiles = cc.share_a_tiles;
+                a.share = sums; a.share_off = share_row0((int)o.cout); a.share_cout = c.Cout; a.share_scale = cc.split_acc_scale;
+                sa.nt = cc.share_a_tiles <= 3 ? cc.share_a_tiles : 2;
+                sb.kind = S_CONV_S4_ADD;
+                c.Cin -= c.src_cstart[2] - c.src_cstart[1];
+                for (int j = 1; j + 1 < c.n_src; ++j) {
+                    c.src[j] = c.src[j + 1]; c.src_ctotal[j] = c.src_ctotal[j + 1]; c.src_choff[j] = c.src_choff[j + 1];
+                    c.src_c4[j] = c.src_c4[j + 1]; c.src_g0[j] = c.src_g0[j + 1]; c.src_gn[j] = c.src_gn[j + 1];
+                }
+                --c.n_src;
+                int e = 0;
+                for (int j = 0; j <= kConvMaxSrc; ++j) {
+                    c.src_ent0[j] = e;
+                    if (j < c.n_src) e += c.src_gn[j];
+                }
+                c.src_end = c.n_src;
+                c.wpk = p->dev_weights + cc.share_b_off; c.nchunks = cc.share_b_rounds;
+                c.chunk_begin = 0; c.chunk_end = c.nchunks;
+                c.share = sums; c.share_cout = c.Cout;
+                steps[w] = sa;
+                steps[++w] = sb;
+                ++k;
+                continue;
+            }
             if (w != k) steps[w] = steps[k];
             continue;
         }
@@ -460,6 +493,8 @@
                 st.u.sf.front.probe = probe; rc = launch_conv_front(st.u.sf.front, B, s); break;
             case S_PAIR: st.u.pair.c.probe = probe; rc = launch_conv_pair(st.u.pair, B, s); break;
             case S_CONV_S4: rc = launch_conv_s4(a, (int)o.k, st.nt, st.wide, B, s); break;
+            case S_CONV_S4_SHARE: rc = launch_conv_s4_share(a, st.nt, B, s); break;
+            case S_CONV_S4_ADD: rc = launch_conv_s4_add(a, st.nt, B, s); break;
             case S_CONV_GENERIC: rc = launch_conv(a, p->conv[st.ci].tiling, B, s); break;
             case S_CONV_SPLIT: rc = launch_conv_split(a, st.ch.p0, st.ch.p1, B, s); break;
             case S_CONV_SPLIT1: rc = launch_conv_split1(a, st.ch.p0, B, s); break;
diff --git a/panoptic-forecasting_amd/csrc/plan_access.hip b/panoptic-forecasting_amd/csrc/plan_access.hip
--- a/panoptic-forecasting_amd/csrc/plan_access.hip
+++ b/panoptic-forecasting_amd/csrc/plan_access.hip
@@ -1,10 +1,11 @@
+#include <algorithm>
 #include <cstring>
 
 #include "hardnet_plan.h"
 
 using namespace pf;
 
-int pf::layout(const pf_plan *p, int B, int H, int W, std::vector<Dims> &d, std::vector<size_t> &off, size_t &total) {
+int pf::layout(const pf_plan *p, int B, int H, int W, std::vector<Dims> &d, std::vector<size_t> &off, size_t &total, size_t *share_off) {
     int rc = propagate_dims(p->net, H, W, d);
     if (rc) return rc;
     off.assign(p->net.tensors.size(), (size_t)-1);
@@ -15,6 +16,16 @@
         off[t] = cur;
         cur += align_up((size_t)B * ((p->net.tensors[t].channels + 3) / 4 * 4) * d[t].h * d[t].w * sizeof(float), 256);
     }
+    size_t share_bytes = 0;
+    const int Bt = p->opt.table_batch > 0 ? p->opt.table_batch : B;
+    for (size_t i = 1; i < p->net.ops.size(); ++i) {
+        const BlobOp &P = p->net.ops[i - 1], &C = p->net.ops[i];
+        const Dims &o = d[C.dst];
+        if (p->conv[i].share_a_off && p->opt.share_s && share_wanted((int)P.cin, (int)P.cout, (int)C.cin, (int)C.cout, o.h, o.w, Bt, p->opt.share_s))
+            share_bytes = std::max(share_bytes, (size_t)B * ((C.cout + 3) / 4 * 4) * o.h * o.w * sizeof(float));
+    }
+    if (share_off) *share_off = share_bytes ? cur : (size_t)-1;
+    cur += align_up(share_bytes, 256);
     total = cur;
     return PF_OK;
 }
diff --git a/panoptic-forecasting_amd/csrc/plan_create.hip b/panoptic-forecasting_amd/csrc/plan_create.hip
--- a/panoptic-forecasting_amd/csrc/plan_create.hip
+++ b/panoptic-forecasting_amd/csrc/plan_create.hip
@@ -29,6 +29,7 @@
     {"range_guard", nullptr, &PlanOptions::range_guard, nullptr, true, true, false},
     {"fuse_front", nullptr, &PlanOptions::fuse_front, nullptr, true, true, false},
     {"fuse_pairs", nullptr, &PlanOptions::fuse_pairs, nullptr, true, true, false},
+    {"share_s", nullptr, &PlanOptions::share_s, nullptr, true, true, false},
     {"profile_tag_ops", nullptr, &PlanOptions::profile_tag_ops, nullptr, true, true, false},
     {"table_batch", nullptr, &PlanOptions::table_batch, nullptr, false, true, true},
     {"normalize_ranges", nullptr, &PlanOptions::normalize_ranges, nullptr, true, false, false},
@@ -260,6 +261,32 @@
     pack_conv_weights_pair_p(wp.data(), (int)P.cin, (int)P.cout, rs, a.at(c.pair_two_off), a.at(c.pair_nine_off));
 }
 
+void pack_share(const BlobOp &P, const float *wP, const BlobOp &o, const float *ws, Arena &a, ConvPlan &c) {
+    const int n = (int)o.n_src, row0 = share_row0((int)P.cout), rows = row0 + (int)o.cout, cS = (int)o.src[0].ch;
+    std::vector<float> wp, wa((size_t)rows * P.cin * 9, 0.f);
+    scale_weights(wP, (size_t)P.cout * P.cin * 9, wp);
+    std::copy(wp.begin(), wp.end(), wa.begin());
+    for (int co = 0; co < (int)o.cout; ++co)
+        for (int ci = 0; ci < (int)P.cin; ++ci)
+            for (int t = 0; t < 9; ++t) wa[((size_t)(row0 + co) * P.cin + ci) * 9 + t] = ws[((size_t)co * o.cin + cS + ci) * 9 + t];
+    const S4Range rs{(int)P.src[0].choff, (int)P.src[0].ch};
+    c.share_a_tiles = (rows + 15) / 16;
+    c.share_a_off = a.take(s4_packed_floats(&rs, 1, rows, 3, 0), 16);
+    pack_conv_weights_s4(wa.data(), (int)P.cin, rows, 3, &rs, 1, 0, a.at(c.share_a_off));
+    S4Range rg[kConvMaxSrc];
+    int cstart[kConvMaxSrc], c0 = 0;
+    for (int j = 0, k = 0; j < n; ++j) {
+        if (j != 1) {
+            rg[k] = S4Range{(int)o.src[j].choff, (int)o.src[j].ch};
+            cstart[k++] = c0;
+        }
+        c0 += (int)o.src[j].ch;
+    }
+    c.share_b_rounds = s4_rounds(rg, n - 1, 3, 0);
+    c.share_b_off = a.take(s4_packed_floats(rg, n - 1, (int)o.cout, 3, 0), 16);
+    pack_conv_weights_s4_ex(ws, (int)o.cin, (int)o.cout, 3, rg, cstart, n - 1, 0, a.at(c.share_b_off));
+}
+
 void pack_front(const BlobOp &o, const float *ws, Arena &a, ConvPlan &c) {
     const S4Range rg{(int)o.src[0].choff, (int)o.src[0].ch};
     c.front_off = a.take(s4_packed_floats(&rg, 1, (int)o.cout, 3, 0), 16);
@@ -314,6 +341,7 @@
         if (o.stride == 1) pack_split(o, ws, src_ch, a, c);
         if (o.stride == 1 && o.kind == OP_CONV) pack_s4(o, ws, a, c);
         if (i > 0 && is_conv_pair(p.net, i - 1)) pack_pair(ops[i - 1], wts + ops[i - 1].w_off, o, ws, a, c);
+        if (i > 0 && p.opt.share_s && is_conv_pair(p.net, i - 1)) pack_share(ops[i - 1], wts + ops[i - 1].w_off, o, ws, a, c);
         if (o.k == 3 && o.stride == 2 && o.kind == OP_CONV && o.n_src == 1 && (o.src[0].choff & 3) == 0 && o.cout <= 32) pack_front(o, ws, a, c);
         if (o.stride == 1) pack_wave(o, w, src_ch, a, c);
         if (o.kind == OP_STEM) pack_stem(o, w, (int)p.net.hdr.n_cls, a, c);
@@ -386,6 +414,29 @@
     return PF_OK;
 }
 
+extern "C" int pf_debug_plan_arena(const void *blob, size_t bytes, int in_ch, int n_cls, float *out, size_t cap, size_t *n_floats,
+                                   long long *table, int table_ops) {
+    if (!blob || !n_floats) return fail(PF_EINVAL, "pf_debug_plan_arena: null argument");
+    pf_plan p;
+    p.opt = g_plan_opt;
+    int rc = parse_net_table(blob, bytes, in_ch, n_cls, p.net);
+    const size_t n_w = rc ? 0 : (bytes - p.net.hdr.weights_off) / sizeof(float);
+    if (!rc) rc = check_plan_ops(p.net, n_w);
+    if (rc) return rc;
+    const float *w0 = reinterpret_cast<const float *>((const char *)blob + p.net.hdr.weights_off);
+    std::vector<float> wnorm(w0, w0 + n_w), host;
+    normalize_ranges(&p, wnorm);
+    if ((rc = build_plan_weights(p, wnorm.data(), host))) return rc;
+    *n_floats = host.size();
+    if (out && cap >= host.size()) memcpy(out, host.data(), host.size() * sizeof(float));
+    for (int i = 0; table && i < table_ops && i < (int)p.conv.size(); ++i) {
+        const ConvPlan &c = p.conv[i];
+        const long long row[6] = {(long long)c.s4_off, c.s4_rounds, (long long)c.share_a_off, c.share_a_tiles, (long long)c.share_b_off, c.share_b_rounds};
+        memcpy(table + 6 * i, row, sizeof(row));
+    }
+    return PF_OK;
+}
+
 extern "C" void pf_hardnet_plan_destroy(pf_plan *p) {
     if (!p) return;
     if (p->dev_weights) (void)hipFree(p->dev_weights);
diff --git a/panoptic-forecasting_amd/lib.py b/panoptic-forecasting_amd/lib.py
--- a/panoptic-forecasting_amd/lib.py
+++ b/panoptic-forecasting_amd/lib.py
@@ -65,6 +65,7 @@
     'pf_hardnet_plan_set_option': (_i, [_vp, _c.c_char_p, _i]),
     'pf_debug_force_conv': (_i, [_i, _i, _i, _i]),
     'pf_debug_probe_read': (_i, [_c.POINTER(_c.c_longlong)]),
+    'pf_debug_plan_arena': (_i, [_vp, _sz, _i, _i, _vp, _sz, _c.POINTER(_sz), _vp, _i]),
     'pf_profile_enable': (_i, [_i]),
     'pf_profile_collect': (_i, []),
     'pf_profile_get': (_i, [_i, _c.c_char_p, _sz, _c.POINTER(_i), _c.POINTER(_c.c_double),
```

Result: faster. 2898 frames/s, median of 6 (+1.8%).
